# hchautran/SplatFormer

Measured on AMD Instinct MI355X. Metric: refined renders/sec (100k GS, 800x800) at 1/2/4/8 MI355X; PSNR vs ref, higher is better.
Workload: dtype fp32; 1 GPU; B: 100000 Gaussians SH1, full PTv3 (ptv3_base) + heads, 9 views 800x800, forward; parallelism=scene-dp1, attention=non-flash (K=128, ptv3_base.gin:27)

## Files before the change

### include/sfx.h

```cpp
#ifndef SFX_H_
#define SFX_H_

#include <stddef.h>
#include <stdint.h>

#ifdef __cplusplus
extern "C" {
#endif

#define SFX_OK 0
#define SFX_ERR_INVALID -1
#define SFX_ERR_HIP -2
#define SFX_ERR_WORKSPACE -3

int sfx_abi_version(void);
const char* sfx_last_error(void);

size_t sfx_scan_workspace_bytes(long long n);
long long sfx_lookback_timeouts(void* stream);
int sfx_lookback_release(void* stream);
int sfx_scan_i32(long long n, const int32_t* in, int32_t* out, int inclusive, void* ws, size_t ws_bytes,
                 int32_t* total, void* stream);
int sfx_scan_i64(long long n, const int64_t* in, int64_t* out, int inclusive, void* ws, size_t ws_bytes,
                 int64_t* total, void* stream);
// ... 58 lines not shown

int sfx_weight_split(int rows, int cols, const float* w, long long ld, float* w_split, float* w_inv, void* stream);

int sfx_amax_f32(int rows, int cols, const float* x, long long ld, unsigned long long* slot, unsigned tag,
                 void* stream);
int sfx_ln_amax_bound(int C, const float* gamma, const float* beta, unsigned long long* slot, unsigned tag,
                      void* stream);

int sfx_gemm_force_config(int cfg, int stream_k);

int sfx_gemm_force_epilogue(int cls);
int sfx_gemm_last_epilogue(void);

int sfx_set_precision(int mode);
int sfx_get_precision(void);

int sfx_linear_bwd_data(int M, int N, int K, const float* dY, long long ldy, const float* Wt, long long ldwt,
                        const float* rowscale, int dact, int dact_ncols, const float* dact_pre, long long ld_pre,
                        float* dX, long long lddx, int accumulate, const float* wt_split, const float* wt_inv,
                        void* stream);
int sfx_linear_wgrad(int M, int N, int K, const float* dY, long long ldy, const float* X, long long ldx, float* dW,
                     long long ldw, float* db, void* stream);
int sfx_linear_wgrad_rs(int M, int N, int K, const float* dY, long long ldy, const float* X, long long ldx,
                        const float* rowscale, float* scaled, float* dW, long long ldw, float* db, void* stream);
int sfx_subm_conv_wgrad(int n, int cin, int cout, const float* dy, long long ldy, const float* x, long long ldx,
                        const int* nbr, const int* pair_in, const int* pair_out, const int* pair_off_host, float* dw,
                        long long ldw, float* db, void* stream);
int sfx_profile_marker(int tag, void* stream);

int sfx_transpose(int rows, int cols, const float* src, long long lds, float* dst, long long ldd, void* stream);
int sfx_subm_conv_bwd_data(int n, int cin, int cout, const float* dy, long long ldy, const int* nbr,
                           const float* weight_t, const int* pair_in, const int* pair_out, const int* pair_off_host,
                           int* centre_ws, float* dx, long long lddx, const float* wt_split, const float* wt_inv,
                           void* stream);
int sfx_window_attention_bwd(int num_windows, int window, int heads, int head_dim, int channels, const float* qkv,
                             const int* order, const int* win, float scale, const float* attn_out, const float* dout,
                             float* dqkv, float* stats, void* stream);
int sfx_window_attention_varlen_bwd(int num_windows, int max_window, int heads, int head_dim, int channels,
                                    const float* qkv, const int* order, const int* win3, float scale,
                                    const float* dout, float* dqkv, float* stats, void* stream);
int sfx_layernorm_bwd(int M, int C, const float* X, long long ldx, const float* gamma, const float* dY,
                      long long ldgy, const float* dR, long long ldr, float eps, float* dX, long long lddx,
                      void* stream);
size_t sfx_layernorm_wgrad_workspace_bytes(int M, int C);
int sfx_layernorm_wgrad(int M, int C, const float* X, long long ldx, const float* dY, long long ldgy, float eps,
                        void* ws, size_t ws_bytes, float* dgamma, float* dbeta, int accumulate, void* stream);
int sfx_cpe_ln_bwd(int M, int C, const float* U, const float* X1, const float* gamma_cpe, const float* gamma1,
                   const float* dX2, const float* dH, float eps, float* dX1, float* dU, void* stream);
size_t sfx_colsum2_workspace_bytes(int M, int C);
int sfx_bn_stats(int M, int C, const float* X, long long ldx, void* ws, size_t ws_bytes, double* sums, void* stream);
int sfx_bn_finalize(int C, double count, const double* sums, const float* gamma, const float* beta, float eps,
                    float momentum, float* running_mean, float* running_var, float* mean_out, float* rstd_out,
                    float* scale_out, float* shift_out, void* stream);
int sfx_affine_act(int M, int C, const float* X, long long ldx, const float* scale, const float* shift, int act,
                   const float* R, long long ldr, const int* ridx, float* Y, long long ldy, void* stream);
int sfx_bn_act_bwd_reduce(int M, int C, const float* X, long long ldx, const float* mean, const float* rstd,
                          const float* gamma, const float* beta, int act, const float* dY, long long ldgy, void* ws,
                          size_t ws_bytes, double* sums, void* stream);
int sfx_bn_act_bwd_apply(int M, int C, const float* X, long long ldx, const float* mean, const float* rstd,
                         const float* gamma, const float* beta, int act, const float* dY, long long ldgy,
                         const double* sums, double count, float* dX, long long lddx, int accumulate, void* stream);
int sfx_segment_max_arg(int m, int C, const int* idx_ptr, const int* sorted_idx, const float* X, float* Y, int* arg,
                        void* stream);
int sfx_segment_max_bwd(int m, int C, const float* dY, const int* arg, float* dX, void* stream);
int sfx_segment_sum(int m, int C, const int* idx_ptr, const int* sorted_idx, const float* X, long long ldx, float* Y,
                    void* stream);
int sfx_act_bwd(int M, int N, const float* dY, long long ldgy, const float* pre, long long ldp, int act, int ncols,
                float* dX, long long lddx, void* stream);
int sfx_drop_mask(long long n, float keep, unsigned long long seed, float* out, void* stream);
int sfx_sumsq(long long n, const float* x, double* out, void* stream);
int sfx_clip_coef(const double* sumsq, float max_norm, float* coef, float* norm_out, void* stream);
int sfx_adam_step(long long n, float* param, const float* grad, float* exp_avg, float* exp_avg_sq,
                  const float* grad_scale, float lr, float beta1, float beta2, float eps, float weight_decay,
                  int step, void* stream);

int sfx_layernorm(int M, int C, const float* X, long long ldx, const float* gamma, const float* beta, float eps,
                  float* Y, long long ldy, void* stream);
int sfx_cpe_residual_ln(int M, int C, const float* T, const float* X, const float* gamma_cpe, const float* beta_cpe,
                        const float* gamma1, const float* beta1, float eps, float* X_out, float* H, void* stream);
int sfx_cpe_residual_ln_pairs(int M, int C, const float* T, long long ldt, const float* partials, const int* pair_pos,
                              long long num_pairs, const float* X, const float* gamma_cpe, const float* beta_cpe,
                              const float* gamma1, const float* beta1, float eps, float* X_out, float* H,
                              void* stream);
int sfx_cpe_residual_ln_cpairs(int M, int C, const float* T, long long ldt, const float* partials,
                               const int* pair_cpos, long long num_pairs, const float* X, const float* gamma_cpe,
                               const float* beta_cpe, const float* gamma1, const float* beta1, float eps, float* X_out,
                               float* H, void* stream);
int sfx_cpe_ln_qkv_pairs(int M, int C, const float* T, long long ldt, const float* partials, const int* pair_pos,
                         long long num_pairs, const float* X, const float* gamma_cpe, const float* beta_cpe,
                         const float* gamma1, const float* beta1, float eps, float* X_out, const float* w_split,
                         const float* w_inv, const float* bias, float* qkv, unsigned long long* amax_slot,
                         unsigned tag, void* stream);

int sfx_window_attention(int num_windows, int window, int heads, int head_dim, int channels, const float* qkv,
                         const int* order, const int* win, float scale, float* out,
                         const unsigned long long* qkv_amax, unsigned qkv_tag, void* stream);
int sfx_window_attention_varlen(int num_windows, int max_window, int heads, int head_dim, int channels,
                                const float* qkv, const int* order, const int* win3, float scale, float* out,
                                const unsigned long long* qkv_amax, unsigned qkv_tag, void* stream);
int sfx_window_attention_proj(int num_windows, int window, int heads, int head_dim, int channels, const float* qkv,
                              const int* order, const int* win, float scale, const unsigned long long* qkv_amax,
                              unsigned qkv_tag, const float* w_split, const float* w_inv, const float* bias,
                              const float* x1, long long ldx1, float* x2, long long ldx2, void* stream);

int sfx_serialize_keys(int n, const int* grid_coord, const int* batch, int depth, int num_orders, int t0, int t1,
                       int t2, int t3, int code_bits, int64_t* codes, uint64_t* keys, void* stream);
int sfx_serialize_permute(int n, int num_orders, const int* order, const int* inverse, const int64_t* codes,
                          const int* grid, const float* coord, int64_t* codes_p, int* order_p, int* inverse_p,
                          int* grid_p, float* coord_p, void* stream);
int sfx_serialize_finalize(int n, int num_orders, const int* sorted_pos, int* order, int* inverse, void* stream);

int sfx_pool_run_flags(int n, int num_orders, const int* order, const int64_t* codes, int shift, int* flags,
                       void* stream);
int sfx_pool_run_counts(int n, const int* order, const int64_t* codes, const int* shifts, int nshift, int* counts,
                        void* stream);
int sfx_pool_assign_runs(int n, int m, int row0, const int* order, const int* pos, const int* flags, int* cluster,
                         int* idx_ptr, int* head, int* sorted_idx, void* stream);
int sfx_pool_reorder(int n, int m, int num_orders, const int* order, const int* pos, const int* flags,
                     const int* cluster, int* new_order, int* new_inverse, void* stream);
int sfx_pool_gather(int m, int n, int num_orders, const int* head, const int64_t* codes, int pooling_depth,
                    const int* grid_coord, const int* batch, int code_bits, int64_t* new_codes, uint64_t* keys,
                    int* new_grid, int* new_batch, void* stream);
int sfx_segment_max_affine_act(int m, int C, const int* idx_ptr, const int* sorted_idx, const float* X,
                               const float* scale, const float* shift, int act, float* Y, void* stream);
int sfx_segment_mean(int m, int D, const int* idx_ptr, const int* sorted_idx, const float* X, float* Y,
                     void* stream);

int sfx_subm_table_log2(int n);
int sfx_subm_neighbors(int n, const int* grid_coord, const int* batch, int log2cap, unsigned long long* table_keys,
                       int* table_vals, int* nbr, unsigned* mask, unsigned long long* mask_keys, void* stream);
int sfx_subm_permute(int n, const int* perm, const int* nbr, const unsigned* mask, int* nbr_sorted,
                     unsigned* mask_sorted, void* stream);
size_t sfx_subm_pairs_workspace_bytes(int n);
int sfx_subm_pairs(int n, const int* nbr, void* ws, size_t ws_bytes, int* pair_in, int* pair_out, int* pair_off,
                   int with_centre, void* stream);
int sfx_subm_pair_pos(int n, long long num_pairs, const int* pair_out, const int* pair_off, int* pair_pos,
                      void* stream);
size_t sfx_subm_pair_lists_workspace_bytes(int n);
int sfx_subm_pair_lists(int n, const int* nbr, void* ws, size_t ws_bytes, int* pair_in, int* pair_out, int* pair_off,
                        int* pair_pos, int* pair_cpos, int with_centre, void* stream);
int sfx_subm_conv(int n, int cin, int cout, const float* x, long long ldx, const int* nbr, const float* weight,
                  const float* bias, const int* pair_in, const int* pair_out, const int* pair_off_host, float* out,
                  long long ldo, const unsigned long long* x_amax, unsigned x_tag,
                  const unsigned long long* w_amax, unsigned w_tag, const float* w_split, const float* w_inv,
                  void* stream);
int sfx_subm_conv_partials(int n, int cin, int cout, const float* x, long long ldx, const int* nbr,
                           const float* weight, const float* bias, const int* pair_in, const int* pair_out,
                           const int* pair_off_host, float* out, long long ldo, float* partials, long long ldp,
                           const float* w_split, const float* w_inv, void* stream);
int sfx_subm_conv_partials_pairs(int n, int cin, int cout, const float* x, long long ldx, const int* nbr,
                                 const float* weight, const float* bias, const int* pair_in, const int* pair_out,
                                 const int* pair_off_host, float* out, long long ldo, float* partials, long long ldp,
                                 const float* w_split, const float* w_inv, void* stream);

int sfx_gs_pack(int n, const float* means, long long ld_means, const float* scales, long long ld_scales,
                const float* opacities, long long ld_opacities, const float* quats, long long ld_quats,
                const float* features_dc, long long ld_dc, const float* features_rest, long long ld_rest,
                int rest_dim, float grid_resolution, float* feat, long long ld_feat, int* grid_coord, int* grid_max,
                void* stream);
int sfx_offsets_to_batch(int n, int B, const long long* offsets, int* batch, void* stream);
int sfx_move_rows(long long n, int words, const void* src, long long src_ld, const int* idx, void* dst,
                  long long dst_ld, int scatter, void* stream);

int sfx_render_prep_project_views(int n, int views, int num_bases, const float* means, long long ld_means,
                                  const float* log_scales, long long ld_scales, const float* quats_raw,
                                  long long ld_quats, const float* opac_logit, long long ld_opac,
                                  const float* features_dc, long long ld_dc, const float* features_rest,
                                  long long ld_rest, const float* camera_to_worlds, float fx, float fy, float cx,
                                  float cy, int img_h, int img_w, int block_width, float* rgbs, float* opacities,
                                  float* xys, float* depths, int* radii, float* conics, int* num_tiles_hit,
                                  float* records, void* stream);
int sfx_isect_emit_views(int n_total, int n_per_view, const float* xys, const float* depths, const int* radii,
                         const int* cum_tiles_hit, int tiles_x, int tiles_y, int block_width, int64_t* isect_ids,
                         int32_t* gaussian_ids, long long capacity, void* stream);
int sfx_rasterize_fwd_views(int views, int tiles_x, int tiles_y, int block_width, int img_h, int img_w,
                            const int32_t* gids_sorted, const int* tile_bins, const float* xys, const float* conics,
                            const float* colors, const float* opacity, const float* background, int clamp_max1,
                            float* final_Ts, int* final_idx, float* out_img, float* out_alpha, void* stream);
int sfx_isect_count_cull_views(int n_total, int n_per_view, const float* xys, const float* conics,
                               const float* opacities, const int* radii, int tiles_x, int tiles_y, int block_width,
                               int img_h, int img_w, int* num_tiles_kept, void* stream);
int sfx_isect_emit_cull_views(int n_total, int n_per_view, const float* xys, const float* conics,
                              const float* opacities, const float* depths, const int* radii, const int* cum_tiles_hit,
                              int tiles_x, int tiles_y, int block_width, int img_h, int img_w, int64_t* isect_ids,
                              int32_t* gaussian_ids, const int* rank, long long capacity, void* stream);
int sfx_depth_keys(long long n, const float* depths, uint64_t* keys, void* stream);
int sfx_invert_permutation(long long n, const int* perm, int* inv, void* stream);
int sfx_rasterize_fwd_views_quad(int views, int tiles_x, int tiles_y, int block_width, int img_h, int img_w,
                                 const int32_t* gids_sorted, const int* tile_bins, const float* records,
                                 const float* background, int clamp_max1, float* final_Ts, int* final_idx,
                                 float* out_img, float* out_alpha, void* stream);
int sfx_rasterize_bwd_quad(int tiles_x, int tiles_y, int block_width, int img_h, int img_w, const int32_t* gids_sorted,
                           const int* tile_bins, const float* xys, const float* conics, const float* colors,
                           const float* opacity, const float* background, const float* final_Ts, const int* final_idx,
                           const float* v_out, const float* v_out_alpha, float* v_xy, float* v_xy_abs, float* v_conic,
                           float* v_rgb, float* v_opacity, void* stream);
int sfx_rasterize_bwd_views_quad(int views, int tiles_x, int tiles_y, int block_width, int img_h, int img_w,
                                 const int32_t* gids_sorted, const int* tile_bins, const float* xys,
                                 const float* conics, const float* colors, const float* opacity,
                                 const float* background, const float* final_Ts, const int* final_idx,
                                 const float* v_out, const float* v_out_alpha, float* v_xy, float* v_xy_abs,
                                 float* v_conic, float* v_rgb, float* v_opacity, void* stream);
int sfx_render_prep_project_views_bwd(int n, int views, int num_bases, const float* means, long long ld_means,
                                      const float* log_scales, long long ld_scales, const float* quats_raw,
                                      long long ld_quats, const float* opac_logit, long long ld_opac,
                                      const float* features_dc, long long ld_dc, const float* features_rest,
                                      long long ld_rest, const float* camera_to_worlds, float fx, float fy,
                                      const int* radii, const float* conics, const float* v_xys,
                                      const float* v_conics, const float* v_rgbs, const float* v_opacities,
                                      float* v_means, long long ld_v_means, float* v_log_scales,
                                      long long ld_v_scales, float* v_quats_raw, long long ld_v_quats,
                                      float* v_opac_logit, long long ld_v_opac, float* v_features_dc,
                                      long long ld_v_dc, float* v_features_rest, long long ld_v_rest, void* stream);
int sfx_rasterize_fwd_nd(int tiles_x, int tiles_y, int block_width, int img_h, int img_w, int channels,
                         const int32_t* gids_sorted, const int* tile_bins, const float* xys, const float* conics,
                         const float* colors, const float* opacity, const float* background, float* final_Ts,
                         int* final_idx, float* out_img, float* out_alpha, void* stream);
int sfx_rasterize_bwd_nd(int tiles_x, int tiles_y, int block_width, int img_h, int img_w, int channels,
                         const int32_t* gids_sorted, const int* tile_bins, const float* xys, const float* conics,
                         const float* colors, const float* opacity, const float* background, const float* final_Ts,
                         const int* final_idx, const float* v_out, const float* v_out_alpha, float* v_xy,
                         float* v_xy_abs, float* v_conic, float* v_colors, float* v_opacity, void* stream);

int sfx_image_stats_u8(int num_images, long long elems_per_image, const float* pred, const float* gt,
                       int clamp_pred, unsigned long long* sums, int* maxes, void* stream);
size_t sfx_ssim_workspace_bytes(int num_images, int height, int width, int channels);
int sfx_ssim(int num_images, int height, int width, int channels, const float* img1, const float* img2,
             const float* window, int quantize_u8, float* out, void* ws, size_t ws_bytes, void* stream);
size_t sfx_image_loss_workspace_bytes(int num_images, int height, int width, int channels);
int sfx_image_loss(int num_images, int height, int width, int channels, const float* pred, const float* gt,
                   const float* window, float l1_weight, float ssim_weight, const float* view_scale, float* terms,
                   float* d_pred, void* ws, size_t ws_bytes, void* stream);

int sfx_voxel_keys(int n, const float* points, long long ld, float voxel_size, unsigned long long* keys,
                   void* stream);
int sfx_nn1(int n, int m, const float* queries, const float* refs, int* out, void* stream);
int sfx_fps(int n, int m, const float* xyz, int start, int* out, float* dist_ws, void* stream);

size_t sfx_mlp_stream_floats(int C);
size_t sfx_mlp_params_floats(int C);
int sfx_mlp_pack(int C, const float* w1, const float* b1, const float* w2, const float* b2, const float* gamma,
                 const float* beta, float* stream, float* params, int* workspace, void* stream_);
int sfx_block_mlp(int M, int C, const float* x, long long ldx, const float* stream, const float* params, float eps,
                  float* y, long long ldy, int* rowexp, void* stream_);
int sfx_block_mlp_last_plan(int* kind, int* split, int* main_wgs, int* tail_wgs, int* pts);
int sfx_block_mlp_train(int M, int C, const float* x, long long ldx, const float* stream, const float* params,
                        float eps, const float* rowscale, float* z, float* y, long long ldy, void* stream_);
int sfx_block_mlp_bwd(int M, int C, const float* dy, long long lddy, const float* stream, const float* params,
                      const float* rowscale, const float* z, float* dh2, long long lddh, void* stream_);

size_t sfx_subm_cpe_pack_bytes(int C);
int sfx_subm_cpe_pack(int C, const float* w, void* wpk, float* winv, float* ws, void* stream);
int sfx_subm_order_keys(int n, const int* nbr, uint64_t* keys, void* stream);
int sfx_subm_rowexp(int n, int C, const float* x, int* e, void* stream);
int sfx_subm_cpe_ln(int n, int C, const float* xc, const float* xres, const int* nbr, const int* perm,
                    const int* rowexp, const void* wpk, const float* winv, const float* bias, const float* gamma_cpe,
                    const float* beta_cpe, const float* gamma1, const float* beta1, float eps, float* x_out,
                    float* h_out, void* stream);

int sfx_point_embed(int n, int K, int N, const float* x, long long ldx, const float* w, const float* b,
                    const float* scale, const float* shift, float* y, long long ldy, void* stream);

size_t sfx_heads_stream_floats(int ng, int kin);
size_t sfx_heads_params_floats(int out_dim);
int sfx_heads_pack(int ng, int kin, int out_dim, const float* w1, int ld1, const float* b1, const float* wm,
                   const float* bm, const float* w4, const float* b4, float* stream, float* params, int* ws,
                   void* stream_);
int sfx_heads(int M, int ng, int kin, int out_dim, const float* x, long long ldx, int res_off, int n_tanh,
              const int* ocols, const float* stream, const float* params, float* y, void* stream_);

#ifdef __cplusplus
}
#endif

#endif
```

### splatformer_amd/csrc/gemm.hip

```cpp
#include <climits>
#include <cstdlib>
#include <cstring>
#include <type_traits>

#include "gemm_common.h"


namespace {

using namespace sfxg;

inline bool aligned16(const void* p) { return (reinterpret_cast<uintptr_t>(p) & 15) == 0; }

inline bool fits(long long rows, long long ld) { return rows * ld * 4 + 64 < (long long)OOB; }

struct TileCfg {
  int bm, bn, nw;
  float eff;
};
constexpr TileCfg kCfgs[] = {{128, 128, 4, 1.0f}, {128, 96, 4, 0.95f}, {128, 64, 4, 0.8f}, {64, 128, 4, 0.95f},
                             {64, 64, 4, 0.8f},   {256, 128, 8, 1.05f}, {128, 256, 8, 1.05f}};
constexpr int kNumCfgs = sizeof(kCfgs) / sizeof(kCfgs[0]);

thread_local int g_prec = 0;
// ... 461 lines not shown
      const int row = 4 * c4 + j;
#pragma unroll
      for (int q = 0; q < NQ; ++q)
        *reinterpret_cast<uint4*>(img + (op * 3 + q) * WG2_PLANE + chunk_off(row, mg)) =
            make_uint4(t0[q].x, t0[q].y, t1[q].x, t1[q].y);
    }
    __syncthreads();
    if (m0 + BK < m_end) {
      load(m0 + BK);
      load_idx(m0 + 2 * BK);
    }
#pragma unroll
    for (int s = 0; s < 2; ++s) {
      bf16x8 af[2][3], bf[2][3];
#pragma unroll
      for (int i = 0; i < 2; ++i)
#pragma unroll
        for (int q = 0; q < NQ; ++q) {
          af[i][q] = __builtin_bit_cast(bf16x8, *reinterpret_cast<const uint4*>(
                                                    img + q * WG2_PLANE + chunk_off(wn * 64 + i * 32 + l32, 2 * s + h)));
          bf[i][q] = __builtin_bit_cast(bf16x8, *reinterpret_cast<const uint4*>(
                                                    img + (3 + q) * WG2_PLANE + chunk_off(wk * 64 + i * 32 + l32, 2 * s + h)));
        }
      constexpr int QA[6] = {2, 1, 0, 1, 0, 0}, QB[6] = {0, 1, 2, 0, 1, 0};
#pragma unroll
      for (int i = 0; i < 2; ++i)
#pragma unroll
        for (int j = 0; j < 2; ++j)
#pragma unroll
          for (int p = NQ == 3 ? 0 : 3; p < 6; ++p)
            acc[i][j] = __builtin_amdgcn_mfma_f32_32x32x16_bf16(af[i][QA[p]], bf[j][QB[p]], acc[i][j], 0, 0, 0);
    }
  }
  if (do_db) {
#pragma unroll
    for (int j = 0; j < 4; ++j)
      if (col + j < N) atomicAdd(&db[col + j], dbs[j]);
  }
  const __amdgpu_buffer_rsrc_t rW = rsrc(dW);
  const unsigned ldw32 = (unsigned)ldw;
#pragma unroll
  for (int i = 0; i < 2; ++i)
#pragma unroll
    for (int j = 0; j < 2; ++j) {
      const int k = k0 + wk * 64 + j * 32 + l32;
#pragma unroll
      for (int r = 0; r < 16; ++r) {
        const int n = n0 + wn * 64 + i * 32 + (r & 3) + 8 * (r >> 2) + 4 * h;
        __builtin_amdgcn_raw_ptr_buffer_atomic_fadd_f32(
            acc[i][j][r], rW, (n < N && k < K) ? ((unsigned)n * ldw32 + (unsigned)k) * 4u : OOB, 0, 0);
      }
    }
}

template <int NQ, int SRC>
__global__ void __launch_bounds__(256, 2) wgrad2_kernel(int M, int N, int K, const float* __restrict__ dY,
                                                        long long ldy, const float* __restrict__ X, long long ldx,
                                                        float* __restrict__ dW, long long ldw, int chunk,
                                                        float* __restrict__ db) {
  __shared__ __attribute__((aligned(16))) char img[2 * 3 * WG2_PLANE];
  const int tiles_k = (K + WG2_T - 1) / WG2_T;
  const int n0 = (blockIdx.x / tiles_k) * WG2_T, k0 = (blockIdx.x % tiles_k) * WG2_T;
  const int m_begin = blockIdx.y * chunk;
  const int m_end = min(M, m_begin + chunk);
  wgrad2_body<NQ, SRC>(img, m_begin, m_end, N, K, n0, k0, dY, ldy, X, ldx, dW, ldw, db, nullptr, nullptr, 0, 0);
}

struct SubmWgradPlan {
  int pair_off[28];
  int item_off[28];
  int chunk;
};

template <int NQ>
__global__ void __launch_bounds__(256, 2) subm_wgrad_kernel(int n, int cin, int cout, const float* __restrict__ dY,
                                                            long long ldy, const float* __restrict__ X, long long ldx,
                                                            const int* __restrict__ nbr,
                                                            const int* __restrict__ pair_in,
                                                            const int* __restrict__ pair_out, SubmWgradPlan plan,
                                                            float* __restrict__ dW, long long ldw,
                                                            float* __restrict__ db) {
  __shared__ __attribute__((aligned(16))) char img[2 * 3 * WG2_PLANE];
  const int tiles_k = (cin + WG2_T - 1) / WG2_T;
  const int n0 = (blockIdx.x / tiles_k) * WG2_T, k0 = (blockIdx.x % tiles_k) * WG2_T;
  const int item = blockIdx.y;
  int k = 0;
  while (k < 26 && item >= plan.item_off[k + 1]) ++k;
  const bool centre = k == 13;
  const int base = centre ? 0 : plan.pair_off[k];
  const int count = centre ? n : plan.pair_off[k + 1] - base;
  const int m_begin = base + (item - plan.item_off[k]) * plan.chunk;
  const int m_end = min(base + count, m_begin + plan.chunk);
  wgrad2_body<NQ, WG2_PAIRS>(img, m_begin, m_end, cout, cin, n0, k0, dY, ldy, X, ldx, dW + (long long)k * cin, ldw,
                             centre ? db : nullptr, centre ? nullptr : pair_out, centre ? nbr : pair_in,
                             centre ? 27 : 1, centre ? 13 : 0);
}

__global__ void __launch_bounds__(256) rowscale_rows_kernel(int M, int n4, const float* __restrict__ dY, long long ldy,
                                                            const float* __restrict__ rowscale,
                                                            float* __restrict__ out) {
  const long long i = (long long)blockIdx.x * 256 + threadIdx.x;
  if (i >= (long long)M * n4) return;
  const int m = (int)(i / n4), c = (int)(i % n4) * 4;
  const float s = rowscale[m];
  const float4 v = *reinterpret_cast<const float4*>(dY + (long long)m * ldy + c);
  *reinterpret_cast<float4*>(out + i * 4) = make_float4(v.x * s, v.y * s, v.z * s, v.w * s);
}

__global__ void __launch_bounds__(256) transpose_kernel(int rows, int cols, const float* __restrict__ src,
                                                        long long lds, float* __restrict__ dst, long long ldd) {
  __shared__ float t[32][33];
  const int r0 = blockIdx.y * 32, c0 = blockIdx.x * 32;
  const int tx = threadIdx.x & 31, ty = threadIdx.x >> 5;
  for (int i = ty; i < 32; i += 8) {
    const int r = r0 + i, c = c0 + tx;
    t[i][tx] = (r < rows && c < cols) ? src[(long long)r * lds + c] : 0.f;
  }
  __syncthreads();
  for (int i = ty; i < 32; i += 8) {
    const int c = c0 + i, r = r0 + tx;
    if (c < cols && r < rows) dst[(long long)c * ldd + r] = t[tx][i];
  }
}


__global__ void centre_pairs_kernel(int n, const int* __restrict__ nbr, int* __restrict__ gather,
                                    int* __restrict__ scatter) {
  const int i = blockIdx.x * 256 + threadIdx.x;
  if (i >= n) return;
  gather[i] = i;
  scatter[i] = nbr[(long long)i * 27 + 13];
}

}

extern "C" {

int sfx_gemm_force_config(int cfg, int stream_k) {
  SFX_REQUIRE(cfg >= -1 && cfg < kNumCfgs && stream_k >= -1 && stream_k <= 1, "sfx_gemm_force_config: bad values");
  read_force_env();
  forced = cfg;
  forced_sk = stream_k;
  return SFX_OK;
}

int sfx_gemm_force_epilogue(int cls) {
  SFX_REQUIRE(cls == -1 || cls == 0, "sfx_gemm_force_epilogue: class %d (-1 automatic, 0 general)", cls);
  forced_epi = cls;
  return SFX_OK;
}

int sfx_gemm_last_epilogue(void) { return last_epi; }

int sfx_weight_split(int rows, int cols, const float* w, long long ld, float* w_split, float* w_inv, void* stream) {
  SFX_REQUIRE(rows >= 0 && cols > 0 && cols % 4 == 0 && ld >= cols && ld % 4 == 0,
              "sfx_weight_split: bad sizes (cols and ld must be multiples of 4)");
  if (rows == 0) return SFX_OK;
  SFX_REQUIRE(w && w_split && w_inv, "sfx_weight_split: null buffer");
  SFX_REQUIRE((reinterpret_cast<uintptr_t>(w) & 15) == 0 && (reinterpret_cast<uintptr_t>(w_split) & 15) == 0,
              "sfx_weight_split: buffers must be 16-byte aligned");
  weight_split_kernel<<<sfx::ceil_div(rows, 4), 256, 0, sfx::as_stream(stream)>>>(rows, cols, w, ld, w_split, w_inv);
  return sfx::check_launch("sfx_weight_split");
}

int sfx_amax_f32(int rows, int cols, const float* x, long long ld, unsigned long long* slot, unsigned tag,
                 void* stream) {
  SFX_REQUIRE(rows >= 0 && cols >= 0 && ld >= cols, "sfx_amax_f32: bad sizes");
  SFX_REQUIRE(slot && tag != 0, "sfx_amax_f32: null slot or tag 0");
  SFX_REQUIRE(rows == 0 || cols == 0 || x, "sfx_amax_f32: null buffer");
  const AmaxJob j{x, ld, 0, rows, cols, 1, nullptr, 0, 1};
  amax_kernel<<<dim3(amax_blocks(j), 1), 256, 0, sfx::as_stream(stream)>>>(j, j, slot, slot, tag, tag);
  return sfx::check_launch("sfx_amax_f32");
}

int sfx_linear(int M, int N, int K, const float* A, long long lda, const int* gather_idx, int num_segments,
               const float* W, long long ldw, const float* bias, const float* scale, const float* shift, int act,
               int act_ncols, const float* R, long long ldr, const int* residual_idx, float* Y, long long ldy,
               float* Ypre, long long ldypre, int groups, long long group_stride_A, long long group_stride_W,
               long long group_stride_bias, long long group_stride_Y, const int* out_row_idx, const float* rowscale,
               int pre_before_act, const unsigned long long* a_amax, unsigned a_tag,
               const unsigned long long* w_amax, unsigned w_tag, unsigned long long* y_amax, unsigned y_tag,
               const float* w_split, const float* w_inv, void* stream) {
  SFX_REQUIRE(M >= 0 && N > 0 && K > 0, "sfx_linear: bad sizes M=%d N=%d K=%d", M, N, K);
  SFX_REQUIRE(act >= 0 && act <= 3, "sfx_linear: bad activation %d", act);
  SFX_REQUIRE(groups >= 1, "sfx_linear: groups < 1");
  if (M == 0) return SFX_OK;
  SFX_REQUIRE(A && W && Y, "sfx_linear: null buffer");
  const int S = gather_idx ? num_segments : 1;
  SFX_REQUIRE(!gather_idx || (S >= 1 && K % S == 0), "sfx_linear: K must be a multiple of num_segments");
  const int Kseg = K / S;
  SFX_REQUIRE(!gather_idx || Kseg % 4 == 0, "sfx_linear: gathered segment width must be a multiple of 4");
  SFX_REQUIRE(ldw >= K && (gather_idx || lda >= K) && ldy >= N, "sfx_linear: leading dimension too small");
  SFX_REQUIRE(!(scale == nullptr) == !(shift == nullptr), "sfx_linear: scale and shift go together");
  SFX_REQUIRE((gather_idx || fits(M, lda)) && fits(M, ldy) && fits(N, ldw) && (!R || residual_idx || fits(M, ldr)) &&
                  (!Ypre || fits(M, ldypre)),
              "sfx_linear: operand exceeds the 2 GiB buffer-descriptor range");
  GemmArgs a{};
  a.M = M; a.N = N; a.K = K; a.A = A; a.lda = lda; a.gidx = gather_idx; a.S = S; a.Kseg = Kseg; a.gstride = S;
  a.W = W; a.ldw = ldw; a.bias = bias; a.scale = scale; a.shift = shift; a.act = act;
  a.act_ncols = act_ncols < 0 ? N : act_ncols; a.R = R; a.ldr = ldr; a.ridx = residual_idx; a.Y = Y; a.ldy = ldy;
  a.Ypre = Ypre; a.ldypre = ldypre; a.gA = group_stride_A; a.gW = group_stride_W; a.gB = group_stride_bias;
  a.gY = group_stride_Y; a.out_rows = out_row_idx; a.rowscale = rowscale; a.pre_before_act = pre_before_act;
  a.a_amax = a_amax; a.a_tag = a_tag; a.w_amax = w_amax; a.w_tag = w_tag; a.y_amax = y_amax; a.y_tag = y_tag;
  const bool vec = (K % 4 == 0) && (lda % 4 == 0) && (ldw % 4 == 0) && aligned16(A) && aligned16(W) &&
                   (group_stride_A % 4 == 0) && (group_stride_W % 4 == 0);
  SFX_REQUIRE(!w_split == !w_inv, "sfx_linear: w_split and w_inv go together");
  if (w_split && vec && aligned16(w_split)) {
    SFX_REQUIRE(groups == 1 || group_stride_W == (long long)N * K, "sfx_linear: w_split needs contiguous groups");
    a.Wsp = w_split; a.ldws = K; a.winv = w_inv; a.gWinv = N;
  }
  dispatch(a, groups, vec, sfx::as_stream(stream));
  return sfx::check_launch("sfx_linear");
}

static int subm_conv_impl(int n, int cin, int cout, const float* x, long long ldx, const int* nbr,
                          const float* weight, const float* bias, const int* pair_in, const int* pair_out,
                          const int* pair_off_host, float* out, long long ldo, const unsigned long long* x_amax,
                          unsigned x_tag, const unsigned long long* w_amax, unsigned w_tag, const float* w_split,
                          const float* w_inv, float* partials, long long ldp, void* stream,
                          bool skip_centre = false) {
  SFX_REQUIRE(n >= 0 && cin > 0 && cout > 0, "sfx_subm_conv: bad sizes");
  if (n == 0) return SFX_OK;
  SFX_REQUIRE(x && nbr && weight && out && pair_off_host, "sfx_subm_conv: null buffer");
  SFX_REQUIRE(ldx >= cin && ldo >= cout, "sfx_subm_conv: leading dimension too small");
  SFX_REQUIRE(fits(n, ldx) && fits(n, ldo) && fits(cout, 27ll * cin),
              "sfx_subm_conv: operand exceeds the 2 GiB buffer-descriptor range");
  SFX_REQUIRE(!partials || (ldp >= cout && fits(pair_off_host[27], ldp)),
              "sfx_subm_conv_partials: partials leading dimension too small or too large");
  hipStream_t st = sfx::as_stream(stream);
  const bool vec = (cin % 4 == 0) && (ldx % 4 == 0) && aligned16(x) && aligned16(weight);
  GemmArgs a{};
  a.M = n; a.N = cout; a.K = cin; a.A = x; a.lda = ldx; a.gidx = nbr + 13; a.S = 1; a.Kseg = cin; a.gstride = 27;
  for (const TunedLaunch& t : kTunedConv)
    if (t.N == cout && t.K == cin && 5ll * n >= 4ll * t.M && 4ll * n <= 5ll * t.M) {
      a.tuned = t.cfg + 1;
      a.tuned_sk = t.sk;
      break;
    }
  a.W = weight + 13ll * cin; a.ldw = 27ll * cin; a.bias = bias; a.act = 0; a.act_ncols = cout; a.Y = out; a.ldy = ldo;
  a.a_amax = x_amax; a.a_tag = x_tag; a.w_amax = w_amax; a.w_tag = w_tag;
  SFX_REQUIRE(!w_split == !w_inv, "sfx_subm_conv: w_split and w_inv go together");
  if (w_split && vec && aligned16(w_split)) {
    a.Wsp = w_split + 13ll * cin; a.ldws = 27ll * cin; a.winv = w_inv;
  }
  if (!a.Wsp && vec && split_mode(cin) == 2 &&
      !prepare_amax(a, AmaxJob{x, ldx, 0, n, cin, 1, nullptr, 0, 1},
                    AmaxJob{weight, 27ll * cin, 0, cout, 27 * cin, 1, nullptr, 0, 1}, st)) {
    a.a_amax = a.w_amax = nullptr;
  }
  if (!skip_centre) {
    dispatch(a, 1, vec, st);
    int rc = sfx::check_launch("sfx_subm_conv(centre)");
    if (rc) return rc;
  }
  if (!pair_in || pair_off_host[27] == 0) return SFX_OK;
  GemmArgs b = a;
  b.gidx = nullptr; b.bias = nullptr; b.gstride = 1; b.pair_mode = 1; b.pair_in = pair_in; b.pair_out = pair_out;
  b.W = weight; b.slice_w_stride = cin; b.num_slices = 27;
  if (a.Wsp) b.Wsp = w_split;
  for (int k = 0; k <= 27; ++k) b.slice_pair_off[k] = pair_off_host[k];
  b.M = pair_off_host[27];
  if (partials) {
    b.pair_store = 1;
    b.Y = partials;
    b.ldy = ldp;
  }
  dispatch(b, 1, vec, st);
  return sfx::check_launch("sfx_subm_conv(pairs)");
}

int sfx_subm_conv(int n, int cin, int cout, const float* x, long long ldx, const int* nbr, const float* weight,
                  const float* bias, const int* pair_in, const int* pair_out, const int* pair_off_host, float* out,
                  long long ldo, const unsigned long long* x_amax, unsigned x_tag,
                  const unsigned long long* w_amax, unsigned w_tag, const float* w_split, const float* w_inv,
                  void* stream) {
  return subm_conv_impl(n, cin, cout, x, ldx, nbr, weight, bias, pair_in, pair_out, pair_off_host, out, ldo, x_amax,
                        x_tag, w_amax, w_tag, w_split, w_inv, nullptr, 0, stream);
}

int sfx_subm_conv_partials(int n, int cin, int cout, const float* x, long long ldx, const int* nbr,
                           const float* weight, const float* bias, const int* pair_in, const int* pair_out,
                           const int* pair_off_host, float* out, long long ldo, float* partials, long long ldp,
                           const float* w_split, const float* w_inv, void* stream) {
  SFX_REQUIRE(n == 0 || pair_off_host[27] == 0 || (partials && pair_in && pair_out),
              "sfx_subm_conv_partials: null partials / pair lists");
  return subm_conv_impl(n, cin, cout, x, ldx, nbr, weight, bias, pair_in, pair_out, pair_off_host, out, ldo, nullptr,
                        0, nullptr, 0, w_split, w_inv, partials, ldp, stream);
}

int sfx_subm_conv_partials_pairs(int n, int cin, int cout, const float* x, long long ldx, const int* nbr,
                                 const float* weight, const float* bias, const int* pair_in, const int* pair_out,
                                 const int* pair_off_host, float* out, long long ldo, float* partials, long long ldp,
                                 const float* w_split, const float* w_inv, void* stream) {
  SFX_REQUIRE(n == 0 || pair_off_host[27] == 0 || (partials && pair_in && pair_out),
              "sfx_subm_conv_partials_pairs: null partials / pair lists");
  return subm_conv_impl(n, cin, cout, x, ldx, nbr, weight, bias, pair_in, pair_out, pair_off_host, out, ldo, nullptr,
                        0, nullptr, 0, w_split, w_inv, partials, ldp, stream, true);
}

int sfx_subm_conv_bwd_data(int n, int cin, int cout, const float* dy, long long ldy, const int* nbr,
                           const float* weight_t, const int* pair_in, const int* pair_out, const int* pair_off_host,
                           int* centre_ws, float* dx, long long lddx, const float* wt_split, const float* wt_inv,
                           void* stream) {
  SFX_REQUIRE(n >= 0 && cin > 0 && cout > 0, "sfx_subm_conv_bwd_data: bad sizes");
  if (n == 0) return SFX_OK;
  SFX_REQUIRE(dy && nbr && weight_t && dx && pair_off_host && centre_ws, "sfx_subm_conv_bwd_data: null buffer");
  SFX_REQUIRE(ldy >= cout && lddx >= cin, "sfx_subm_conv_bwd_data: leading dimension too small");
  SFX_REQUIRE(fits(n, ldy) && fits(n, lddx) && fits(27ll * cin, cout),
              "sfx_subm_conv_bwd_data: operand exceeds the 2 GiB buffer-descriptor range");
  hipStream_t st = sfx::as_stream(stream);
  const bool vec = (cout % 4 == 0) && (ldy % 4 == 0) && aligned16(dy) && aligned16(weight_t);
  SFX_REQUIRE(!wt_split == !wt_inv, "sfx_subm_conv_bwd_data: wt_split and wt_inv go together");
  const bool presplit = wt_split && vec && aligned16(wt_split);
  GemmArgs am{};
  if (!presplit && vec && split_mode(cout) == 2)
    (void)prepare_amax(am, AmaxJob{dy, ldy, 0, n, cout, 1, nullptr, 0, 1},
                       AmaxJob{weight_t, (long long)cout, 0, 27 * cin, cout, 1, nullptr, 0, 1}, st);
  int* cg = centre_ws;
  int* cs = centre_ws + n;
  centre_pairs_kernel<<<sfx::ceil_div(n, 256), 256, 0, st>>>(n, nbr, cg, cs);
  GemmArgs a{};
  a.N = cin; a.K = cout; a.A = dy; a.lda = ldy; a.S = 1; a.Kseg = cout; a.gstride = 1;
  a.ldw = cout; a.act = 0; a.act_ncols = cin; a.Y = dx; a.ldy = lddx;
  a.pair_mode = 1; a.slice_w_stride = (long long)cin * cout;
  a.a_amax = am.a_amax; a.a_tag = am.a_tag; a.w_amax = am.w_amax; a.w_tag = am.w_tag;
  if (presplit) { a.ldws = cout; a.winv = wt_inv; a.slice_winv_stride = cin; }
  GemmArgs c = a;
  c.pair_in = cg; c.pair_out = cs; c.W = weight_t + 13ll * cin * cout; c.num_slices = 1;
  if (presplit) { c.Wsp = wt_split + 13ll * cin * cout; c.winv = wt_inv + 13ll * cin; }
  c.slice_pair_off[0] = 0; c.slice_pair_off[1] = n; c.M = n;
  dispatch(c, 1, vec, st);
  int rc = sfx::check_launch("sfx_subm_conv_bwd_data(centre)");
  if (rc || !pair_in || pair_off_host[27] == 0) return rc;
  GemmArgs b = a;
  b.pair_in = pair_out; b.pair_out = pair_in; b.W = weight_t; b.num_slices = 27;
  if (presplit) b.Wsp = wt_split;
  for (int k = 0; k <= 27; ++k) b.slice_pair_off[k] = pair_off_host[k];
  b.M = pair_off_host[27];
  dispatch(b, 1, vec, st);
  return sfx::check_launch("sfx_subm_conv_bwd_data(pairs)");
}

int sfx_linear_bwd_data(int M, int N, int K, const float* dY, long long ldy, const float* Wt, long long ldwt,
                        const float* rowscale, int dact, int dact_ncols, const float* dact_pre, long long ld_pre,
                        float* dX, long long lddx, int accumulate, const float* wt_split, const float* wt_inv,
                        void* stream) {
  SFX_REQUIRE(M >= 0 && N > 0 && K > 0, "sfx_linear_bwd_data: bad sizes M=%d N=%d K=%d", M, N, K);
  SFX_REQUIRE(dact >= 0 && dact <= 3, "sfx_linear_bwd_data: bad dact %d", dact);
  if (M == 0) return SFX_OK;
  SFX_REQUIRE(dY && Wt && dX && (!dact || dact_pre), "sfx_linear_bwd_data: null buffer");
  SFX_REQUIRE(ldy >= N && ldwt >= N && lddx >= K && (!dact || ld_pre >= K), "sfx_linear_bwd_data: leading dim");
  SFX_REQUIRE(fits(M, ldy) && fits(K, ldwt) && fits(M, lddx) && (!dact || fits(M, ld_pre)),
              "sfx_linear_bwd_data: operand exceeds the 2 GiB buffer-descriptor range");
  GemmArgs a{};
  a.M = M; a.N = K; a.K = N; a.A = dY; a.lda = ldy; a.S = 1; a.Kseg = N; a.gstride = 1;
  a.W = Wt; a.ldw = ldwt; a.act = 0; a.act_ncols = dact_ncols < 0 ? K : dact_ncols;
  a.Y = dX; a.ldy = lddx;
  if (accumulate) { a.R = dX; a.ldr = lddx; }
  a.rowscale = rowscale; a.dact = dact; a.dact_pre = dact_pre; a.ld_dact = ld_pre;
  const bool vec = (N % 4 == 0) && (ldy % 4 == 0) && (ldwt % 4 == 0) && aligned16(dY) && aligned16(Wt);
  SFX_REQUIRE(!wt_split == !wt_inv, "sfx_linear_bwd_data: wt_split and wt_inv go together");
  if (wt_split && vec && aligned16(wt_split)) {
    a.Wsp = wt_split; a.ldws = N; a.winv = wt_inv;
  }
  dispatch(a, 1, vec, sfx::as_stream(stream));
  return sfx::check_launch("sfx_linear_bwd_data");
}

int sfx_set_precision(int mode) {
  SFX_REQUIRE(mode == 0 || mode == 1, "sfx_set_precision: mode %d (0 fp32-accurate, 1 reference precision)", mode);
  g_prec = mode;
  return SFX_OK;
}

int sfx_get_precision(void) { return g_prec; }

static int linear_wgrad(const char* what, int M, int N, int K, const float* dY, long long ldy, const float* X,
                        long long ldx, float* dW, long long ldw, float* db, void* stream) {
  SFX_REQUIRE(M >= 0 && N > 0 && K > 0, "%s: bad sizes M=%d N=%d K=%d", what, M, N, K);
  if (M == 0) return SFX_OK;
  SFX_REQUIRE(dY && X && dW, "%s: null buffer", what);
  SFX_REQUIRE(N % 4 == 0 && K % 4 == 0 && ldy % 4 == 0 && ldx % 4 == 0 && aligned16(dY) && aligned16(X),
              "%s: N, K, leading dims must be multiples of 4 and operands 16-byte aligned", what);
  SFX_REQUIRE(ldy >= N && ldx >= K && ldw >= K, "%s: leading dim", what);
  SFX_REQUIRE(fits(M, ldy) && fits(M, ldx) && fits(N, ldw), "%s: operand exceeds 2 GiB range", what);
  hipStream_t st = sfx::as_stream(stream);
  const int slabs = (int)sfx::ceil_div(M, BK);
  if (split_mode(M) != 0) {
    const int tiles2 = (int)(sfx::ceil_div(N, WG2_T) * sfx::ceil_div(K, WG2_T));
    int splits2 = (int)sfx::ceil_div(2 * num_cus(), tiles2);
    if (splits2 > slabs) splits2 = slabs;
    if (splits2 < 1) splits2 = 1;
    const int chunk2 = (int)sfx::ceil_div(slabs, splits2) * BK;
    splits2 = (int)sfx::ceil_div(M, chunk2);
    if (g_prec == 1)
      wgrad2_kernel<2, WG2_DENSE><<<dim3(tiles2, splits2), 256, 0, st>>>(M, N, K, dY, ldy, X, ldx, dW, ldw, chunk2, db);
    else
      wgrad2_kernel<3, WG2_DENSE><<<dim3(tiles2, splits2), 256, 0, st>>>(M, N, K, dY, ldy, X, ldx, dW, ldw, chunk2, db);
    return sfx::check_launch(what);
  }
  const int tiles = (int)(sfx::ceil_div(N, WG_TILE) * sfx::ceil_div(K, WG_TILE));
  int splits = (int)sfx::ceil_div(4 * num_cus(), tiles);
  if (splits > slabs) splits = slabs;
  if (splits < 1) splits = 1;
  const int chunk = (int)sfx::ceil_div(slabs, splits) * BK;
  splits = (int)sfx::ceil_div(M, chunk);
  wgrad_kernel<<<dim3(tiles, splits), THREADS, 0, st>>>(M, N, K, dY, ldy, X, ldx, dW, ldw, chunk, db);
  return sfx::check_launch(what);
}

int sfx_linear_wgrad(int M, int N, int K, const float* dY, long long ldy, const float* X, long long ldx, float* dW,
                     long long ldw, float* db, void* stream) {
  return linear_wgrad("sfx_linear_wgrad", M, N, K, dY, ldy, X, ldx, dW, ldw, db, stream);
}

int sfx_linear_wgrad_rs(int M, int N, int K, const float* dY, long long ldy, const float* X, long long ldx,
                        const float* rowscale, float* scaled, float* dW, long long ldw, float* db, void* stream) {
  if (!rowscale || M <= 0) return linear_wgrad("sfx_linear_wgrad_rs", M, N, K, dY, ldy, X, ldx, dW, ldw, db, stream);
  SFX_REQUIRE(N > 0 && N % 4 == 0 && dY && ldy >= N && ldy % 4 == 0 && aligned16(dY) && fits(M, ldy),
              "sfx_linear_wgrad_rs: bad dY");
  SFX_REQUIRE(scaled && aligned16(scaled) && fits(M, N), "sfx_linear_wgrad_rs: scaled must be M*N floats, 16-byte aligned");
  rowscale_rows_kernel<<<sfx::ceil_div((long long)M * (N / 4), 256), 256, 0, sfx::as_stream(stream)>>>(
      M, N / 4, dY, ldy, rowscale, scaled);
  int rc = sfx::check_launch("sfx_linear_wgrad_rs(scale)");
  if (rc) return rc;
  return linear_wgrad("sfx_linear_wgrad_rs", M, N, K, scaled, N, X, ldx, dW, ldw, db, stream);
}

int sfx_subm_conv_wgrad(int n, int cin, int cout, const float* dy, long long ldy, const float* x, long long ldx,
                        const int* nbr, const int* pair_in, const int* pair_out, const int* pair_off_host, float* dw,
                        long long ldw, float* db, void* stream) {
  SFX_REQUIRE(n >= 0 && cin > 0 && cout > 0, "sfx_subm_conv_wgrad: bad sizes");
  if (n == 0) return SFX_OK;
  SFX_REQUIRE(dy && x && nbr && dw && pair_off_host, "sfx_subm_conv_wgrad: null buffer");
  SFX_REQUIRE(cin % 4 == 0 && cout % 4 == 0 && ldy % 4 == 0 && ldx % 4 == 0 && aligned16(dy) && aligned16(x),
              "sfx_subm_conv_wgrad: channels and leading dims must be multiples of 4 and operands 16-byte aligned");
  SFX_REQUIRE(ldy >= cout && ldx >= cin && ldw >= 27ll * cin, "sfx_subm_conv_wgrad: leading dimension too small");
  SFX_REQUIRE(fits(n, ldy) && fits(n, ldx) && fits(cout, ldw) && fits(n, 27),
              "sfx_subm_conv_wgrad: operand exceeds the 2 GiB buffer-descriptor range");
  const int pairs = pair_off_host[27];
  SFX_REQUIRE(pair_off_host[0] == 0 && pairs >= 0 && pairs <= 26ll * n && pair_off_host[14] == pair_off_host[13],
              "sfx_subm_conv_wgrad: pair offsets are not those of lists without the centre offset");
  for (int k = 0; k < 27; ++k)
    SFX_REQUIRE(pair_off_host[k + 1] >= pair_off_host[k], "sfx_subm_conv_wgrad: pair offsets decrease");
  SFX_REQUIRE(pairs == 0 || (pair_in && pair_out && fits(pairs, 1)), "sfx_subm_conv_wgrad: null pair lists");
  const int tiles = (int)(sfx::ceil_div(cout, WG2_T) * sfx::ceil_div(cin, WG2_T));
  const long long total = (long long)n + pairs;
  const long long want = sfx::ceil_div(2 * num_cus(), tiles);
  SubmWgradPlan plan;
  plan.chunk = (int)sfx::ceil_div(sfx::ceil_div(total, want), BK) * BK;
// ... 27 lines not shown
```

### splatformer_amd/csrc/gemm_common.h

```cpp
#pragma once

#include <type_traits>

#include "common.h"

namespace sfxg {

typedef float floatx16 __attribute__((ext_vector_type(16)));
typedef float floatx4 __attribute__((ext_vector_type(4)));
typedef __bf16 bf16x8 __attribute__((ext_vector_type(8)));

constexpr int BK = 32;
#ifndef SFX_PERCU4
#define SFX_PERCU4 2
#endif
#ifndef SFX_PERCU8
#define SFX_PERCU8 1
#endif
#ifndef SFX_NBUF8
#define SFX_NBUF8 2
#endif
constexpr int kPerCu4 = SFX_PERCU4, kPerCu8 = SFX_PERCU8;
constexpr int LDS_STRIDE = BK + 4;
constexpr int THREADS = 256;
constexpr unsigned OOB = 0x7ffffff0u;
constexpr int RSRC_FLAGS = 0x00020000;

enum Act { ACT_NONE = 0, ACT_GELU = 1, ACT_RELU = 2, ACT_TANH = 3 };
enum Epi { EPI_GENERAL = 0, EPI_LIN = 1, EPI_LIN_GELU = 2, EPI_PAIR_STORE = 3 };

struct GemmArgs {
  int M, N, K;
  const float* A;
  long long lda;
  const int* gidx;
  int S, Kseg, gstride;
  const float* W;
  long long ldw;
  const float* bias;
  const float* scale;
  const float* shift;
  int act, act_ncols;
  const float* R;
  long long ldr;
  const int* ridx;
  float* Y;
  long long ldy;
  float* Ypre;
  long long ldypre;
  long long gA, gW, gB, gY;
  const int* out_rows;
  int pair_mode;
  const int* pair_in;
  const int* pair_out;
  int slice_tile_off[28];
  int slice_pair_off[28];
  int num_slices;
  long long slice_w_stride;
  const float* rowscale;
  int pre_before_act;
  const float* dact_pre;
  long long ld_dact;
  int dact;
  int sk;
  int split;
  const unsigned long long* a_amax;
  const unsigned long long* w_amax;
  unsigned a_tag, w_tag;
  unsigned long long* y_amax;
  unsigned y_tag;
  const float* Wsp;
  long long ldws;
  const float* winv;
  long long gWinv;
  long long slice_winv_stride;
  int tuned, tuned_sk;
  int pair_store;
  int epi;
  int dbg;
};

__device__ __forceinline__ int row_exp(float m) {
  int e = __builtin_amdgcn_frexp_expf(m);
  e = 13 - e;
  return e > 126 ? 126 : (e < -126 ? -126 : e);
}

__device__ __forceinline__ float gelu_erf(float x) {
  const float t = fminf(fabsf(x), 5.65f);
  float q = 2.79405867e-06f;
  q = __builtin_fmaf(q, t, -3.89084234e-05f);
  q = __builtin_fmaf(q, t, 0.000184072458f);
  q = __builtin_fmaf(q, t, 0.000141672252f);
  q = __builtin_fmaf(q, t, -0.00706906663f);
  q = __builtin_fmaf(q, t, 0.0524996631f);
  q = __builtin_fmaf(q, t, 0.459207207f);
  q = __builtin_fmaf(q, t, 1.15110528f);
  const float half_tail = 0.5f * __builtin_amdgcn_exp2f(-(t * q));
  return x >= 0.f ? x * (1.f - half_tail) : (x < -5.65f ? 0.f : x * half_tail);
}
__device__ __forceinline__ float gelu_erf_grad(float x) {
  const float cdf = 0.5f * (1.f + erff(x * 0.70710678118654752f));
  const float pdf = 0.39894228040143268f * expf(-0.5f * x * x);
  return cdf + x * pdf;
}
enum DAct { DACT_NONE = 0, DACT_GELU = 1, DACT_RELU = 2, DACT_TANH_OUT = 3 };
__device__ __forceinline__ float dact_grad(int dact, float pre) {
  if (dact == DACT_GELU) return gelu_erf_grad(pre);
  if (dact == DACT_RELU) return pre > 0.f ? 1.f : 0.f;
  return 1.f - pre * pre;
}

__device__ __forceinline__ __amdgpu_buffer_rsrc_t rsrc(const void* p) {
  const unsigned long long a = reinterpret_cast<unsigned long long>(p);
  const unsigned lo = __builtin_amdgcn_readfirstlane((unsigned)a);
  const unsigned hi = __builtin_amdgcn_readfirstlane((unsigned)(a >> 32));
  void* u = reinterpret_cast<void*>(((unsigned long long)hi << 32) | lo);
  return __builtin_amdgcn_make_buffer_rsrc(u, (short)0, (int)OOB, RSRC_FLAGS);
}

__device__ __forceinline__ __amdgpu_buffer_rsrc_t rsrc_ext(const void* p, unsigned bytes) {
  const unsigned long long a = reinterpret_cast<unsigned long long>(p);
  const unsigned lo = __builtin_amdgcn_readfirstlane((unsigned)a);
  const unsigned hi = __builtin_amdgcn_readfirstlane((unsigned)(a >> 32));
  void* u = reinterpret_cast<void*>(((unsigned long long)hi << 32) | lo);
  return __builtin_amdgcn_make_buffer_rsrc(u, (short)0, (int)__builtin_amdgcn_readfirstlane(bytes), RSRC_FLAGS);
}

__device__ __forceinline__ float4 bload4(__amdgpu_buffer_rsrc_t r, unsigned off) {
  const floatx4 v = __builtin_bit_cast(floatx4, __builtin_amdgcn_raw_buffer_load_b128(r, off, 0, 0));
  return make_float4(v.x, v.y, v.z, v.w);
}
__device__ __forceinline__ float bload1(__amdgpu_buffer_rsrc_t r, unsigned off) {
  return __builtin_bit_cast(float, __builtin_amdgcn_raw_buffer_load_b32(r, off, 0, 0));
}
__device__ __forceinline__ int bload1i(__amdgpu_buffer_rsrc_t r, unsigned off) {
  return (int)__builtin_amdgcn_raw_buffer_load_b32(r, off, 0, 0);
}
__device__ __forceinline__ void bstore1(__amdgpu_buffer_rsrc_t r, unsigned off, float v) {
  __builtin_amdgcn_raw_buffer_store_b32(__builtin_bit_cast(unsigned, v), r, off, 0, 0);
}

using sfx::split3;
using sfx::split2h;

enum Mode { MODE_DENSE = 0, MODE_GATHER1 = 1, MODE_GATHERS = 2, MODE_PAIR = 3 };

inline int num_cus() {
  static int cus = 0;
  if (!cus) {
    int dev = 0;
    (void)hipGetDevice(&dev);
    if (hipDeviceGetAttribute(&cus, hipDeviceAttributeMultiprocessorCount, dev) != hipSuccess || cus <= 0) cus = 256;
  }
  return cus;
}

inline int tiles_m_of(GemmArgs& a, int BM) {
  if (!a.pair_mode) return (int)sfx::ceil_div(a.M, BM);
  int t = 0;
  for (int k = 0; k < a.num_slices; ++k) {
    a.slice_tile_off[k] = t;
    t += (a.slice_pair_off[k + 1] - a.slice_pair_off[k] + BM - 1) / BM;
  }
  a.slice_tile_off[a.num_slices] = t;
  return t;
}

void launch_m0_w4(int cfg, const GemmArgs& a, int groups, bool vec, hipStream_t st);
void launch_m0_w8(int cfg, const GemmArgs& a, int groups, bool vec, hipStream_t st);
void launch_m1_w4(int cfg, const GemmArgs& a, int groups, bool vec, hipStream_t st);
void launch_m1_w8(int cfg, const GemmArgs& a, int groups, bool vec, hipStream_t st);
void launch_m2_w4(int cfg, const GemmArgs& a, int groups, bool vec, hipStream_t st);
void launch_m3_w4(int cfg, const GemmArgs& a, int groups, bool vec, hipStream_t st);
void launch_m3_w8(int cfg, const GemmArgs& a, int groups, bool vec, hipStream_t st);

}
```

### splatformer_amd/csrc/gemm_kernel.h

```cpp
#pragma once
#include <climits>
#include <cstdlib>
#include <cstring>
#include <type_traits>

#include "gemm_common.h"


namespace {

using namespace sfxg;



template <int BM, int BN, int WGM, int NW, bool VEC, int MODE, int SPL, int EPI = EPI_GENERAL>
__global__ void __launch_bounds__(NW * 64, NW == 4 ? 2 : 1) gemm_kernel(GemmArgs p, int tiles_n, int total_tiles) {
  constexpr bool SPLIT = SPL != 0;
  static_assert(EPI == EPI_GENERAL || (SPL == 2 && VEC), "specialised epilogues: fp16x2 operands only");
  static_assert((EPI != EPI_LIN && EPI != EPI_LIN_GELU) || MODE == MODE_DENSE, "EPI_LIN*: dense rows");
  static_assert(EPI != EPI_PAIR_STORE || MODE == MODE_PAIR, "EPI_PAIR_STORE: pair mode");
  constexpr bool F16 = SPL == 2 || SPL == 1;
  constexpr int NTERM = SPL == 1 ? 1 : (F16 ? 2 : 3);
  static_assert(SPL == 0 || SPL == 1 || SPL == 2 || SPL == 3, "operand precision");
  constexpr int NT = NW * 64;
  constexpr int WGN = NW / WGM;
  constexpr int WM = BM / WGM, WN = BN / WGN;
  constexpr int MB = WM / 32, NB = WN / 32;
  constexpr int RPP = NT / 8;
  static_assert(WM % 32 == 0 && WN % 32 == 0 && (BM * BK / 4) % NT == 0 && (BN * BK / 4) % NT == 0,
                "tile shape must split into 32x32 MFMA blocks and whole staging passes");
  static_assert(SPLIT || NW == 4, "fp32 tiles run 4 waves");
  constexpr int A_ITERS = BM * BK / 4 / NT;
  constexpr int W_ITERS = BN * BK / 4 / NT;
  constexpr int NBUF = SPLIT ? (NW == 8 ? SFX_NBUF8 : 1) : 2;
  constexpr int AUX_FLOATS = F16 ? NBUF * BM + 2 * BM + 4 : 0;
  constexpr int A_FLOATS = (SPLIT ? NBUF * NTERM * BM * BK / 2 : 2 * BM * LDS_STRIDE) + AUX_FLOATS;
  constexpr int W_FLOATS = SPLIT ? NBUF * NTERM * BN * BK / 2 : 2 * BN * LDS_STRIDE;
  __shared__ __attribute__((aligned(16))) float sAraw[A_FLOATS];
  __shared__ __attribute__((aligned(16))) float sWraw[W_FLOATS];
  float (*sA)[BM * LDS_STRIDE] = reinterpret_cast<float (*)[BM * LDS_STRIDE]>(sAraw);
  float (*sW)[BN * LDS_STRIDE] = reinterpret_cast<float (*)[BN * LDS_STRIDE]>(sWraw);
  char* sAs = reinterpret_cast<char*>(sAraw);
  char* sWs = reinterpret_cast<char*>(sWraw);
  auto swz = [](int r, int c4) -> int { return r * 64 + ((((c4 >> 1) ^ (r >> 2)) & 3) << 4) + ((c4 & 1) << 3); };
  float* s_fac = sAraw + (A_FLOATS - AUX_FLOATS);
  float* s_inv = s_fac + NBUF * BM;
  int* s_flag = reinterpret_cast<int*>(s_inv + 2 * BM);

  const int g = blockIdx.z;
  const float* A = p.A + g * p.gA;
  const float* bias = p.bias ? p.bias + g * p.gB : nullptr;
  float* Y = p.Y + g * p.gY;
  const __amdgpu_buffer_rsrc_t rA = rsrc(A);
  const __amdgpu_buffer_rsrc_t rY = rsrc(Y);
  const __amdgpu_buffer_rsrc_t rR = rsrc(p.R ? p.R : Y);
  const __amdgpu_buffer_rsrc_t rP = rsrc(p.Ypre ? p.Ypre : Y);

  const int tid = threadIdx.x, lane = tid & 63, wid = tid >> 6;
  const int wm = wid / WGN, wn = wid % WGN;
  const int h = lane >> 5, l32 = lane & 31;
  const int K = p.K;
  const int nk = (K + BK - 1) / BK;
  if constexpr (F16) {
    if (tid < NBUF) s_flag[tid] = 0;
  }
  const unsigned lda32 = (unsigned)p.lda, ldw32 = (unsigned)p.ldw, ldy32 = (unsigned)p.ldy, ldws32 = (unsigned)p.ldws;
  const unsigned ldr32 = (unsigned)p.ldr, ldp32 = (unsigned)p.ldypre;
  const int lrow = tid >> 3, lcol = (tid & 7) * 4;

  struct Tile {
    int m0, n0, M;
    const int* gidx;
    int gstride;
    const int* out_rows;
    const float* W;
    const float* winv;
  };
  auto tile_info = [&](int t) -> Tile {
    Tile ti;
    const int tm = t / tiles_n, tn = t - tm * tiles_n;
    ti.n0 = tn * BN;
    ti.m0 = tm * BM;
    ti.M = p.M;
    ti.gidx = MODE == MODE_DENSE ? nullptr : p.gidx;
    ti.gstride = p.gstride;
    ti.out_rows = p.out_rows;
    ti.W = (F16 ? p.Wsp : p.W) + g * p.gW;
    ti.winv = p.winv ? p.winv + g * p.gWinv : nullptr;
    if constexpr (MODE == MODE_PAIR) {
      int sl = 0;
      for (int q = 1; q < p.num_slices; ++q)
        if (p.slice_tile_off[q] <= tm) sl = q;
      const int base = p.slice_pair_off[sl];
      ti.M = p.slice_pair_off[sl + 1] - base;
      ti.m0 = (tm - p.slice_tile_off[sl]) * BM;
      ti.gidx = p.pair_in + base;
      ti.gstride = 1;
      ti.out_rows = p.pair_out + base;
      ti.W = (F16 ? p.Wsp : p.W) + sl * p.slice_w_stride;
      if (p.winv) ti.winv = p.winv + sl * p.slice_winv_stride;
    }
    return ti;
  };

  int grow[A_ITERS];
  auto load_rows = [&](const Tile& ti, int kt, int (&rows)[A_ITERS]) {
    if constexpr (MODE != MODE_DENSE) {
      const __amdgpu_buffer_rsrc_t rG = rsrc(ti.gidx);
      const int seg = MODE == MODE_GATHERS ? (kt * BK + lcol) / p.Kseg : 0;
#pragma unroll
      for (int i = 0; i < A_ITERS; ++i) {
        const int m = ti.m0 + lrow + RPP * i;
        rows[i] = bload1i(rG, (m < ti.M && seg < p.S) ? ((unsigned)m * (unsigned)ti.gstride + (unsigned)seg) * 4u
                                                      : OOB);
      }
    }
  };

  float4 ra[A_ITERS], rw[W_ITERS];
  auto load_tiles = [&](const Tile& ti, int kt, bool first) {
    const __amdgpu_buffer_rsrc_t rW = rsrc(ti.W);
    const int k = kt * BK + lcol;
    const bool kin = k < K && !(p.dbg & 2);
    int seg = 0, kk = k;
    if constexpr (MODE == MODE_GATHERS) {
      seg = k / p.Kseg;
      kk = k - seg * p.Kseg;
    }
#pragma unroll
    for (int i = 0; i < A_ITERS; ++i) {
      const int m = ti.m0 + lrow + RPP * i;
      const bool mok = m < ti.M;
      unsigned off;
      if constexpr (MODE != MODE_DENSE) {
        const int r = grow[i];
        off = (mok && r >= 0 && kin && seg < p.S) ? ((unsigned)r * lda32 + (unsigned)kk) * 4u : OOB;
      } else {
        off = (mok && kin) ? ((unsigned)m * lda32 + (unsigned)kk) * 4u : OOB;
      }
      if (VEC) {
        ra[i] = bload4(rA, off);
      } else {
        float4 v;
        v.x = bload1(rA, (k + 0 < K) ? off : OOB);
        v.y = bload1(rA, (k + 1 < K) ? off + 4 : OOB);
        v.z = bload1(rA, (k + 2 < K) ? off + 8 : OOB);
        v.w = bload1(rA, (k + 3 < K) ? off + 12 : OOB);
        ra[i] = v;
      }
    }
#pragma unroll
    for (int i = 0; i < W_ITERS; ++i) {
      const int n = ti.n0 + lrow + RPP * i;
      const unsigned off = (n < p.N && kin) ? ((unsigned)n * (F16 ? ldws32 : ldw32) + (unsigned)k) * 4u : OOB;
      if (VEC) {
        rw[i] = bload4(rW, off);
      } else {
        float4 v;
        v.x = bload1(rW, (k + 0 < K) ? off : OOB);
        v.y = bload1(rW, (k + 1 < K) ? off + 4 : OOB);
        v.z = bload1(rW, (k + 2 < K) ? off + 8 : OOB);
        v.w = bload1(rW, (k + 3 < K) ? off + 12 : OOB);
        rw[i] = v;
      }
    }
  };
  int erow[A_ITERS];
  float srow[A_ITERS], thr[A_ITERS];
#pragma unroll
  for (int i = 0; i < A_ITERS; ++i) { erow[i] = INT_MIN; srow[i] = 1.f; thr[i] = 0.f; }
  int sq = 0, cq = 0;
  int sp = 0;
  auto store_tiles = [&](int buf, bool first, int par) {
    if (p.dbg & 8) return;
    if constexpr (SPLIT) {
      const int b = NBUF == 2 ? buf : 0;
      if constexpr (F16) {
        ++sq;
        float m[A_ITERS];
        bool over = false;
#pragma unroll
        for (int i = 0; i < A_ITERS; ++i) {
          m[i] = fmaxf(fmaxf(fabsf(ra[i].x), fabsf(ra[i].y)), fmaxf(fabsf(ra[i].z), fabsf(ra[i].w)));
          over |= m[i] > thr[i];
        }
        bool dec = false;
        if (first || __builtin_amdgcn_ballot_w64(over) != 0) {
#pragma unroll
          for (int i = 0; i < A_ITERS; ++i) {
            float mr = m[i];
            mr = fmaxf(mr, __int_as_float(__builtin_amdgcn_mov_dpp(__float_as_int(mr), 0xB1, 0xF, 0xF, false)));
            mr = fmaxf(mr, __int_as_float(__builtin_amdgcn_mov_dpp(__float_as_int(mr), 0x4E, 0xF, 0xF, false)));
            mr = fmaxf(mr, __int_as_float(__builtin_amdgcn_mov_dpp(__float_as_int(mr), 0x141, 0xF, 0xF, false)));
            int e = first ? INT_MIN : erow[i];
            float fac = 1.f;
            bool chg = first;
            if (mr > 0.f && mr <= 3.4028235e38f) {
              int e2 = 13 - __builtin_amdgcn_frexp_expf(mr);
              e2 = e2 > 126 ? 126 : (e2 < -126 ? -126 : e2);
              if (e == INT_MIN) {
                e = e2;
                chg = true;
              } else if (mr * srow[i] > 65504.f) {
                fac = ldexpf(1.f, e2 - e);
                e = e2;
                chg = true;
                dec = true;
              }
            }
            erow[i] = e;
            const bool set = e != INT_MIN;
            srow[i] = set ? ldexpf(1.f, e) : 1.f;
            thr[i] = set ? ldexpf(65504.f, -e) : 0.f;
            if ((tid & 7) == 0) {
              s_fac[b * BM + lrow + RPP * i] = fac;
              if (chg) s_inv[par * BM + lrow + RPP * i] = set ? ldexpf(1.f, -e) : 1.f;
            }
          }
        } else if ((tid & 7) == 0) {
#pragma unroll
          for (int i = 0; i < A_ITERS; ++i) s_fac[b * BM + lrow + RPP * i] = 1.f;
        }
        if (__builtin_amdgcn_ballot_w64(dec) != 0 && lane == 0) s_flag[b] = sq;
#pragma unroll
        for (int i = 0; i < A_ITERS; ++i) {
          uint2 t[2];
          split2h(ra[i], srow[i], t);
          const int o = swz(lrow + RPP * i, lcol >> 2);
          *reinterpret_cast<uint2*>(sAs + ((b * NTERM + 0) * BM) * 64 + o) = t[0];
          if constexpr (NTERM == 2) *reinterpret_cast<uint2*>(sAs + ((b * NTERM + 1) * BM) * 64 + o) = t[1];
        }
#pragma unroll
        for (int i = 0; i < W_ITERS; ++i) {
          const uint4 w = __builtin_bit_cast(uint4, rw[i]);
          const int o = swz(lrow + RPP * i, lcol >> 2);
          *reinterpret_cast<uint2*>(sWs + ((b * NTERM + 0) * BN) * 64 + o) = make_uint2(w.x, w.y);
          if constexpr (NTERM == 2) *reinterpret_cast<uint2*>(sWs + ((b * NTERM + 1) * BN) * 64 + o) = make_uint2(w.z, w.w);
        }
        return;
      } else {
#pragma unroll
      for (int i = 0; i < A_ITERS; ++i) {
        uint2 t[NTERM];
        split3(ra[i], t);
        const int o = swz(lrow + RPP * i, lcol >> 2);
#pragma unroll
        for (int q = 0; q < NTERM; ++q) *reinterpret_cast<uint2*>(sAs + ((b * NTERM + q) * BM) * 64 + o) = t[q];
      }
#pragma unroll
      for (int i = 0; i < W_ITERS; ++i) {
        uint2 t[NTERM];
        split3(rw[i], t);
        const int o = swz(lrow + RPP * i, lcol >> 2);
#pragma unroll
        for (int q = 0; q < NTERM; ++q) *reinterpret_cast<uint2*>(sWs + ((b * NTERM + q) * BN) * 64 + o) = t[q];
      }
      return;
      }
    }
#pragma unroll
    for (int i = 0; i < A_ITERS; ++i)
      *reinterpret_cast<float4*>(&sA[buf][(lrow + RPP * i) * LDS_STRIDE + lcol]) = ra[i];
#pragma unroll
    for (int i = 0; i < W_ITERS; ++i)
      *reinterpret_cast<float4*>(&sW[buf][(lrow + RPP * i) * LDS_STRIDE + lcol]) = rw[i];
  };

  floatx16 acc[MB][NB];
  auto zero_acc = [&]() {
#pragma unroll
    for (int a = 0; a < MB; ++a)
#pragma unroll
      for (int b = 0; b < NB; ++b)
#pragma unroll
        for (int r = 0; r < 16; ++r) acc[a][b][r] = 0.f;
  };

  float ebias[NB], escale[NB], eshift[NB], ewinv[NB];
  int mrow[MB][16];
  float ymax = 0.f;
  auto load_mrow = [&](const Tile& ti, __amdgpu_buffer_rsrc_t rO) {
#pragma unroll
    for (int a = 0; a < MB; ++a)
#pragma unroll
      for (int r = 0; r < 16; ++r) {
        const int mt = ti.m0 + wm * WM + a * 32 + (r & 3) + 8 * (r >> 2) + 4 * h;
        mrow[a][r] = bload1i(rO, mt < ti.M ? (unsigned)mt * 4u : OOB);
// ... 307 lines not shown
        }
        if (p.Ypre && !p.pre_before_act) {
#pragma unroll
          for (int r = 0; r < 16; ++r) {
            const int m = mrow[a][r];
            bstore1(rP, (nok && m >= 0) ? ((unsigned)m * ldp32 + (unsigned)n) * 4u : OOB, v[r]);
          }
        }
        if (p.R && owner0) {
          float rv[16];
          const __amdgpu_buffer_rsrc_t rI = rsrc(p.ridx ? (const void*)p.ridx : (const void*)p.W);
          int rr[16];
#pragma unroll
          for (int r = 0; r < 16; ++r) {
            const int m = mrow[a][r];
            const int ri = bload1i(rI, (p.ridx && m >= 0) ? (unsigned)m * 4u : OOB);
            rr[r] = p.ridx ? ri : m;
          }
#pragma unroll
          for (int r = 0; r < 16; ++r) {
            const int m = mrow[a][r];
            rv[r] = bload1(rR, (nok && m >= 0) ? ((unsigned)rr[r] * ldr32 + (unsigned)n) * 4u : OOB);
          }
#pragma unroll
          for (int r = 0; r < 16; ++r) v[r] += rv[r];
        }
        if (p.y_amax) {
#pragma unroll
          for (int r = 0; r < 16; ++r) ymax = fmaxf(ymax, mrow[a][r] >= 0 ? fabsf(v[r]) : 0.f);
        }
        if (partial) {
#pragma unroll
          for (int r = 0; r < 16; ++r) {
            const int m = mrow[a][r];
            __builtin_amdgcn_raw_ptr_buffer_atomic_fadd_f32(
                v[r], rY, (nok && m >= 0) ? ((unsigned)m * ldy32 + (unsigned)n) * 4u : OOB, 0, 0);
          }
        } else {
#pragma unroll
          for (int r = 0; r < 16; ++r) {
            const int m = mrow[a][r];
            bstore1(rY, (nok && m >= 0) ? ((unsigned)m * ldy32 + (unsigned)n) * 4u : OOB, v[r]);
          }
        }
      }
    }
  };

  auto compute_split = [&](int buf, int s0, int s1) {
    const int bb = NBUF == 2 ? buf : 0;
    typedef __attribute__((ext_vector_type(8))) _Float16 f16x8;
    typedef typename std::conditional<F16, f16x8, bf16x8>::type frag_t;
#pragma unroll
    for (int s = s0; s < s1; ++s) {
      frag_t af[MB][NTERM], wf[NB][NTERM];
#pragma unroll
      for (int q = 0; q < NTERM; ++q) {
#pragma unroll
        for (int a = 0; a < MB; ++a) {
          const int r = wm * WM + a * 32 + l32;
          af[a][q] = __builtin_bit_cast(
              frag_t, *reinterpret_cast<const uint4*>(sAs + ((bb * NTERM + q) * BM) * 64 + swz(r, 4 * s + 2 * h)));
        }
#pragma unroll
        for (int b = 0; b < NB; ++b) {
          const int r = wn * WN + b * 32 + l32;
          wf[b][q] = __builtin_bit_cast(
              frag_t, *reinterpret_cast<const uint4*>(sWs + ((bb * NTERM + q) * BN) * 64 + swz(r, 4 * s + 2 * h)));
        }
      }
      if constexpr (F16) {
        constexpr int QA[3] = {1, 0, 0}, QW[3] = {0, 1, 0};
#pragma unroll
        for (int j = SPL == 1 ? 2 : 0; j < 3; ++j)
#pragma unroll
          for (int a = 0; a < MB; ++a)
#pragma unroll
            for (int b = 0; b < NB; ++b)
              acc[a][b] = __builtin_amdgcn_mfma_f32_32x32x16_f16(af[a][QA[j]], wf[b][QW[j]], acc[a][b], 0, 0, 0);
      } else {
        constexpr int QA[6] = {2, 1, 0, 1, 0, 0}, QW[6] = {0, 1, 2, 0, 1, 0};
#pragma unroll
        for (int j = 0; j < 6; ++j)
#pragma unroll
          for (int a = 0; a < MB; ++a)
#pragma unroll
            for (int b = 0; b < NB; ++b)
              acc[a][b] = __builtin_amdgcn_mfma_f32_32x32x16_bf16(af[a][QA[j]], wf[b][QW[j]], acc[a][b], 0, 0, 0);
      }
    }
  };
  auto compute = [&](int buf) {
    if (p.dbg & 1) return;
    if constexpr (F16) {
      ++cq;
      const int b = NBUF == 2 ? buf : 0;
      if (__builtin_amdgcn_readfirstlane(s_flag[b]) == cq) {
#pragma unroll
        for (int a = 0; a < MB; ++a)
#pragma unroll
          for (int gq = 0; gq < 4; ++gq) {
            const float4 f = *reinterpret_cast<const float4*>(s_fac + b * BM + wm * WM + a * 32 + 8 * gq + 4 * h);
#pragma unroll
            for (int bb = 0; bb < NB; ++bb) {
              acc[a][bb][4 * gq + 0] *= f.x;
              acc[a][bb][4 * gq + 1] *= f.y;
              acc[a][bb][4 * gq + 2] *= f.z;
              acc[a][bb][4 * gq + 3] *= f.w;
            }
          }
      }
    }
    if constexpr (SPLIT) {
      compute_split(buf, 0, BK / 16);
      return;
    }
    const float* a_lds = &sA[buf][(wm * WM + l32) * LDS_STRIDE + h * 16];
    const float* w_lds = &sW[buf][(wn * WN + l32) * LDS_STRIDE + h * 16];
#pragma unroll
    for (int c = 0; c < 4; ++c) {
      float4 af[MB], wf[NB];
#pragma unroll
      for (int a = 0; a < MB; ++a) af[a] = *reinterpret_cast<const float4*>(a_lds + a * 32 * LDS_STRIDE + 4 * c);
#pragma unroll
      for (int b = 0; b < NB; ++b) wf[b] = *reinterpret_cast<const float4*>(w_lds + b * 32 * LDS_STRIDE + 4 * c);
#pragma unroll
      for (int a = 0; a < MB; ++a)
#pragma unroll
        for (int b = 0; b < NB; ++b) {
          acc[a][b] = __builtin_amdgcn_mfma_f32_32x32x2f32(af[a].x, wf[b].x, acc[a][b], 0, 0, 0);
          acc[a][b] = __builtin_amdgcn_mfma_f32_32x32x2f32(af[a].y, wf[b].y, acc[a][b], 0, 0, 0);
          acc[a][b] = __builtin_amdgcn_mfma_f32_32x32x2f32(af[a].z, wf[b].z, acc[a][b], 0, 0, 0);
          acc[a][b] = __builtin_amdgcn_mfma_f32_32x32x2f32(af[a].w, wf[b].w, acc[a][b], 0, 0, 0);
        }
    }
  };

  const int nwg = (int)gridDim.x;
  const int lid = (nwg % 8 == 0) ? (int)(blockIdx.x % 8) * (nwg / 8) + (int)(blockIdx.x / 8) : (int)blockIdx.x;
  int t, kb = 0, ke = nk;
  long long it_end = 0;
  if (p.sk) {
    const long long total_it = (long long)total_tiles * nk;
    const long long it0 = total_it * lid / nwg;
    it_end = total_it * (lid + 1) / nwg;
    if (it0 >= it_end) return;
    t = (int)(it0 / nk);
    kb = (int)(it0 - (long long)t * nk);
    ke = (int)min((long long)nk, kb + (it_end - it0));
  } else {
    t = lid;
    if (t >= total_tiles) return;
  }
  constexpr bool per_tile_rows = MODE == MODE_GATHER1 || MODE == MODE_PAIR;
  Tile ti = tile_info(t);
  load_rows(ti, kb, grow);
  load_tiles(ti, kb, true);
  store_tiles(0, true, sp);
  __syncthreads();
  int buf = 0;
  while (true) {
    int nt, nke = nk;
    bool has_next;
    if (p.sk) {
      nt = t + 1;
      has_next = (long long)nt * nk < it_end;
      if (has_next) nke = (int)min((long long)nk, it_end - (long long)nt * nk);
    } else {
      nt = t + nwg;
      has_next = nt < total_tiles;
    }
    const Tile tn = has_next ? tile_info(nt) : ti;
    int grow_next[A_ITERS];
    if constexpr (per_tile_rows) load_rows(tn, 0, grow_next);
    zero_acc();
    for (int kt = kb; kt + 1 < ke; ++kt) {
      if constexpr (MODE == MODE_GATHERS) load_rows(ti, kt + 1, grow);
      load_tiles(ti, kt + 1, false);
      __builtin_amdgcn_sched_barrier(0);
      compute(buf);
      __builtin_amdgcn_sched_barrier(0);
      if constexpr (NBUF == 1) __syncthreads();
      store_tiles(buf ^ 1, false, sp);
      __syncthreads();
      if constexpr (NBUF == 2) buf ^= 1;
    }
    pre_epilogue(ti);
    if (has_next) {
      if constexpr (per_tile_rows) {
#pragma unroll
        for (int i = 0; i < A_ITERS; ++i) grow[i] = grow_next[i];
      } else {
        load_rows(tn, 0, grow);
      }
      load_tiles(tn, 0, true);
    }
    __builtin_amdgcn_sched_barrier(0);
    compute(buf);
    __builtin_amdgcn_sched_barrier(0);
    epilogue(ti, kb != 0 || ke != nk, kb == 0);
    if (!has_next) break;
    if constexpr (NBUF == 1) __syncthreads();
    __builtin_amdgcn_sched_barrier(0);
    store_tiles(buf ^ 1, true, sp ^ 1);
    __syncthreads();
    if constexpr (NBUF == 2) buf ^= 1;
    sp ^= 1;
    t = nt;
    ti = tn;
    kb = 0;
    ke = nke;
  }
  if (p.y_amax) {
    __shared__ float ywaves[NW];
    sfx::publish_amax(ymax, p.y_amax, p.y_tag, ywaves);
  }
}
template <int BM, int BN, int WGM, int NW, int MODE>
void launch_f16x2(const GemmArgs& a, dim3 grid, int tiles_n, int total, hipStream_t st) {
  constexpr int T = NW * 64;
  if constexpr (MODE == MODE_DENSE) {
    if (a.epi == EPI_LIN) {
      gemm_kernel<BM, BN, WGM, NW, true, MODE, 2, EPI_LIN><<<grid, T, 0, st>>>(a, tiles_n, total);
      return;
    }
    if (a.epi == EPI_LIN_GELU) {
      gemm_kernel<BM, BN, WGM, NW, true, MODE, 2, EPI_LIN_GELU><<<grid, T, 0, st>>>(a, tiles_n, total);
      return;
    }
  }
  if constexpr (MODE == MODE_PAIR) {
    if (a.epi == EPI_PAIR_STORE) {
      gemm_kernel<BM, BN, WGM, NW, true, MODE, 2, EPI_PAIR_STORE><<<grid, T, 0, st>>>(a, tiles_n, total);
      return;
    }
  }
  gemm_kernel<BM, BN, WGM, NW, true, MODE, 2><<<grid, T, 0, st>>>(a, tiles_n, total);
}

template <int BM, int BN, int WGM, int NW, int MODE>
void launch(GemmArgs a, int groups, bool vec, hipStream_t st) {
  const bool split = a.split != 0;
  const int tiles_m = tiles_m_of(a, BM);
  const int tiles_n = (int)sfx::ceil_div(a.N, BN);
  const int total = tiles_m * tiles_n;
  const int per_cu = NW == 4 ? kPerCu4 : kPerCu8;
  const int slots = per_cu * num_cus() / groups > 0 ? per_cu * num_cus() / groups : 1;
  int grid_x;
  if (a.sk) {
    const long long iters = (long long)total * sfx::ceil_div(a.K, BK);
    grid_x = (int)(iters < slots ? iters : slots);
    if (grid_x >= 8) grid_x = grid_x / 8 * 8;
    if (grid_x < 1) grid_x = 1;
    if (!a.pair_mode)
      (void)hipMemset2DAsync(a.Y, (size_t)a.ldy * 4, 0, (size_t)a.N * 4, (size_t)a.M, st);
  } else {
    const int per = (total + slots - 1) / slots;
    grid_x = total > 0 ? (total + per - 1) / per : 1;
    if (grid_x >= 8) grid_x = (grid_x + 7) / 8 * 8;
  }
  dim3 grid(grid_x, 1, groups);
  if constexpr (NW == 8) {
    if (a.split == 2)
      launch_f16x2<BM, BN, WGM, 8, MODE>(a, grid, tiles_n, total, st);
    else if (a.split == 1)
      gemm_kernel<BM, BN, WGM, 8, true, MODE, 1><<<grid, 512, 0, st>>>(a, tiles_n, total);
    else
      gemm_kernel<BM, BN, WGM, 8, true, MODE, 3><<<grid, 512, 0, st>>>(a, tiles_n, total);
  } else {
    if (vec && a.split == 2)
      launch_f16x2<BM, BN, WGM, 4, MODE>(a, grid, tiles_n, total, st);
    else if (vec && a.split == 1)
      gemm_kernel<BM, BN, WGM, 4, true, MODE, 1><<<grid, 256, 0, st>>>(a, tiles_n, total);
    else if (vec && split)
      gemm_kernel<BM, BN, WGM, 4, true, MODE, 3><<<grid, 256, 0, st>>>(a, tiles_n, total);
    else if (vec)
      gemm_kernel<BM, BN, WGM, 4, true, MODE, 0><<<grid, 256, 0, st>>>(a, tiles_n, total);
    else
      gemm_kernel<BM, BN, WGM, 4, false, MODE, 0><<<grid, 256, 0, st>>>(a, tiles_n, total);
  }
}

}
```

### splatformer_amd/csrc/subm.hip

```cpp
#include "common.h"

#include <climits>

namespace {

constexpr unsigned long long EMPTY = ~0ull;

__device__ __forceinline__ unsigned long long pack(int b, int x, int y, int z) {
  return ((unsigned long long)(unsigned)b << 48) | ((unsigned long long)(unsigned)(x + 1) << 32) |
         ((unsigned long long)(unsigned)(y + 1) << 16) | (unsigned long long)(unsigned)(z + 1);
}

__device__ __forceinline__ unsigned slot_of(unsigned long long key, int log2cap) {
  return (unsigned)((key * 0x9E3779B97F4A7C15ull) >> (64 - log2cap));
}

__global__ void subm_init_kernel(long long cap, int n, unsigned long long* __restrict__ keys, int* __restrict__ vals,
                                 unsigned* __restrict__ mask, unsigned long long* __restrict__ mask_keys) {
  const long long t = (long long)blockIdx.x * blockDim.x + threadIdx.x;
  if (t < cap) {
    keys[t] = EMPTY;
    vals[t] = 0x7f7f7f7f;
  }
  if (t < n) {
    if (mask) mask[t] = 0u;
    if (mask_keys) mask_keys[t] = 0ull;
  }
}

__global__ void subm_insert_kernel(int n, const int* __restrict__ grid, const int* __restrict__ batch,
                                   unsigned long long* __restrict__ keys, int* __restrict__ vals, int log2cap) {
  const int i = blockIdx.x * blockDim.x + threadIdx.x;
  if (i >= n) return;
  const unsigned long long key = pack(batch ? batch[i] : 0, grid[3 * i], grid[3 * i + 1], grid[3 * i + 2]);
  const unsigned mask = (1u << log2cap) - 1u;
  unsigned s = slot_of(key, log2cap);
  while (true) {
    const unsigned long long prev = atomicCAS(&keys[s], EMPTY, key);
    if (prev == EMPTY || prev == key) {
      atomicMin(&vals[s], i);
      return;
    }
    s = (s + 1) & mask;
  }
}

__global__ void subm_query_kernel(int n, const int* __restrict__ grid, const int* __restrict__ batch,
                                  const unsigned long long* __restrict__ keys, const int* __restrict__ vals,
                                  int log2cap, int* __restrict__ nbr, unsigned* __restrict__ mask_out,
                                  unsigned long long* __restrict__ mask_keys) {
  const long long q = (long long)blockIdx.x * blockDim.x + threadIdx.x;
  if (q >= 27ll * n) return;
  const int i = (int)(q / 27), k = (int)(q - 27ll * i);
  const int x = grid[3 * i] + k / 9 - 1, y = grid[3 * i + 1] + (k / 3) % 3 - 1, z = grid[3 * i + 2] + k % 3 - 1;
  const unsigned cmask = (1u << log2cap) - 1u;
  int out = -1;
  if (x >= 0 && y >= 0 && z >= 0) {
    const unsigned long long key = pack(batch ? batch[i] : 0, x, y, z);
    unsigned s = slot_of(key, log2cap);
    while (true) {
      const unsigned long long kk = keys[s];
      if (kk == key) {
        out = vals[s];
        break;
      }
      if (kk == EMPTY) break;
      s = (s + 1) & cmask;
    }
  }
  nbr[q] = out;
  if (out >= 0) {
    if (mask_out) atomicOr(&mask_out[i], 1u << k);
    if (mask_keys) atomicOr(&mask_keys[i], 1ull << k);
  }
}

__global__ void subm_permute_kernel(int n, const int* __restrict__ perm, const int* __restrict__ nbr,
                                    const unsigned* __restrict__ mask, int* __restrict__ nbr_sorted,
                                    unsigned* __restrict__ mask_sorted) {
  const long long t = (long long)blockIdx.x * blockDim.x + threadIdx.x;
  if (t >= 27ll * n) return;
  const int p = (int)(t / 27), k = (int)(t - 27ll * p);
  const int src = perm[p];
  nbr_sorted[t] = nbr[27ll * src + k];
  if (k == 0) mask_sorted[p] = mask[src];
}

__global__ void subm_pair_flags_kernel(int n, const int* __restrict__ nbr, int* __restrict__ flags, int with_centre) {
  const long long t = (long long)blockIdx.x * blockDim.x + threadIdx.x;
  if (t >= 27ll * n) return;
  const int k = (int)(t / n), i = (int)(t - (long long)k * n);
  flags[t] = ((k != 13 || with_centre) && nbr[27ll * i + k] >= 0) ? 1 : 0;
}

__global__ void subm_pair_fill_kernel(int n, const int* __restrict__ nbr, const int* __restrict__ flags,
                                      const int* __restrict__ pos, int* __restrict__ pair_in,
                                      int* __restrict__ pair_out, int* __restrict__ pair_off) {
  const long long t = (long long)blockIdx.x * blockDim.x + threadIdx.x;
  if (t >= 27ll * n) return;
  const int k = (int)(t / n), i = (int)(t - (long long)k * n);
  if (i == 0) pair_off[k] = pos[t];
  if (flags[t]) {
    const int p = pos[t];
    pair_out[p] = i;
    pair_in[p] = nbr[27ll * i + k];
  }
}

__global__ void subm_pair_pos_kernel(long long num_pairs, const int* __restrict__ pair_out,
                                     const int* __restrict__ pair_off, int* __restrict__ pair_pos) {
  const long long p = (long long)blockIdx.x * blockDim.x + threadIdx.x;
  if (p >= num_pairs) return;
  int k = 0;
#pragma unroll 1
  for (int q = 1; q < 27; ++q)
    if (pair_off[q] <= p) k = q;
  pair_pos[27ll * pair_out[p] + k] = (int)p;
}

__device__ __forceinline__ bool pair_flag(const int* row, int k, bool in, int with_centre) {
  return in && (k != 13 || with_centre) && row[k] >= 0;
}
__global__ void __launch_bounds__(256) subm_pair_count_kernel(int n, const int* __restrict__ nbr,
                                                              int* __restrict__ counts, int nb, int with_centre) {
  __shared__ int wc[27][4];
  const int i = blockIdx.x * 256 + threadIdx.x, lane = threadIdx.x & 63, wid = threadIdx.x >> 6;
  const bool in = i < n;
  const int* row = nbr + 27ll * (in ? i : 0);
#pragma unroll
  for (int k = 0; k < 27; ++k) {
    const unsigned long long bal = __ballot(pair_flag(row, k, in, with_centre));
    if (lane == 0) wc[k][wid] = __popcll(bal);
  }
  __syncthreads();
  if (threadIdx.x < 27) {
    const int k = threadIdx.x;
    counts[(long long)k * nb + blockIdx.x] = wc[k][0] + wc[k][1] + wc[k][2] + wc[k][3];
  }
}
__global__ void __launch_bounds__(256) subm_pair_write_kernel(int n, const int* __restrict__ nbr,
                                                              const int* __restrict__ first, int nb, int with_centre,
                                                              int* __restrict__ pair_in, int* __restrict__ pair_out,
                                                              int* __restrict__ pair_off, int* __restrict__ pair_pos,
                                                              int* __restrict__ pair_cpos) {
  __shared__ int wc[27][4];
  const int i = blockIdx.x * 256 + threadIdx.x, lane = threadIdx.x & 63, wid = threadIdx.x >> 6;
  const bool in = i < n;
  const int* row = nbr + 27ll * (in ? i : 0);
  unsigned long long bal[27];
#pragma unroll
  for (int k = 0; k < 27; ++k) {
    bal[k] = __ballot(pair_flag(row, k, in, with_centre));
    if (lane == 0) wc[k][wid] = __popcll(bal[k]);
  }
  __syncthreads();
  if (blockIdx.x == 0 && threadIdx.x < 27) pair_off[threadIdx.x] = first[(long long)threadIdx.x * nb];
  int pk[27], rank[27], cnt = 0;
#pragma unroll
  for (int k = 0; k < 27; ++k) {
    int base = first[(long long)k * nb + blockIdx.x];
    for (int w = 0; w < wid; ++w) base += wc[k][w];
    const unsigned lrank = __builtin_amdgcn_mbcnt_hi((unsigned)(bal[k] >> 32),
                                                     __builtin_amdgcn_mbcnt_lo((unsigned)bal[k], 0u));
    const bool fl = (bal[k] >> lane) & 1ull;
    const int p = base + (int)lrank;
    if (fl) {
      pair_out[p] = i;
      pair_in[p] = row[k];
    }
    if (pair_pos && in) pair_pos[27ll * i + k] = fl ? p : -1;
    pk[k] = fl ? p : -1;
    rank[k] = cnt;
    cnt += fl ? 1 : 0;
  }
  if (pair_cpos && in) {
    int c[32];
#pragma unroll
    for (int q = 0; q < 31; ++q) c[q] = -1;
#pragma unroll
    for (int k = 0; k < 27; ++k)
#pragma unroll
      for (int q = 0; q <= k; ++q) c[q] = (pk[k] >= 0 && rank[k] == q) ? pk[k] : c[q];
    c[31] = cnt;
    int4* dst = reinterpret_cast<int4*>(pair_cpos + 32ll * i);
#pragma unroll
    for (int q = 0; q < 8; ++q) dst[q] = make_int4(c[4 * q], c[4 * q + 1], c[4 * q + 2], c[4 * q + 3]);
  }
}
}

extern "C" {

int sfx_subm_table_log2(int n) {
  int l = 4;
  while ((1ll << l) < 2ll * (n > 0 ? n : 1)) ++l;
  return l;
}

int sfx_subm_neighbors(int n, const int* grid_coord, const int* batch, int log2cap, unsigned long long* table_keys,
                       int* table_vals, int* nbr, unsigned* mask, unsigned long long* mask_keys, void* stream) {
  SFX_REQUIRE(n >= 0, "sfx_subm_neighbors: n < 0");
  SFX_REQUIRE(log2cap >= 4 && log2cap <= 31 && (1ll << log2cap) >= 2ll * n, "sfx_subm_neighbors: table too small");
  if (n == 0) return SFX_OK;
  SFX_REQUIRE(grid_coord && table_keys && table_vals && nbr, "sfx_subm_neighbors: null buffer");
  hipStream_t st = sfx::as_stream(stream);
  const size_t cap = (size_t)1 << log2cap;
  subm_init_kernel<<<sfx::ceil_div((long long)cap, 256), 256, 0, st>>>((long long)cap, n, table_keys, table_vals, mask,
                                                                       mask_keys);
  subm_insert_kernel<<<sfx::ceil_div(n, 256), 256, 0, st>>>(n, grid_coord, batch, table_keys, table_vals, log2cap);
  subm_query_kernel<<<sfx::ceil_div(27ll * n, 256), 256, 0, st>>>(n, grid_coord, batch, table_keys, table_vals,
                                                                  log2cap, nbr, mask, mask_keys);
  return sfx::check_launch("sfx_subm_neighbors");
}

size_t sfx_subm_pairs_workspace_bytes(int n) {
  const long long e = 27ll * (n > 0 ? n : 1);
  return (size_t)(2 * e * sizeof(int) + 256) + sfx_scan_workspace_bytes(e);
}

int sfx_subm_pairs(int n, const int* nbr, void* ws, size_t ws_bytes, int* pair_in, int* pair_out, int* pair_off,
                   int with_centre, void* stream) {
  SFX_REQUIRE(n >= 0, "sfx_subm_pairs: n < 0");
  SFX_REQUIRE(ws_bytes >= sfx_subm_pairs_workspace_bytes(n), "sfx_subm_pairs: workspace too small");
  SFX_REQUIRE(pair_off, "sfx_subm_pairs: null pair_off");
  hipStream_t st = sfx::as_stream(stream);
  if (n == 0) {
    hipMemsetAsync(pair_off, 0, 28 * sizeof(int), st);
    return sfx::check_launch("sfx_subm_pairs");
  }
  SFX_REQUIRE(nbr && ws && pair_in && pair_out, "sfx_subm_pairs: null buffer");
  const long long e = 27ll * n;
  int* flags = reinterpret_cast<int*>(ws);
  int* pos = flags + e;
  char* scan_ws = reinterpret_cast<char*>(pos + e);
  scan_ws += (256 - (reinterpret_cast<uintptr_t>(scan_ws) & 255)) & 255;
  subm_pair_flags_kernel<<<sfx::ceil_div(e, 256), 256, 0, st>>>(n, nbr, flags, with_centre);
  int rc = sfx_scan_i32(e, flags, pos, 0, scan_ws, sfx_scan_workspace_bytes(e), pair_off + 27, stream);
  if (rc) return rc;
  subm_pair_fill_kernel<<<sfx::ceil_div(e, 256), 256, 0, st>>>(n, nbr, flags, pos, pair_in, pair_out, pair_off);
  return sfx::check_launch("sfx_subm_pairs");
}

size_t sfx_subm_pair_lists_workspace_bytes(int n) {
  const long long e = 27ll * sfx::ceil_div(n > 0 ? n : 1, 256);
  return (size_t)(2 * e * sizeof(int) + 256) + sfx_scan_workspace_bytes(e);
}
int sfx_subm_pair_lists(int n, const int* nbr, void* ws, size_t ws_bytes, int* pair_in, int* pair_out, int* pair_off,
                        int* pair_pos, int* pair_cpos, int with_centre, void* stream) {
  SFX_REQUIRE(n >= 0, "sfx_subm_pair_lists: n < 0");
  SFX_REQUIRE(ws_bytes >= sfx_subm_pair_lists_workspace_bytes(n), "sfx_subm_pair_lists: workspace too small");
  SFX_REQUIRE(pair_off, "sfx_subm_pair_lists: null pair_off");
  hipStream_t st = sfx::as_stream(stream);
  if (n == 0) {
    hipMemsetAsync(pair_off, 0, 28 * sizeof(int), st);
    return sfx::check_launch("sfx_subm_pair_lists");
  }
  SFX_REQUIRE(nbr && ws && pair_in && pair_out, "sfx_subm_pair_lists: null buffer");
  const int nb = (int)sfx::ceil_div(n, 256);
  const long long e = 27ll * nb;
  int* counts = reinterpret_cast<int*>(ws);
  int* first = counts + e;
  char* scan_ws = reinterpret_cast<char*>(first + e);
  scan_ws += (256 - (reinterpret_cast<uintptr_t>(scan_ws) & 255)) & 255;
  subm_pair_count_kernel<<<nb, 256, 0, st>>>(n, nbr, counts, nb, with_centre);
  const int rc = sfx_scan_i32(e, counts, first, 0, scan_ws, sfx_scan_workspace_bytes(e), pair_off + 27, stream);
  if (rc) return rc;
  subm_pair_write_kernel<<<nb, 256, 0, st>>>(n, nbr, first, nb, with_centre, pair_in, pair_out, pair_off, pair_pos,
                                             pair_cpos);
  return sfx::check_launch("sfx_subm_pair_lists");
}
int sfx_subm_pair_pos(int n, long long num_pairs, const int* pair_out, const int* pair_off, int* pair_pos,
                      void* stream) {
  SFX_REQUIRE(n >= 0 && num_pairs >= 0 && num_pairs <= 26ll * n, "sfx_subm_pair_pos: bad sizes");
  if (n == 0) return SFX_OK;
  SFX_REQUIRE(pair_pos && (num_pairs == 0 || (pair_out && pair_off)), "sfx_subm_pair_pos: null buffer");
  hipStream_t st = sfx::as_stream(stream);
  hipMemsetAsync(pair_pos, 0xff, 27ll * n * sizeof(int), st);
  if (num_pairs > 0)
    subm_pair_pos_kernel<<<sfx::ceil_div(num_pairs, 256), 256, 0, st>>>(num_pairs, pair_out, pair_off, pair_pos);
  return sfx::check_launch("sfx_subm_pair_pos");
}

int sfx_subm_permute(int n, const int* perm, const int* nbr, const unsigned* mask, int* nbr_sorted,
                     unsigned* mask_sorted, void* stream) {
  SFX_REQUIRE(n >= 0, "sfx_subm_permute: n < 0");
  if (n == 0) return SFX_OK;
  SFX_REQUIRE(perm && nbr && mask && nbr_sorted && mask_sorted, "sfx_subm_permute: null buffer");
  subm_permute_kernel<<<sfx::ceil_div(27ll * n, 256), 256, 0, sfx::as_stream(stream)>>>(n, perm, nbr, mask,
                                                                                        nbr_sorted, mask_sorted);
  return sfx::check_launch("sfx_subm_permute");
}

}
```

### splatformer_amd/ptv3.py

```python
from __future__ import annotations

import math
import os
from typing import Dict, List, Optional, Sequence

import torch
import torch.nn as nn
from torch import Tensor

from . import _lib
from . import ptv3_ops as ops

ORDERS = ("z", "z-trans", "hilbert", "hilbert-trans")
POOL_COUNTS_UPFRONT = os.environ.get("SFX_POOL_COUNTS_UPFRONT", "1") != "0"


NBR_EARLY = os.environ.get("SFX_NBR_EARLY", "1") != "0"

class Point(dict):

    def __getattr__(self, k):
        try:
            return self[k]
        except KeyError as e:
            raise AttributeError(k) from e

    def __setattr__(self, k, v):
        self[k] = v


class SubMConv3d(nn.Module):

    def __init__(self, in_channels, out_channels, kernel_size=3, bias=True, indice_key=None):
        super().__init__()
        assert kernel_size == 3
        self.in_channels, self.out_channels, self.indice_key = in_channels, out_channels, indice_key
        self.weight = nn.Parameter(torch.empty(out_channels, 3, 3, 3, in_channels))
        self.bias = nn.Parameter(torch.empty(out_channels)) if bias else None
        fan_in = in_channels * 27
        bound = 1.0 / math.sqrt(fan_in)
        nn.init.uniform_(self.weight, -math.sqrt(3.0) * bound, math.sqrt(3.0) * bound)
        if self.bias is not None:
            nn.init.uniform_(self.bias, -bound, bound)


class PointSequential(nn.Sequential):
    pass


class MLP(nn.Module):
    def __init__(self, in_channels, hidden_channels, out_channels):
        super().__init__()
        self.fc1 = nn.Linear(in_channels, hidden_channels)
        self.act = nn.GELU()
        self.fc2 = nn.Linear(hidden_channels, out_channels)
        self.drop = nn.Dropout(0.0)


class SerializedAttention(nn.Module):
    def __init__(self, channels, num_heads, patch_size, order_index=0, enable_flash=False):
        super().__init__()
        assert channels % num_heads == 0
        self.channels, self.num_heads = channels, num_heads
        self.enable_flash = enable_flash
        self.scale = (channels // num_heads) ** -0.5
        self.order_index = order_index
        self.patch_size_max = patch_size
        self.qkv = nn.Linear(channels, channels * 3, bias=True)
        self.proj = nn.Linear(channels, channels)
        self.attn_drop = nn.Dropout(0.0)
        self.proj_drop = nn.Dropout(0.0)
        self.softmax = nn.Softmax(dim=-1)


class Block(nn.Module):
    def __init__(self, channels, num_heads, patch_size=128, mlp_ratio=4.0, order_index=0, cpe_indice_key=None,
                 enable_flash=False):
        super().__init__()
        self.channels = channels
        self.pre_norm = True
        self.cpe = PointSequential(SubMConv3d(channels, channels, 3, True, cpe_indice_key),
                                   nn.Linear(channels, channels), nn.LayerNorm(channels))
        self.norm1 = PointSequential(nn.LayerNorm(channels))
        self.attn = SerializedAttention(channels, num_heads, patch_size, order_index, enable_flash)
        self.norm2 = PointSequential(nn.LayerNorm(channels))
        self.mlp = PointSequential(MLP(channels, int(channels * mlp_ratio), channels))
        self.drop_path = PointSequential(nn.Identity())
        self.drop_prob = 0.0

    def cpe_fused(self):
        conv, lin = self.cpe[0], self.cpe[1]
        ts = (conv.weight, conv.bias, lin.weight, lin.bias)
        key = tuple((t.data_ptr(), t._version) for t in ts)
        cache = self.__dict__.get("_sfx_cpe")
        if cache is not None and cache[0] == key:
            return cache[1], cache[2]
        from .train_ops import transpose
        with torch.no_grad():
            C = self.channels
            wc = conv.weight.detach().reshape(C, -1)
            wf = ops.linear(lin.weight.detach(), transpose(wc))
            bf = ops.linear(conv.bias.detach()[None].contiguous(), lin.weight.detach(), lin.bias.detach())[0]
        self.__dict__["_sfx_cpe"] = (key, wf.contiguous(), bf.contiguous())
        return wf, bf

    def cpe_packed(self):
        wf, bf = self.cpe_fused()
        key = self.__dict__["_sfx_cpe"][0]
        cache = self.__dict__.get("_sfx_cpe_pk")
        if cache is None or cache[0] != key:
            with torch.no_grad():
                wpk, winv = ops.subm_cpe_pack(wf)
            cache = (key, wpk, winv)
            self.__dict__["_sfx_cpe_pk"] = cache
        return cache[1], cache[2], bf

    def run(self, point: Point, conv_in: Optional[Tensor] = None, out: Optional[Tensor] = None) -> Point:
        x = point.feat
        C = self.channels
        ln_c = self.cpe[2]
        ln1 = self.norm1[0]
        xc = x if conv_in is None else conv_in
        fused = ops.subm_fused_ok(C, x.shape[0])
        if fused:
            wpk, winv, bf = self.cpe_packed()
            re = point.get("feat_rowexp")
            x1, h = ops.subm_cpe_ln(xc, x, point.nbr, wpk, winv, bf, ln_c.weight, ln_c.bias, ln1.weight, ln1.bias,
                                    ln1.eps, rowexp=re[1] if re is not None and re[0] is xc else None)
        else:
            wf, bf = self.cpe_fused()
            t = ops.subm_conv(xc, point.nbr, wf, bf, partials=ops.subm_partials_ok(xc, point.nbr, C))
            if ops.cpe_ln_qkv_ok(t, C, self.attn.qkv.weight):
                x1, qkv, q_amax = ops.cpe_ln_qkv(t, x, ln_c.weight, ln_c.bias, ln1.weight, ln1.bias, ln1.eps,
                                                 self.attn.qkv)
                h = None
            else:
                x1, h = ops.cpe_residual_ln(t, x, ln_c.weight, ln_c.bias, ln1.weight, ln1.bias, ln1.eps)
        oi = point.order_type[self.attn.order_index]
        if h is not None:
            qkv, q_amax = ops.linear(h, self.attn.qkv.weight, self.attn.qkv.bias, y_amax=True)
        if self.attn.enable_flash:
            K, win3, nw = point_windows_flash(point, self.attn.patch_size_max)
            a = ops.window_attention_varlen(qkv, point.order_phys[oi], win3, nw, K, self.attn.num_heads, C,
                                            qkv_amax=q_amax)
        else:
            K, win, nw = point_windows(point, self.attn.patch_size_max)
            if ops.window_attention_proj_ok(C, self.attn.num_heads):
                x2 = ops.window_attention_proj(qkv, point.order_phys[oi], win, nw, K, self.attn.num_heads, C,
                                               self.attn.proj, x1, q_amax)
                return self._mlp_tail(point, x2, out, rowexp=fused)
            a = ops.window_attention(qkv, point.order_phys[oi], win, nw, K, self.attn.num_heads, C, qkv_amax=q_amax)
        x2 = ops.linear(a, self.attn.proj.weight, self.attn.proj.bias, residual=x1)
        return self._mlp_tail(point, x2, out, rowexp=fused)

    def _mlp_tail(self, point: Point, x2: Tensor, out: Optional[Tensor], rowexp: bool = False) -> Point:
        ln2 = self.norm2[0]
        mlp = self.mlp[0]
        point.pop("feat_rowexp", None)
        if ops.block_mlp_ok(x2, self.channels):
            e = torch.empty(x2.shape[0], device=x2.device, dtype=torch.int32) if rowexp else None
            point.feat = ops.block_mlp(x2, ln2, mlp.fc1, mlp.fc2, out=out, rowexp=e)
            if e is not None:
                point.feat_rowexp = (point.feat, e)
            return point
        h2 = ops.layernorm(x2, ln2.weight, ln2.bias, ln2.eps)
        m = ops.linear(h2, mlp.fc1.weight, mlp.fc1.bias, act=ops.ACT_GELU)
        point.feat = ops.linear(m, mlp.fc2.weight, mlp.fc2.bias, residual=x2, out=out)
        return point


def bn_affine(bn: nn.BatchNorm1d):
    ts = (bn.weight, bn.bias, bn.running_mean, bn.running_var)
    key = tuple((t.data_ptr(), t._version) for t in ts) + (bn.eps,)
    cache = getattr(bn, "_sfx_affine", None)
    if cache is not None and cache[0] == key:
        return cache[1]
    with torch.no_grad():
        scale = bn.weight / torch.sqrt(bn.running_var + bn.eps)
        shift = bn.bias - bn.running_mean * scale
    val = (scale.detach().contiguous(), shift.detach().contiguous())
    object.__setattr__(bn, "_sfx_affine", (key, val))
    return val


class SerializedPooling(nn.Module):
    def __init__(self, in_channels, out_channels, stride=2, norm_layer=None, act_layer=None):
        super().__init__()
        assert stride == 2 ** (math.ceil(stride) - 1).bit_length()
        self.stride = stride
        self.proj = nn.Linear(in_channels, out_channels)
        self.norm = PointSequential(norm_layer(out_channels))
        self.act = PointSequential(act_layer())

    def pooling_depth(self, depth: int) -> int:
        pd = (math.ceil(self.stride) - 1).bit_length()
        return 0 if pd > depth else pd

    def _pd(self, point: Point) -> int:
        return self.pooling_depth(point.serialized_depth)

    def geometry_begin(self, point: Point):
        return ops.pool_geometry_begin(point.codes_phys, point.order_phys, self._pd(point))

    def geometry_end(self, point: Point, perm: Sequence[int], state, m: Optional[int] = None,
                     deferred: Optional[list] = None, pairs: bool = True, centre: bool = False):
        pd = self._pd(point)
        depth = point.serialized_depth - pd
        code_bits = point.code_bits - 3 * pd
        sidx, cluster, idx_ptr, m, codes, order, inverse, grid, batch = ops.pool_geometry_end(
            state, point.codes_phys, point.order_phys, point.order_type[0], pd, point.grid_coord, point.get("batch"),
            point.code_bits, m=m, deferred=deferred)
        coord = ops.segment_mean(point.coord, idx_ptr, sidx, m)
        new = Point(coord=coord, grid_coord=grid, codes_phys=codes, order_phys=order,
                    inverse_phys=inverse, order_type=[point.order_type[p] for p in perm],
                    serialized_depth=depth, code_bits=code_bits, pooling_inverse=cluster, pooling_parent=point)
        if batch is not None:
            new.batch = batch
            new.offset = torch.cumsum(torch.bincount(batch.long().cpu(), minlength=len(point.offset)), 0).tolist()
        else:
            new.offset = [m]
        new.nbr = ops.subm_neighbors(grid, new.get("batch"), with_pairs=pairs, centre=centre)
        return new, sidx, idx_ptr, m

    def geometry(self, point: Point, perm: Sequence[int]):
        return self.geometry_end(point, perm, self.geometry_begin(point))

    def run(self, point: Point, perm: Sequence[int], m: Optional[int] = None, deferred: Optional[list] = None,
            pairs: bool = True, centre: bool = False) -> Point:
        st = self.geometry_begin(point)
        pf = ops.linear(point.feat, self.proj.weight, self.proj.bias)
        new, sidx, idx_ptr, m = self.geometry_end(point, perm, st, m, deferred, pairs=pairs, centre=centre)
        sc, sh = bn_affine(self.norm[0])
        new.feat = ops.segment_max_affine_act(pf, idx_ptr, sidx, m, sc, sh, ops.ACT_GELU)
        return new


class SerializedUnpooling(nn.Module):
    def __init__(self, in_channels, skip_channels, out_channels, norm_layer=None, act_layer=None):
        super().__init__()
        self.proj = PointSequential(nn.Linear(in_channels, out_channels), norm_layer(out_channels), act_layer())
        self.proj_skip = PointSequential(nn.Linear(skip_channels, out_channels), norm_layer(out_channels),
                                         act_layer())

    def run(self, point: Point) -> Point:
        parent = point.pop("pooling_parent")
        inverse = point.pop("pooling_inverse")
        sc, sh = bn_affine(self.proj[1])
        coarse = ops.linear(point.feat, self.proj[0].weight, self.proj[0].bias, scale=sc, shift=sh, act=ops.ACT_GELU)
        sc2, sh2 = bn_affine(self.proj_skip[1])
        skip = torch.empty(parent.feat.shape[0], coarse.shape[1], device=coarse.device)
        parent.feat = ops.linear(
            parent.feat, self.proj_skip[0].weight, self.proj_skip[0].bias, scale=sc2, shift=sh2, act=ops.ACT_GELU,
            residual=coarse, residual_idx=inverse, pre_out=skip)
        parent.stale_conv_feat = skip
        return parent


def point_windows(point: Point, patch_size_max: int):
    counts = [b - a for a, b in zip([0] + list(point.offset[:-1]), point.offset)]
    K = min(min(counts), patch_size_max)
    key = ("win", K)
    if key not in point:
        t = torch.from_numpy(ops.window_table_np(point.offset, K)).pin_memory()
        point[key] = (t.to(point.feat.device, non_blocking=True), t.shape[0])
    win, nw = point[key]
    return K, win, nw


def point_windows_flash(point: Point, patch_size_max: int):
    K = patch_size_max
    key = ("winv", K)
    if key not in point:
        t = torch.from_numpy(ops.window_table_varlen_np(point.offset, K)).pin_memory()
        point[key] = (t.to(point.feat.device, non_blocking=True), t.shape[0])
    win3, nw = point[key]
    return K, win3, nw


class _Container(nn.Module):
    def add(self, module, name):
        self.add_module(name, module)


class PointTransformerV3(nn.Module):
    def __init__(self, in_channels=6, order=ORDERS, stride=(2, 2, 2, 2), enc_depths=(2, 2, 2, 6, 2),
                 enc_channels=(32, 64, 128, 256, 512), enc_num_head=(2, 4, 8, 16, 32),
                 enc_patch_size=(48, 48, 48, 48, 48), dec_depths=(2, 2, 2, 2), dec_channels=(64, 64, 128, 256),
                 dec_num_head=(4, 4, 8, 16), dec_patch_size=(48, 48, 48, 48), mlp_ratio=4, turn_off_bn=False,
                 shuffle_orders=True, embedding_type="MLP", drop_path=0.3, enable_flash=False):
        super().__init__()
        if turn_off_bn:
            raise NotImplementedError("turn_off_bn=True is not on the SplatFormer path (ptv3_base.gin:30)")
        if embedding_type != "MLP":
            raise NotImplementedError("only embedding_type='MLP' (ptv3_base.gin:32) is on the path")
        self.num_stages = len(enc_depths)
        self.order = [order] if isinstance(order, str) else list(order)
        self.shuffle_orders = shuffle_orders
        self.enc_channels, self.dec_channels = list(enc_channels), list(dec_channels)
        assert self.num_stages == len(stride) + 1 == len(enc_channels) == len(enc_num_head)
        bn_layer = lambda c: nn.BatchNorm1d(c, eps=1e-3, momentum=0.01)
        self.embedding = PointSequential(nn.Linear(in_channels, enc_channels[0]), bn_layer(enc_channels[0]),
                                         nn.GELU())
        self.enc = _Container()
        for s in range(self.num_stages):
            enc = _Container()
            if s > 0:
                enc.add(SerializedPooling(enc_channels[s - 1], enc_channels[s], stride[s - 1], bn_layer, nn.GELU),
                        "down")
            for i in range(enc_depths[s]):
                enc.add(Block(enc_channels[s], enc_num_head[s], enc_patch_size[s], mlp_ratio, i % len(self.order),
                              f"stage{s}", enable_flash), f"block{i}")
            self.enc.add(enc, f"enc{s}")
        enc_dp = torch.linspace(0, drop_path, sum(enc_depths)).tolist()
        for s in range(self.num_stages):
            stage = getattr(self.enc, f"enc{s}")
            for i in range(enc_depths[s]):
                getattr(stage, f"block{i}").drop_prob = enc_dp[sum(enc_depths[:s]) + i]
        self.dec = _Container()
        dch = list(dec_channels) + [enc_channels[-1]]
        for s in reversed(range(self.num_stages - 1)):
            dec = _Container()
            dec.add(SerializedUnpooling(dch[s + 1], enc_channels[s], dch[s], bn_layer, nn.GELU), "up")
            for i in range(dec_depths[s]):
                dec.add(Block(dch[s], dec_num_head[s], dec_patch_size[s], mlp_ratio, i % len(self.order),
                              f"stage{s}", enable_flash), f"block{i}")
            self.dec.add(dec, f"dec{s}")
        dec_dp = torch.linspace(0, drop_path, sum(dec_depths)).tolist()
        for s in range(self.num_stages - 1):
            sl = dec_dp[sum(dec_depths[:s]):sum(dec_depths[:s + 1])][::-1]
            stage = getattr(self.dec, f"dec{s}")
            for i in range(dec_depths[s]):
                getattr(stage, f"block{i}").drop_prob = sl[i]
        self.last_perms: List[List[int]] = []

    def _draw_perm(self, perms_override, k):
        if perms_override is not None:
            p = list(perms_override[k])
        elif self.shuffle_orders:
            p = torch.randperm(len(self.order)).tolist()
        else:
            p = list(range(len(self.order)))
        self.last_perms.append(p)
        return p

    def stage_needs_pairs(self, s: int, n: Optional[int] = None) -> bool:
        chans = [self.enc_channels[s]] + ([self.dec_channels[s]] if s < len(self.dec_channels) else [])
        return not all(ops.subm_fused_ok(c, n) for c in chans)

    def prepare(self, data_dict, perms: Optional[List[Sequence[int]]] = None, pairs: bool = True,
                reorder: bool = False, centre_pairs: bool = False) -> Point:
        feat = data_dict["feat"]
        _lib.require_gpu(feat)
        dev = feat.device
        offset = data_dict["offset"]
        offset = offset.tolist() if isinstance(offset, Tensor) else list(offset)
        grid = data_dict["grid_coord"]
        grid = grid if grid.dtype == torch.int32 else grid.int()
        grid = grid.contiguous()
        n = feat.shape[0]
        B = len(offset)
        batch = None
        if B > 1:
            batch = torch.empty(n, device=dev, dtype=torch.int32)
            offs = torch.tensor(offset, dtype=torch.int64, device=dev)
            _lib.call("sfx_offsets_to_batch", n, B, offs.data_ptr(), batch.data_ptr(), _lib.stream())
        nbr = None if (reorder or not NBR_EARLY) else ops.subm_neighbors(grid, batch, with_pairs=pairs,
                                                                          centre=centre_pairs)
        d = data_dict.get("serialized_depth")
        if isinstance(d, _lib.HostRead):
            depth = int(d.get()[0]).bit_length()
        else:
            depth = int(d) if d is not None else int(grid.max().item()).bit_length()
        assert depth * 3 + len(offset).bit_length() <= 63 and depth <= 16
        code_bits = 3 * depth + max(0, (B - 1).bit_length())
        self.last_perms = []
        codes, order, inverse = ops.serialize(grid, batch, depth, code_bits, self.order)
        p0 = self._draw_perm(perms, 0)
        coord = data_dict["coord"].float().contiguous()
        perm = None
        if reorder and batch is None:
            perm = order[0]
            codes, order, inverse, grid, coord = ops.serialize_permute(codes, order, inverse, grid, coord)
        point = Point(coord=coord, grid_coord=grid, offset=offset, codes_phys=codes,
                      order_phys=order, inverse_phys=inverse, order_type=p0, serialized_depth=depth,
                      code_bits=code_bits)
        if perm is not None:
            point.perm = perm
        if batch is not None:
            point.batch = batch
        point.nbr = nbr if nbr is not None else ops.subm_neighbors(grid, batch, with_pairs=pairs, centre=centre_pairs)
        return point

    @torch.no_grad()
    def forward(self, data_dict, perms: Optional[List[Sequence[int]]] = None, out: Optional[Tensor] = None,
                reorder: bool = False) -> Point:
        feat = data_dict["feat"]
        _lib.require_gpu(feat)
        emb, bnm = self.embedding[0], self.embedding[1]
        sc, sh = bn_affine(bnm)
        if ops.point_embed_ok(feat, emb.weight):
            emb_feat = ops.point_embed(feat, emb.weight, emb.bias, sc, sh)
        else:
            emb_feat = ops.linear(feat, emb.weight, emb.bias, scale=sc, shift=sh, act=ops.ACT_GELU)
        cp = ops.SUBM_CENTRE_PAIRS
        point = self.prepare(data_dict, perms, pairs=self.stage_needs_pairs(0, feat.shape[0]), reorder=reorder,
                             centre_pairs=cp)
        perm = point.get("perm")
        point.feat = emb_feat if perm is None else ops.move_rows(emb_feat, perm)
        final_out = out
        if perm is not None:
            out = None
        pools = [getattr(self.enc, f"enc{s}").down for s in range(1, self.num_stages)]
        shifts, depth, cum = [], point.serialized_depth, 0
        for mod in pools:
            pd = mod.pooling_depth(depth)
            depth, cum = depth - pd, cum + pd
            shifts.append(3 * cum)
        counts_rd = ops.pool_counts_begin(point.codes_phys, point.order_phys, shifts) if POOL_COUNTS_UPFRONT else None
        self.check_deferred(wait=True)
        self._forward_id = self.__dict__.get("_forward_id", 0) + 1
        deferred: list = []
        k = 1
        for s in range(self.num_stages):
            stage = getattr(self.enc, f"enc{s}")
            for name, mod in stage.named_children():
                if name == "down":
                    m = counts_rd.get()[k - 1] if counts_rd is not None else None
                    point = mod.run(point, self._draw_perm(perms, k), m=m, deferred=deferred,
                                    pairs=self.stage_needs_pairs(s, m), centre=cp)
                    k += 1
                else:
                    point = mod.run(point)
        dec_names = [f"dec{s}" for s in reversed(range(self.num_stages - 1))]
        for di, dn in enumerate(dec_names):
            stage = getattr(self.dec, dn)
            children = list(stage.named_children())
            for ci, (name, mod) in enumerate(children):
                if name == "up":
                    point = mod.run(point)
                else:
                    conv_in = point.pop("stale_conv_feat", None)
                    last = di == len(dec_names) - 1 and ci == len(children) - 1
                    point = mod.run(point, conv_in=conv_in, out=out if last else None)
        fid = self._forward_id
        self._deferred = self.__dict__.get("_deferred", []) + [(rd, m, fid, i + 1) for i, (rd, m) in
                                                                enumerate(deferred)]
        self.check_deferred(wait=False)
        if perm is not None and final_out is not None:
            ops.move_rows(point.feat, perm, dst=final_out, scatter=True)
        return point

    def check_deferred(self, wait: bool = True) -> None:
        pending, errors = [], []
        for rd, m, fid, k in self.__dict__.get("_deferred", []):
            if not (wait or rd.ready()):
                pending.append((rd, m, fid, k))
                continue
            try:
                ops.check_pool_runs(rd.get(), m)
            except RuntimeError as e:
                errors.append(f"forward {fid}, pooling {k}: {e}")
        self._deferred = pending
        if errors:
            raise RuntimeError("; ".join(errors))


class PointTransformerV3Model(nn.Module):

    def __init__(self, in_channels, enable_flash=False, enc_dim=64, output_dim=96, turn_off_bn=False,
                 stride=(1, 2, 2, 2), embedding_type="MLP", enc_depths=(2, 2, 2, 6, 2), enc_num_head=(2, 4, 8, 16, 32),
                 dec_depths=(2, 2, 2, 2), dec_num_head=(4, 4, 8, 16), dec_channels=None, enc_channels=None,
                 pdnorm_bn=False, pdnorm_ln=False, pretrained_ckpt=None, additional_info=None):
        super().__init__()
        if pdnorm_bn or pdnorm_ln:
            raise NotImplementedError("PDNorm is not on the SplatFormer path")
        if additional_info and additional_info.get("tome") not in (None, "base") or \
                (additional_info and float(additional_info.get("r", 0.0)) != 0.0):
            raise NotImplementedError("token merging variants are out of scope (SURVEY.md §2); base r=0 only")
        if dec_channels is None:
            dec_channels = {64: (64, 64, 128, 256), 128: (128, 128, 256, 256), 96: (96, 96, 128, 256)}.get(output_dim)
            if dec_channels is None:
                raise ValueError("Unsupported output_dim")
        if enc_channels is None:
            enc_channels = {32: (32, 64, 128, 256, 512), 64: (64, 96, 128, 256, 512)}.get(enc_dim)
            if enc_channels is None:
                raise ValueError("Unsupported enc_dim")
        self.dec_channels = tuple(dec_channels)
        patch = 1024 if enable_flash else 128
        self.backbone = PointTransformerV3(
            in_channels=in_channels, order=ORDERS, stride=stride, enc_depths=enc_depths, enc_channels=enc_channels,
            enc_num_head=enc_num_head, enc_patch_size=(patch,) * len(enc_channels), dec_depths=dec_depths,
            dec_channels=dec_channels, dec_num_head=dec_num_head, dec_patch_size=(patch,) * len(dec_channels),
            mlp_ratio=4, turn_off_bn=turn_off_bn, shuffle_orders=True, embedding_type=embedding_type,
            enable_flash=enable_flash)
        self.enable_flash = enable_flash
        self.output_dim = self.dec_channels[0]
        if pretrained_ckpt is not None:
            sd = torch.load(pretrained_ckpt, map_location="cpu", weights_only=True)["state_dict"]
            sd = {k.replace("module.backbone.", ""): v for k, v in sd.items() if "backbone." in k}
            own = self.backbone.state_dict()
            load = {k: v for k, v in sd.items() if k in own and own[k].shape == v.shape}
            self.backbone.load_state_dict(load, strict=False)

    def forward(self, x, perms=None, out=None, reorder=False):
        return self.backbone(x, perms=perms, out=out, reorder=reorder)
```

### splatformer_amd/ptv3_ops.py

```python
from __future__ import annotations

import contextlib
import ctypes
import os
from typing import List, Optional, Sequence, Tuple

import numpy as np
import torch
from torch import Tensor

from . import _lib
from ._lib import call, ptr, stream

ACT_NONE, ACT_GELU, ACT_RELU, ACT_TANH = 0, 1, 2, 3
GEMM_NUM_CONFIGS = 7


def gemm_force_config(cfg: int = -1, stream_k: int = -1) -> None:
    call("sfx_gemm_force_config", cfg, stream_k)


def gemm_force_epilogue(cls: int = -1) -> None:
    call("sfx_gemm_force_epilogue", cls)

# ... 185 lines not shown
    px, ldx = _rows(x)
    y = torch.empty(M, out_dim, device=x.device, dtype=torch.float32)
    oc = (ctypes.c_int * len(ocols))(*ocols)
    call("sfx_heads", M, len(ocols) - 1, kin, out_dim, px, ldx, res_off, n_tanh, oc, ptr(st), ptr(pr), ptr(y),
         stream())
    return y


def grouped_linear(x: Tensor, weight: Tensor, bias: Tensor, groups: int, *, act: int = ACT_NONE,
                   out: Optional[Tensor] = None, a_amax: Optional[Tuple[int, int]] = None,
                   w_amax: Optional[Tuple[int, int]] = None, y_amax: bool = False):
    G, N, K = weight.shape
    M = x.shape[0]
    if out is None:
        out = torch.empty(M, G * N, device=x.device, dtype=torch.float32)
    pa, lda = _rows(x)
    py, ldy = _rows(out)
    ys = new_amax(out.device) if y_amax else None
    call("sfx_linear", M, N, K, pa, lda, None, 1, ptr(weight), K, ptr(bias), None, None, act, -1, None, 0, None, py,
         ldy, None, 0, G, K, N * K, N, N, None, None, 0, *_slot_args(a_amax), *_slot_args(w_amax),
         *_slot_args(ys), *weight_split(weight, G * N), stream())
    return (out, ys) if y_amax else out


MLP_FUSED = os.environ.get("SFX_MLP_FUSED", "1") != "0"
MLP_CHANNELS = (64, 96, 128, 256)
MLP_FUSED_CHANNELS = tuple(int(c) for c in os.environ.get("SFX_MLP_CHANNELS", "64,96,128,256").split(",") if c)


def mlp_pack(ln2, fc1, fc2) -> Tuple[Tensor, Tensor]:
    ts = (ln2.weight, ln2.bias, fc1.weight, fc1.bias, fc2.weight, fc2.bias)
    key = tuple((t.data_ptr(), t._version) for t in ts)
    c = fc1.__dict__.get("_sfx_mlp")
    if c is not None and c[0] == key:
        return c[1], c[2]
    C = fc1.weight.shape[1]
    dev = fc1.weight.device
    st = torch.empty(int(_lib.fn("sfx_mlp_stream_floats")(C)), device=dev, dtype=torch.float32)
    pr = torch.empty(int(_lib.fn("sfx_mlp_params_floats")(C)), device=dev, dtype=torch.float32)
    ws = torch.empty(9 * C, device=dev, dtype=torch.int32)
    w = [t.detach().contiguous() for t in ts]
    call("sfx_mlp_pack", C, ptr(w[2]), ptr(w[3]), ptr(w[4]), ptr(w[5]), ptr(w[0]), ptr(w[1]), ptr(st), ptr(pr),
         ptr(ws), stream())
    fc1.__dict__["_sfx_mlp"] = (key, st, pr, w)
    return st, pr


def block_mlp_ok(x: Tensor, C: int) -> bool:
    return MLP_FUSED and C in MLP_FUSED_CHANNELS and C in MLP_CHANNELS and x.dim() == 2 and x.stride(1) == 1 and x.data_ptr() % 16 == 0 \
        and x.stride(0) % 4 == 0


def block_mlp(x2: Tensor, ln2, fc1, fc2, out: Optional[Tensor] = None, rowexp: Optional[Tensor] = None) -> Tensor:
    M, C = x2.shape
    st, pr = mlp_pack(ln2, fc1, fc2)
    if out is None:
        out = torch.empty(M, C, device=x2.device, dtype=torch.float32)
    px, ldx = _rows(x2)
    py, ldy = _rows(out)
    call("sfx_block_mlp", M, C, px, ldx, ptr(st), ptr(pr), float(ln2.eps), py, ldy, ptr(rowexp, torch.int32), stream())
    return out


def block_mlp_last_plan() -> dict:
    import ctypes
    v = [ctypes.c_int(0) for _ in range(5)]
    call("sfx_block_mlp_last_plan", *[ctypes.addressof(c) for c in v])
    return dict(zip(("kind", "split", "main_wgs", "tail_wgs", "pts"), (c.value for c in v)))


def block_mlp_train(x2: Tensor, ln2, fc1, fc2, z: Tensor, rowscale: Optional[Tensor] = None,
                    out: Optional[Tensor] = None) -> Tensor:
    M, C = x2.shape
    if z.shape != (M, 4 * C) or not z.is_contiguous():
        raise ValueError("block_mlp_train: z must be a contiguous [M, 4C] tensor")
    st, pr = mlp_pack(ln2, fc1, fc2)
    if out is None:
        out = torch.empty(M, C, device=x2.device, dtype=torch.float32)
    px, ldx = _rows(x2)
    py, ldy = _rows(out)
    call("sfx_block_mlp_train", M, C, px, ldx, ptr(st), ptr(pr), float(ln2.eps), ptr(rowscale), ptr(z), py, ldy,
         stream())
    return out


def mlp_bwd_pack(ln2, fc1, fc2) -> Tuple[Tensor, Tensor]:
    ts = (fc1.weight, fc2.weight)
    key = tuple((t.data_ptr(), t._version) for t in ts)
    c = fc2.__dict__.get("_sfx_mlp_bwd")
    if c is not None and c[0] == key:
        return c[1], c[2]
    C = fc1.weight.shape[1]
    dev = fc1.weight.device
    st = torch.empty(int(_lib.fn("sfx_mlp_stream_floats")(C)), device=dev, dtype=torch.float32)
    pr = torch.empty(int(_lib.fn("sfx_mlp_params_floats")(C)), device=dev, dtype=torch.float32)
    ws = torch.empty(9 * C, device=dev, dtype=torch.int32)
    w1t = fc2.weight.detach().t().contiguous()
    w2t = fc1.weight.detach().t().contiguous()
    z4, z1 = torch.zeros(4 * C, device=dev), torch.zeros(C, device=dev)
    one = torch.ones(C, device=dev)
    call("sfx_mlp_pack", C, ptr(w1t), ptr(z4), ptr(w2t), ptr(z1), ptr(one), ptr(z1), ptr(st), ptr(pr), ptr(ws),
         stream())
    fc2.__dict__["_sfx_mlp_bwd"] = (key, st, pr, (w1t, w2t, z4, z1, one))
    return st, pr


def block_mlp_bwd(dy: Tensor, ln2, fc1, fc2, z: Tensor, rowscale: Optional[Tensor] = None,
                  out: Optional[Tensor] = None) -> Tensor:
    M, C = dy.shape
    if z.shape != (M, 4 * C) or not z.is_contiguous():
        raise ValueError("block_mlp_bwd: z must be a contiguous [M, 4C] tensor")
    st, pr = mlp_bwd_pack(ln2, fc1, fc2)
    if out is None:
        out = torch.empty(M, C, device=dy.device, dtype=torch.float32)
    pd, ldd = _rows(dy)
    po, ldo = _rows(out)
    call("sfx_block_mlp_bwd", M, C, pd, ldd, ptr(st), ptr(pr), ptr(rowscale), ptr(z), po, ldo, stream())
    return out


def layernorm(x: Tensor, gamma: Tensor, beta: Tensor, eps: float, out: Optional[Tensor] = None) -> Tensor:
    M, C = x.shape
    if out is None:
        out = torch.empty(M, C, device=x.device, dtype=torch.float32)
    px, ldx = _rows(x)
    py, ldy = _rows(out)
    call("sfx_layernorm", M, C, px, ldx, ptr(gamma), ptr(beta), float(eps), py, ldy, stream())
    return out


def cpe_residual_ln(t, x: Tensor, g_cpe: Tensor, b_cpe: Tensor, g1: Tensor, b1: Tensor, eps: float,
                    x_out: Optional[Tensor] = None) -> Tuple[Tensor, Tensor]:
    M, C = x.shape
    x_out = torch.empty_like(x) if x_out is None else x_out
    h = torch.empty_like(x)
    if isinstance(t, SubmPartials):
        if t.cpos is not None:
            call("sfx_cpe_residual_ln_cpairs", M, C, ptr(t.centre), t.ldt, ptr(t.partials), ptr(t.cpos), t.num_pairs,
                 ptr(x), ptr(g_cpe), ptr(b_cpe), ptr(g1), ptr(b1), float(eps), ptr(x_out), ptr(h), stream())
        else:
            call("sfx_cpe_residual_ln_pairs", M, C, ptr(t.centre), t.ldt, ptr(t.partials), ptr(t.pair_pos),
                 t.num_pairs, ptr(x), ptr(g_cpe), ptr(b_cpe), ptr(g1), ptr(b1), float(eps), ptr(x_out), ptr(h), stream())
    else:
        call("sfx_cpe_residual_ln", M, C, ptr(t), ptr(x), ptr(g_cpe), ptr(b_cpe), ptr(g1), ptr(b1), float(eps),
             ptr(x_out), ptr(h), stream())
    return x_out, h


LN_QKV = os.environ.get("SFX_LN_QKV", "0") == "1"
LN_QKV_CHANNELS = (64, 96, 128)


def cpe_ln_qkv_ok(t, C: int, qkv_weight: Tensor) -> bool:
    return (LN_QKV and isinstance(t, SubmPartials) and C in LN_QKV_CHANNELS and get_precision() == "fp32"
            and weight_split(qkv_weight)[0] is not None)


def cpe_ln_qkv(t: "SubmPartials", x: Tensor, g_cpe: Tensor, b_cpe: Tensor, g1: Tensor, b1: Tensor, eps: float,
               qkv: "torch.nn.Linear") -> Tuple[Tensor, Tensor, Tuple[int, int]]:
    M, C = x.shape
    x_out = torch.empty_like(x)
    out = torch.empty(M, 3 * C, device=x.device, dtype=torch.float32)
    wsp, winv = weight_split(qkv.weight)
    ys = new_amax(x.device)
    call("sfx_cpe_ln_qkv_pairs", M, C, ptr(t.centre), t.ldt, ptr(t.partials), ptr(t.pair_pos), t.num_pairs, ptr(x),
         ptr(g_cpe), ptr(b_cpe), ptr(g1), ptr(b1), float(eps), ptr(x_out), wsp, winv, ptr(qkv.bias), ptr(out),
         ys[0], ys[1], stream())
    return x_out, out, ys


def window_table(offsets: Sequence[int], K: int) -> List[Tuple[int, int]]:
    tab = []
    start = 0
    for end in offsets:
        n = end - start
        nw = (n + K - 1) // K
        for w in range(nw):
            ks = start + w * K
            qs = ks
            if ks + K > end:
                ks = end - K
            tab.append((ks, qs))
        start = end
    return tab


def window_table_np(offsets: Sequence[int], K: int) -> np.ndarray:
    parts = []
    start = 0
    for end in offsets:
        n = end - start
        nw = (n + K - 1) // K
        qs = start + K * np.arange(nw, dtype=np.int64)
        ks = np.minimum(qs, end - K)
        parts.append(np.stack([ks, qs], 1))
        start = end
    tab = np.concatenate(parts) if parts else np.zeros((0, 2), np.int64)
    return np.ascontiguousarray(tab, dtype=np.int32)


def window_table_varlen_np(offsets: Sequence[int], K: int) -> np.ndarray:
    parts = []
    start = 0
    for end in offsets:
        n = end - start
        if 0 < n <= K:
            parts.append(np.array([[start, start, n]], np.int64))
        elif n > K:
            qs = start + K * np.arange((n + K - 1) // K, dtype=np.int64)
            ks = np.minimum(qs, end - K)
            parts.append(np.stack([ks, qs, np.full_like(qs, K)], 1))
        start = end
    tab = np.concatenate(parts) if parts else np.zeros((0, 3), np.int64)
    return np.ascontiguousarray(tab, dtype=np.int32)


def window_attention_varlen(qkv: Tensor, order: Tensor, win3: Tensor, num_windows: int, K: int, heads: int,
                            channels: int, out: Optional[Tensor] = None,
                            qkv_amax: Optional[Tuple[int, int]] = None) -> Tensor:
    n = qkv.shape[0]
    d = channels // heads
    if qkv.shape != (n, 3 * channels) or order.shape[0] != n or tuple(win3.shape) != (num_windows, 3):
        raise ValueError(f"window_attention_varlen: shapes qkv {tuple(qkv.shape)} order {tuple(order.shape)} "
                         f"win3 {tuple(win3.shape)} for C={channels}, {num_windows} windows")
    if out is None:
        out = torch.empty(n, channels, device=qkv.device, dtype=torch.float32)
    call("sfx_window_attention_varlen", num_windows, K, heads, d, channels, ptr(qkv), ptr(order, torch.int32),
         ptr(win3, torch.int32), float(d ** -0.5), ptr(out), *_slot_args(qkv_amax), stream())
    return out


def window_attention(qkv: Tensor, order: Tensor, win: Tensor, num_windows: int, K: int, heads: int, channels: int,
                     out: Optional[Tensor] = None, qkv_amax: Optional[Tuple[int, int]] = None) -> Tensor:
    n = qkv.shape[0]
    d = channels // heads
    if out is None:
        out = torch.empty(n, channels, device=qkv.device, dtype=torch.float32)
    call("sfx_window_attention", num_windows, K, heads, d, channels, ptr(qkv), ptr(order, torch.int32),
         ptr(win, torch.int32), float(d ** -0.5), ptr(out), *_slot_args(qkv_amax), stream())
    return out


_ATTN_PROJ_MODE = os.environ.get("SFX_ATTN_PROJ", "1")
_ATTN_PROJ_SHAPES = {(64, 32), (96, 24), (128, 16), (256, 16)}
_ATTN_PROJ_DEFAULT = {(64, 32), (96, 24)}


def window_attention_proj_ok(channels: int, heads: int) -> bool:
    if _ATTN_PROJ_MODE == "0":
        return False
    shapes = _ATTN_PROJ_SHAPES if _ATTN_PROJ_MODE == "all" else _ATTN_PROJ_DEFAULT
    return (channels, channels // heads) in shapes and get_precision() == "fp32"


def window_attention_proj(qkv: Tensor, order: Tensor, win: Tensor, num_windows: int, K: int, heads: int,
                          channels: int, proj: "torch.nn.Linear", x1: Tensor, qkv_amax: Tuple[int, int],
                          out: Optional[Tensor] = None) -> Tensor:
    n = qkv.shape[0]
    d = channels // heads
    if qkv.shape != (n, 3 * channels) or order.shape[0] != n or x1.shape != (n, channels):
        raise ValueError(f"window_attention_proj: shapes qkv {tuple(qkv.shape)} order {tuple(order.shape)} "
                         f"x1 {tuple(x1.shape)} for C={channels}")
    wsp, winv = weight_split(proj.weight)
    if wsp is None:
        raise RuntimeError("window_attention_proj: the projection weight has no fp16x2 pre-split")
    if out is None:
        out = torch.empty(n, channels, device=qkv.device, dtype=torch.float32)
    px, ldx = _rows(x1)
    po, ldo = _rows(out)
    call("sfx_window_attention_proj", num_windows, K, heads, d, channels, ptr(qkv), ptr(order, torch.int32),
         ptr(win, torch.int32), float(d ** -0.5), *qkv_amax, wsp, winv, ptr(proj.bias), px, ldx, po, ldo, stream())
    return out


def _sort(keys: Tensor, vals: Optional[Tensor], begin: int, end: int) -> Tuple[Tensor, Tensor]:
    n = keys.shape[0]
    ko = torch.empty_like(keys)
    vo = torch.empty(n, device=keys.device, dtype=torch.int32)
    ws = _lib.workspace(_lib.fn("sfx_sort_workspace_bytes")(n), keys.device)
    call("sfx_sort_pairs_u64", n, ptr(keys), ptr(vals), ptr(ko), ptr(vo), begin, end, ptr(ws), ws.numel(), stream())
    return ko, vo


def _finalize(keys: Tensor, n: int, R: int, code_bits: int) -> Tuple[Tensor, Tensor]:
    _, pos = _sort(keys, None, 0, code_bits + 2)
    order = torch.empty(R, n, device=keys.device, dtype=torch.int32)
    inverse = torch.empty(R, n, device=keys.device, dtype=torch.int32)
    call("sfx_serialize_finalize", n, R, ptr(pos), ptr(order), ptr(inverse), stream())
    return order, inverse


def serialize(grid_coord: Tensor, batch: Optional[Tensor], depth: int, code_bits: int,
              orders: Sequence[str]) -> Tuple[Tensor, Tensor, Tensor]:
    n = grid_coord.shape[0]
    R = len(orders)
    t = [ORDER_TYPES[o] for o in orders] + [0] * (4 - R)
    codes = torch.empty(R, n, device=grid_coord.device, dtype=torch.int64)
    keys = torch.empty(R * n, device=grid_coord.device, dtype=torch.int64)
    call("sfx_serialize_keys", n, ptr(grid_coord, torch.int32), ptr(batch), depth, R, t[0], t[1], t[2], t[3],
         code_bits, ptr(codes), ptr(keys), stream())
    order, inverse = _finalize(keys, n, R, code_bits)
    return codes, order, inverse


def serialize_permute(codes: Tensor, order: Tensor, inverse: Tensor, grid: Tensor, coord: Tensor):
    R, n = codes.shape
    cp, op, ip = torch.empty_like(codes), torch.empty_like(order), torch.empty_like(inverse)
# ... 3 lines not shown
         ptr(grid, torch.int32), ptr(coord, torch.float32), ptr(cp), ptr(op), ptr(ip), ptr(gp), ptr(xp), stream())
    return cp, op, ip, gp, xp


def scan_i32(x: Tensor, inclusive: bool = True, total: Optional[Tensor] = None) -> Tuple[Tensor, Tensor]:
    n = x.shape[0]
    out = torch.empty_like(x)
    if total is None:
        total = torch.empty(1, device=x.device, dtype=torch.int32)
    ws = _lib.workspace(_lib.fn("sfx_scan_workspace_bytes")(n), x.device)
    call("sfx_scan_i32", n, ptr(x), ptr(out), 1 if inclusive else 0, ptr(ws), ws.numel(), ptr(total), stream())
    return out, total


def pool_geometry_begin(codes: Tensor, order: Tensor, pooling_depth: int):
    R, n = codes.shape
    flags = torch.empty(R * n, device=codes.device, dtype=torch.int32)
    call("sfx_pool_run_flags", n, R, ptr(order, torch.int32), ptr(codes, torch.int64), 3 * pooling_depth,
         ptr(flags), stream())
    pos, _ = scan_i32(flags)
    return flags, pos, _lib.HostRead(pos.view(R, n)[:, -1])


def pool_counts_begin(codes: Tensor, order: Tensor, shifts: Sequence[int]) -> "_lib.HostRead":
    n = codes.shape[1]
    counts = torch.empty(max(len(shifts), 1), device=codes.device, dtype=torch.int32)
    for k in range(0, len(shifts), 8):
        sh = list(shifts[k:k + 8])
        call("sfx_pool_run_counts", n, ptr(order[0], torch.int32), ptr(codes[0], torch.int64),
             ctypes.cast((ctypes.c_int * len(sh))(*sh), ctypes.c_void_p), len(sh), counts[k:].data_ptr(), stream())
    return _lib.HostRead(counts)


def check_pool_runs(ends: Sequence[int], m: int) -> None:
    runs = [ends[0]] + [ends[r] - ends[r - 1] for r in range(1, len(ends))]
    if any(c != m for c in runs):
        raise RuntimeError(f"sfx pooling: order rows count cluster runs {runs}, expected {m}; the serialization codes "
                           "are not hierarchical (code >> 3 must be the parent cell's code)")


def pool_geometry_end(state, codes: Tensor, order: Tensor, row0: int, pooling_depth: int, grid_coord: Tensor,
                      batch: Optional[Tensor], code_bits: int, m: Optional[int] = None,
                      deferred: Optional[list] = None):
    flags, pos, ends_rd = state
    R, n = codes.shape
    dev = codes.device
    shift = 3 * pooling_depth
    if m is None:
        ends = ends_rd.get()
        m = ends[0]
        check_pool_runs(ends, m)
    else:
        deferred.append((ends_rd, m))
    cluster = torch.empty(n, device=dev, dtype=torch.int32)
    sidx = torch.empty(n, device=dev, dtype=torch.int32)
    idx_ptr = torch.empty(m + 1, device=dev, dtype=torch.int32)
    head = torch.empty(m, device=dev, dtype=torch.int32)
    call("sfx_pool_assign_runs", n, m, row0, ptr(order), ptr(pos), ptr(flags), ptr(cluster), ptr(idx_ptr),
         ptr(head), ptr(sidx), stream())
    new_order = torch.empty(R, m, device=dev, dtype=torch.int32)
    new_inverse = torch.empty(R, m, device=dev, dtype=torch.int32)
    call("sfx_pool_reorder", n, m, R, ptr(order), ptr(pos), ptr(flags), ptr(cluster), ptr(new_order),
         ptr(new_inverse), stream())
    new_codes = torch.empty(R, m, device=dev, dtype=torch.int64)
    new_grid = torch.empty(m, 3, device=dev, dtype=torch.int32)
    new_batch = torch.empty(m, device=dev, dtype=torch.int32) if batch is not None else None
    call("sfx_pool_gather", m, n, R, ptr(head), ptr(codes), pooling_depth, ptr(grid_coord), ptr(batch),
         code_bits - shift, ptr(new_codes), None, ptr(new_grid), ptr(new_batch), stream())
    return sidx, cluster, idx_ptr, m, new_codes, new_order, new_inverse, new_grid, new_batch


def pool_geometry(codes: Tensor, order: Tensor, row0: int, pooling_depth: int, grid_coord: Tensor,
                  batch: Optional[Tensor], code_bits: int):
    st = pool_geometry_begin(codes, order, pooling_depth)
    return pool_geometry_end(st, codes, order, row0, pooling_depth, grid_coord, batch, code_bits)


def segment_max_affine_act(x: Tensor, idx_ptr: Tensor, sorted_idx: Tensor, m: int, scale: Optional[Tensor],
                           shift: Optional[Tensor], act: int) -> Tensor:
    C = x.shape[1]
    out = torch.empty(m, C, device=x.device, dtype=torch.float32)
    call("sfx_segment_max_affine_act", m, C, ptr(idx_ptr), ptr(sorted_idx), ptr(x), ptr(scale), ptr(shift), act,
         ptr(out), stream())
    return out


def segment_mean(x: Tensor, idx_ptr: Tensor, sorted_idx: Tensor, m: int) -> Tensor:
    D = x.shape[1]
    out = torch.empty(m, D, device=x.device, dtype=torch.float32)
    call("sfx_segment_mean", m, D, ptr(idx_ptr), ptr(sorted_idx), ptr(x.contiguous()), ptr(out), stream())
    return out


PAIR_LISTS = os.environ.get("SFX_PAIR_LISTS", "1") != "0"
LN_COMPACT = os.environ.get("SFX_LN_COMPACT", "1") != "0"


class PairLists:

    def __init__(self, nbr: Tensor, centre: bool):
        n = nbr.shape[0]
        dev = nbr.device
        cap = max(1, (27 if centre else 26) * n)
        self.centre = centre
        self.pair_in = torch.empty(cap, device=dev, dtype=torch.int32)
        self.pair_out = torch.empty(cap, device=dev, dtype=torch.int32)
        self.off_dev = torch.empty(28, device=dev, dtype=torch.int32)
        if PAIR_LISTS:
            self.cpos = torch.empty(max(1, n), 32, device=dev, dtype=torch.int32) if LN_COMPACT else None
            self._pos = None if LN_COMPACT else torch.empty(max(1, n), 27, device=dev, dtype=torch.int32)
            ws = _lib.workspace(_lib.fn("sfx_subm_pair_lists_workspace_bytes")(n), dev)
            call("sfx_subm_pair_lists", n, ptr(nbr), ptr(ws), ws.numel(), ptr(self.pair_in), ptr(self.pair_out),
                 ptr(self.off_dev), ptr(self._pos), ptr(self.cpos), 1 if centre else 0, stream())
        else:
            self._pos = None
            self.cpos = None
            ws = _lib.workspace(_lib.fn("sfx_subm_pairs_workspace_bytes")(n), dev)
            call("sfx_subm_pairs", n, ptr(nbr), ptr(ws), ws.numel(), ptr(self.pair_in), ptr(self.pair_out),
                 ptr(self.off_dev), 1 if centre else 0, stream())
        self._rd = _lib.HostRead(self.off_dev)
        self._n = n
        self._off = None
        self._off_c = None

    def off_ready(self) -> bool:
        return self._off is not None

    @property
    def pair_off(self) -> List[int]:
        if self._off is None:
            self._off = self._rd.get()
        return self._off

    @property
    def off_host(self):
        if self._off_c is None:
            self._off_c = (ctypes.c_int * 28)(*self.pair_off)
        return self._off_c

    @property
    def num_pairs(self) -> int:
        return self.pair_off[27]

    @property
    def pair_pos(self) -> Tensor:
        if self._pos is None:
            pos = torch.empty(self._n, 27, device=self.pair_in.device, dtype=torch.int32)
            call("sfx_subm_pair_pos", self._n, self.num_pairs, ptr(self.pair_out), ptr(self.off_dev), ptr(pos),
                 stream())
            self._pos = pos
        return self._pos


class SubmMap:

    def __init__(self, nbr: Tensor, mask: Optional[Tensor], centre_pref: bool = False):
        self.nbr, self.mask = nbr, mask
        self.centre_pref = centre_pref
        self._lists = {}
        self._order = None

    def lists(self, centre: bool = False) -> PairLists:
        pl = self._lists.get(centre)
        if pl is None:
            pl = self._lists[centre] = PairLists(self.nbr, centre)
        return pl

    def ensure_pairs(self) -> "SubmMap":
        self.lists(False)
        return self

    @property
    def pair_in(self) -> Tensor:
        return self.lists(False).pair_in

    @property
    def pair_out(self) -> Tensor:
        return self.lists(False).pair_out

    @property
    def pair_pos(self) -> Tensor:
        return self.lists(False).pair_pos

    @property
    def order(self) -> Tensor:
        if self._order is None:
            n = self.nbr.shape[0]
            keys = torch.empty(n, device=self.nbr.device, dtype=torch.int64)
            call("sfx_subm_order_keys", n, ptr(self.nbr), ptr(keys), stream())
            _, self._order = _sort(keys, None, 0, 16)
        return self._order

    def pair_off_ready(self) -> bool:
        return self.lists(False).off_ready()

    @property
    def pair_off(self) -> List[int]:
        return self.lists(False).pair_off

    @property
    def _off_host(self):
        return self.lists(False).off_host

    @property
    def shape(self):
        return self.nbr.shape

    @property
    def num_pairs(self) -> int:
        return self.lists(False).num_pairs


SUBM_MASK = os.environ.get("SFX_SUBM_MASK", "0") == "1"


def subm_neighbors(grid_coord: Tensor, batch: Optional[Tensor], with_pairs: bool = True, centre: bool = False):
    n = grid_coord.shape[0]
    dev = grid_coord.device
    l2 = _lib.fn("sfx_subm_table_log2")(n)
    tk = torch.empty(1 << l2, device=dev, dtype=torch.int64)
    tv = torch.empty(1 << l2, device=dev, dtype=torch.int32)
    nbr = torch.empty(n, 27, device=dev, dtype=torch.int32)
    mask = torch.empty(n, device=dev, dtype=torch.int32) if SUBM_MASK else None
    call("sfx_subm_neighbors", n, ptr(grid_coord, torch.int32), ptr(batch), l2, ptr(tk), ptr(tv), ptr(nbr), ptr(mask),
         None, stream())
    smap = SubmMap(nbr, mask, centre_pref=centre)
    if with_pairs:
        smap.lists(centre)
    return smap


SUBM_PARTIALS = os.environ.get("SFX_SUBM_ATOMIC", "0") != "1"
SUBM_CENTRE_PAIRS = os.environ.get("SFX_SUBM_CENTRE_PAIRS", "1") != "0"
SUBM_CENTRE_FIRST = os.environ.get("SFX_SUBM_CENTRE_FIRST", "1") != "0"
PAIRS_LN_CHANNELS = (64, 96, 128, 256, 512)


def subm_partials_ok(x: Tensor, smap: "SubmMap", cout: int) -> bool:
    return (SUBM_PARTIALS and cout in PAIRS_LN_CHANNELS and x.shape[1] == cout and x.is_contiguous()
            and x.data_ptr() % 16 == 0 and (27 * smap.nbr.shape[0] * cout * 4 + 64 < 0x7ffffff0
                                            or smap.lists(smap.centre_pref).num_pairs * cout * 4 + 64 < 0x7ffffff0))


SUBM_FUSED_MODE = os.environ.get("SFX_SUBM_FUSED", "auto")
SUBM_FUSED_MIN_ROWS = int(os.environ.get("SFX_SUBM_FUSED_MIN_ROWS", "120000"))
SUBM_FUSED_AUTO_MAX_C = 128
SUBM_FUSED_KERNELS = (64, 96, 128, 256)
SUBM_FUSED_CHANNELS = tuple(int(c) for c in os.environ.get("SFX_SUBM_FUSED_CHANNELS", "64,96,128,256").split(",")
                            if c and int(c) in SUBM_FUSED_KERNELS)


def subm_fused_ok(C: int, n: Optional[int] = None) -> bool:
    if SUBM_FUSED_MODE == "0" or C not in SUBM_FUSED_CHANNELS:
        return False
    if SUBM_FUSED_MODE == "1":
        return True
    return n is not None and n >= SUBM_FUSED_MIN_ROWS and C <= SUBM_FUSED_AUTO_MAX_C


def subm_cpe_pack(wf: Tensor) -> Tuple[Tensor, Tensor]:
    C = wf.shape[0]
    nb = int(_lib.fn("sfx_subm_cpe_pack_bytes")(C))
    if nb == 0 or wf.shape[1] != 27 * C:
        raise RuntimeError(f"subm_cpe_pack: no fused conv for C={C}")
    wpk = torch.empty(nb // 4, device=wf.device, dtype=torch.float32)
    winv = torch.empty(C, device=wf.device, dtype=torch.float32)
    ws = torch.empty(C, device=wf.device, dtype=torch.float32)
    call("sfx_subm_cpe_pack", C, ptr(wf.contiguous()), ptr(wpk), ptr(winv), ptr(ws), stream())
    return wpk, winv


def subm_rowexp(x: Tensor) -> Tensor:
    n, C = x.shape
    e = torch.empty(n, device=x.device, dtype=torch.int32)
    call("sfx_subm_rowexp", n, C, ptr(x), ptr(e), stream())
    return e


def subm_cpe_ln(xc: Tensor, x: Tensor, smap: "SubmMap", wpk: Tensor, winv: Tensor, bias: Tensor, g_cpe: Tensor,
                b_cpe: Tensor, g1: Tensor, b1: Tensor, eps: float,
                rowexp: Optional[Tensor] = None) -> Tuple[Tensor, Tensor]:
    n, C = x.shape
    if xc.shape != x.shape or not (xc.is_contiguous() and x.is_contiguous()):
        raise RuntimeError("subm_cpe_ln: contiguous [n, C] inputs expected")
    x1 = torch.empty_like(x)
    h = torch.empty_like(x)
    call("sfx_subm_cpe_ln", n, C, ptr(xc), ptr(x), ptr(smap.nbr), ptr(smap.order),
         ptr(subm_rowexp(xc) if rowexp is None else rowexp), ptr(wpk),
         ptr(winv), ptr(bias), ptr(g_cpe), ptr(b_cpe), ptr(g1), ptr(b1), float(eps), ptr(x1), ptr(h), stream())
    return x1, h


_ZERO_OFFS = (ctypes.c_int * 28)()


class SubmPartials:

    def __init__(self, centre: Tensor, partials: Tensor, pair_pos, num_pairs: int, ldt: Optional[int] = None,
                 cpos: Optional[Tensor] = None):
        self.centre, self.partials, self._pair_pos, self.num_pairs = centre, partials, pair_pos, num_pairs
        self.ldt = centre.shape[-1] if ldt is None else ldt
        self.cpos = cpos

    @property
    def pair_pos(self) -> Tensor:
        return self._pair_pos.pair_pos if isinstance(self._pair_pos, PairLists) else self._pair_pos

    def total(self) -> Tensor:
        n = self.pair_pos.shape[0]
        out = self.centre.expand(n, -1).clone() if self.ldt == 0 else self.centre.clone()
        pos = self.pair_pos.long()
        for k in range(27):
            sel = pos[:, k] >= 0
            if bool(sel.any()):
                out[sel] += self.partials[pos[sel, k]]
        return out


def subm_conv(x: Tensor, smap: "SubmMap", weight: Tensor, bias: Optional[Tensor],
              out: Optional[Tensor] = None, x_amax: Optional[Tuple[int, int]] = None,
              w_amax: Optional[Tuple[int, int]] = None, partials: bool = False):
    n, cin = x.shape
    cout = weight.shape[0]
    if out is None:
        out = torch.empty(n, cout, device=x.device, dtype=torch.float32)
    px, ldx = _rows(x)
    po, ldo = _rows(out)
    if partials:
        wsp = weight_split(weight)
        if smap.centre_pref and SUBM_CENTRE_PAIRS:
            pl = smap.lists(True)
            npairs = pl.num_pairs
            part = torch.empty(max(1, npairs), cout, device=x.device, dtype=torch.float32)
            call("sfx_subm_conv_partials_pairs", n, cin, cout, px, ldx, ptr(smap.nbr), ptr(weight), ptr(bias),
                 ptr(pl.pair_in), ptr(pl.pair_out), pl.off_host, po, ldo, ptr(part), cout, *wsp, stream())
            b = bias if bias is not None else torch.zeros(cout, device=x.device, dtype=torch.float32)
            return SubmPartials(b.contiguous(), part, pl, npairs, ldt=0, cpos=pl.cpos)
        if SUBM_CENTRE_FIRST and not smap.pair_off_ready():
            call("sfx_subm_conv_partials", n, cin, cout, px, ldx, ptr(smap.nbr), ptr(weight), ptr(bias), None, None,
                 _ZERO_OFFS, po, ldo, None, cout, *wsp, stream())
            npairs = smap.num_pairs
            part = torch.empty(max(1, npairs), cout, device=x.device, dtype=torch.float32)
            call("sfx_subm_conv_partials_pairs", n, cin, cout, px, ldx, ptr(smap.nbr), ptr(weight), ptr(bias),
                 ptr(smap.pair_in), ptr(smap.pair_out), smap._off_host, po, ldo, ptr(part), cout, *wsp, stream())
            return SubmPartials(out, part, smap.lists(False), npairs, cpos=smap.lists(False).cpos)
        npairs = smap.num_pairs
        part = torch.empty(max(1, npairs), cout, device=x.device, dtype=torch.float32)
        call("sfx_subm_conv_partials", n, cin, cout, px, ldx, ptr(smap.nbr), ptr(weight), ptr(bias),
             ptr(smap.pair_in), ptr(smap.pair_out), smap._off_host, po, ldo, ptr(part), cout, *wsp, stream())
        return SubmPartials(out, part, smap.lists(False), npairs, cpos=smap.lists(False).cpos)
    call("sfx_subm_conv", n, cin, cout, px, ldx, ptr(smap.nbr), ptr(weight), ptr(bias), ptr(smap.pair_in),
         ptr(smap.pair_out), smap._off_host, po, ldo, *_slot_args(x_amax), *_slot_args(w_amax),
         *weight_split(weight), stream())
    return out


def move_rows(src: Tensor, idx: Tensor, dst: Optional[Tensor] = None, scatter: bool = False) -> Tensor:
    s2 = src if src.dim() == 2 else src.reshape(src.shape[0], -1)
    esz = s2.element_size()
    if esz not in (4, 8) or s2.stride(1) != 1:
        raise RuntimeError("move_rows: rows of 4- or 8-byte elements, unit column stride")
    n = idx.shape[0]
    if dst is None:
        if scatter:
            raise RuntimeError("move_rows: scatter needs a destination")
        dst = torch.empty((n,) + tuple(src.shape[1:]), device=src.device, dtype=src.dtype)
    d2 = dst if dst.dim() == 2 else dst.reshape(dst.shape[0], -1)
    words = s2.shape[1] * esz // 4
    call("sfx_move_rows", n, words, s2.data_ptr(), s2.stride(0) * esz // 4, ptr(idx, torch.int32), d2.data_ptr(),
         d2.stride(0) * esz // 4, 1 if scatter else 0, stream())
    return dst


def gs_pack(gs: dict, feat_out: Tensor, grid_resolution: float, grid_out: Optional[Tensor],
            grid_max: Optional[Tensor] = None) -> None:
    n = gs["means"].shape[0]

    def rp(t):
        t2 = t if t.dim() == 2 else t.reshape(t.shape[0], -1)
        if t2.stride(-1) != 1:
            t2 = t2.contiguous()
        return t2.data_ptr(), t2.stride(0), t2

    keep = []
    args = []
    for k in ["means", "scales", "opacities", "quats", "features_dc"]:
        p_, l_, t_ = rp(gs[k])
        keep.append(t_)
        args += [p_, l_]
    rest = gs.get("features_rest")
    if rest is not None:
        p_, l_, t_ = rp(rest if rest.is_contiguous() else rest.contiguous())
        keep.append(t_)
        rd = t_.shape[1]
    else:
        p_, l_, rd = None, 0, 0
    pf, ldf = _rows(feat_out)
    call("sfx_gs_pack", n, *args, p_, l_, rd, float(grid_resolution), pf, ldf, ptr(grid_out), ptr(grid_max),
         stream())
```

Before: 684.9 renders/s.

## Group submanifold conv neighbor triples into fused K=3*Cin GEMM tiles

Adds a grouped submanifold-conv path that buckets each point's 27 neighbors into 9 triples, classified into 54 classes by which of the three neighbors exist. A new MODE_PAIRG GEMM kernel gathers up to three input rows per entry and multiplies by a contiguous K=segs*Cin weight slice, writing one partial per (point, triple) instead of one per pair. The aim is fewer partial rows and larger K per tile for the 128/256/512-channel stages, cutting partial-store traffic and per-pair GEMM overhead. In exchange it adds a group-list build pass, an extra host readback of class offsets, and a new reduction layout that the fused LN/QKV path does not accept.

```diff
diff --git a/include/sfx.h b/include/sfx.h
--- a/include/sfx.h
+++ b/include/sfx.h
@@ -234,6 +234,13 @@
                                  const float* weight, const float* bias, const int* pair_in, const int* pair_out,
                                  const int* pair_off_host, float* out, long long ldo, float* partials, long long ldp,
                                  const float* w_split, const float* w_inv, void* stream);
+size_t sfx_subm_group_lists_workspace_bytes(int n);
+int sfx_subm_group_lists(int n, const int* nbr, void* ws, size_t ws_bytes, int* grp_in, int* grp_out, int* grp_off,
+                         int* grp_cpos, void* stream);
+int sfx_gemm_split_mode(int K);
+int sfx_subm_conv_grouped(int n, int cin, int cout, const float* x, long long ldx, const int* grp_in,
+                          const int* grp_off_host, float* partials, long long ldp, const float* w_split,
+                          const float* w_inv, void* stream);
 
 int sfx_gs_pack(int n, const float* means, long long ld_means, const float* scales, long long ld_scales,
                 const float* opacities, long long ld_opacities, const float* quats, long long ld_quats,
diff --git a/splatformer_amd/csrc/gemm.hip b/splatformer_amd/csrc/gemm.hip
--- a/splatformer_amd/csrc/gemm.hip
+++ b/splatformer_amd/csrc/gemm.hip
@@ -637,6 +637,8 @@
 
 int sfx_gemm_last_epilogue(void) { return last_epi; }
 
+int sfx_gemm_split_mode(int K) { return split_mode(K); }
+
 int sfx_weight_split(int rows, int cols, const float* w, long long ld, float* w_split, float* w_inv, void* stream) {
   SFX_REQUIRE(rows >= 0 && cols > 0 && cols % 4 == 0 && ld >= cols && ld % 4 == 0,
               "sfx_weight_split: bad sizes (cols and ld must be multiples of 4)");
@@ -781,6 +783,44 @@
               "sfx_subm_conv_partials_pairs: null partials / pair lists");
   return subm_conv_impl(n, cin, cout, x, ldx, nbr, weight, bias, pair_in, pair_out, pair_off_host, out, ldo, nullptr,
                         0, nullptr, 0, w_split, w_inv, partials, ldp, stream, true);
+}
+
+int sfx_subm_conv_grouped(int n, int cin, int cout, const float* x, long long ldx, const int* grp_in,
+                          const int* grp_off_host, float* partials, long long ldp, const float* w_split,
+                          const float* w_inv, void* stream) {
+  SFX_REQUIRE(n >= 0 && cin > 0 && cout > 0, "sfx_subm_conv_grouped: bad sizes");
+  SFX_REQUIRE(cin % BK == 0, "sfx_subm_conv_grouped: cin must be a multiple of %d", BK);
+  if (n == 0) return SFX_OK;
+  SFX_REQUIRE(x && grp_off_host && w_split && w_inv, "sfx_subm_conv_grouped: null buffer");
+  const long long total = grp_off_host[kMaxSlices];
+  SFX_REQUIRE(grp_off_host[0] == 0 && total >= 0 && total <= 9ll * n, "sfx_subm_conv_grouped: bad class offsets");
+  for (int c = 0; c < kMaxSlices; ++c)
+    SFX_REQUIRE(grp_off_host[c + 1] >= grp_off_host[c], "sfx_subm_conv_grouped: class offsets decrease");
+  if (total == 0) return SFX_OK;
+  SFX_REQUIRE(grp_in && partials, "sfx_subm_conv_grouped: null lists / partials");
+  SFX_REQUIRE(ldx >= cin && ldx % 4 == 0 && ldp >= cout && aligned16(x) && aligned16(w_split),
+              "sfx_subm_conv_grouped: leading dimensions / 16-byte alignment");
+  SFX_REQUIRE(fits(n, ldx) && fits(cout, 27ll * cin) && fits(total, ldp) && fits(total, 3),
+              "sfx_subm_conv_grouped: operand exceeds the 2 GiB buffer-descriptor range");
+  SFX_REQUIRE(split_mode(cin) == 2 && g_prec == 0,
+              "sfx_subm_conv_grouped: fp16x2 operands only (SFX_GEMM_PREC / reference precision select the pair path)");
+  GemmArgs a{};
+  a.M = (int)total; a.N = cout; a.K = 3 * cin; a.A = x; a.lda = ldx; a.S = 3; a.Kseg = cin; a.gstride = 3;
+  a.W = w_split; a.ldw = 27ll * cin; a.Wsp = w_split; a.ldws = 27ll * cin; a.winv = w_inv;
+  a.act = 0; a.act_ncols = cout; a.Y = partials; a.ldy = ldp;
+  a.pair_mode = 1; a.pair_grouped = 1; a.pair_store = 1; a.pair_in = grp_in; a.pair_out = grp_in;
+  a.slice_w_stride = cin; a.num_slices = kMaxSlices; a.split = 2;
+  for (int c = 0; c <= kMaxSlices; ++c) a.slice_pair_off[c] = grp_off_host[c];
+  for (const TunedLaunch& t : kTunedConv)
+    if (t.N == cout && t.K == cin && 5ll * n >= 4ll * t.M && 4ll * n <= 5ll * t.M) {
+      a.tuned = t.cfg + 1;
+      break;
+    }
+  const int cfg = pick_cfg(a, 1, true);
+  a.sk = 0;
+  a.epi = last_epi = EPI_PAIR_STORE;
+  (kCfgs[cfg].nw == 8 ? launch_m4_w8 : launch_m4_w4)(cfg, a, sfx::as_stream(stream));
+  return sfx::check_launch("sfx_subm_conv_grouped");
 }
 
 int sfx_subm_conv_bwd_data(int n, int cin, int cout, const float* dy, long long ldy, const int* nbr,
diff --git a/splatformer_amd/csrc/gemm_common.h b/splatformer_amd/csrc/gemm_common.h
--- a/splatformer_amd/csrc/gemm_common.h
+++ b/splatformer_amd/csrc/gemm_common.h
@@ -29,6 +29,8 @@
 enum Act { ACT_NONE = 0, ACT_GELU = 1, ACT_RELU = 2, ACT_TANH = 3 };
 enum Epi { EPI_GENERAL = 0, EPI_LIN = 1, EPI_LIN_GELU = 2, EPI_PAIR_STORE = 3 };
 
+constexpr int kMaxSlices = 54;
+
 struct GemmArgs {
   int M, N, K;
   const float* A;
@@ -53,9 +55,10 @@
   int pair_mode;
   const int* pair_in;
   const int* pair_out;
-  int slice_tile_off[28];
-  int slice_pair_off[28];
+  int slice_tile_off[kMaxSlices + 1];
+  int slice_pair_off[kMaxSlices + 1];
   int num_slices;
+  int pair_grouped;
   long long slice_w_stride;
   const float* rowscale;
   int pre_before_act;
@@ -144,7 +147,21 @@
 using sfx::split3;
 using sfx::split2h;
 
-enum Mode { MODE_DENSE = 0, MODE_GATHER1 = 1, MODE_GATHERS = 2, MODE_PAIR = 3 };
+enum Mode { MODE_DENSE = 0, MODE_GATHER1 = 1, MODE_GATHERS = 2, MODE_PAIR = 3, MODE_PAIRG = 4 };
+
+__host__ __device__ inline int grp_class_at(int pos) {
+  if (pos < 9) return 6 * pos + 5;
+  if (pos < 27) return 6 * ((pos - 9) >> 1) + 3 + ((pos - 9) & 1);
+  return 6 * ((pos - 27) / 3) + (pos - 27) % 3;
+}
+__host__ __device__ inline int grp_segs(int cls) {
+  const int q = cls % 6;
+  return q < 3 ? 1 : (q < 5 ? 2 : 3);
+}
+__host__ __device__ inline int grp_first(int cls) {
+  const int q = cls % 6;
+  return 3 * (cls / 6) + (q < 3 ? q : (q == 4 ? 1 : 0));
+}
 
 inline int num_cus() {
   static int cus = 0;
@@ -160,8 +177,9 @@
   if (!a.pair_mode) return (int)sfx::ceil_div(a.M, BM);
   int t = 0;
   for (int k = 0; k < a.num_slices; ++k) {
+    const int c = a.pair_grouped ? grp_class_at(k) : k;
     a.slice_tile_off[k] = t;
-    t += (a.slice_pair_off[k + 1] - a.slice_pair_off[k] + BM - 1) / BM;
+    t += (a.slice_pair_off[c + 1] - a.slice_pair_off[c] + BM - 1) / BM;
   }
   a.slice_tile_off[a.num_slices] = t;
   return t;
@@ -174,5 +192,7 @@
 void launch_m2_w4(int cfg, const GemmArgs& a, int groups, bool vec, hipStream_t st);
 void launch_m3_w4(int cfg, const GemmArgs& a, int groups, bool vec, hipStream_t st);
 void launch_m3_w8(int cfg, const GemmArgs& a, int groups, bool vec, hipStream_t st);
+void launch_m4_w4(int cfg, const GemmArgs& a, hipStream_t st);
+void launch_m4_w8(int cfg, const GemmArgs& a, hipStream_t st);
 
 }
diff --git a/splatformer_amd/csrc/gemm_k44.hip b/splatformer_amd/csrc/gemm_k44.hip
--- /dev/null
+++ b/splatformer_amd/csrc/gemm_k44.hip
@@ -0,0 +1,15 @@
+#include "gemm_kernel.h"
+
+namespace sfxg {
+
+void launch_m4_w4(int cfg, const GemmArgs& a, hipStream_t st) {
+  switch (cfg) {
+    case 0: launch_grouped<128, 128, 2, 4>(a, st); break;
+    case 1: launch_grouped<128, 96, 4, 4>(a, st); break;
+    case 2: launch_grouped<128, 64, 2, 4>(a, st); break;
+    case 3: launch_grouped<64, 128, 2, 4>(a, st); break;
+    default: launch_grouped<64, 64, 2, 4>(a, st); break;
+  }
+}
+
+}
diff --git a/splatformer_amd/csrc/gemm_k48.hip b/splatformer_amd/csrc/gemm_k48.hip
--- /dev/null
+++ b/splatformer_amd/csrc/gemm_k48.hip
@@ -0,0 +1,12 @@
+#include "gemm_kernel.h"
+
+namespace sfxg {
+
+void launch_m4_w8(int cfg, const GemmArgs& a, hipStream_t st) {
+  switch (cfg) {
+    case 5: launch_grouped<256, 128, 4, 8>(a, st); break;
+    default: launch_grouped<128, 256, 2, 8>(a, st); break;
+  }
+}
+
+}
diff --git a/splatformer_amd/csrc/gemm_kernel.h b/splatformer_amd/csrc/gemm_kernel.h
--- a/splatformer_amd/csrc/gemm_kernel.h
+++ b/splatformer_amd/csrc/gemm_kernel.h
@@ -18,7 +18,8 @@
   constexpr bool SPLIT = SPL != 0;
   static_assert(EPI == EPI_GENERAL || (SPL == 2 && VEC), "specialised epilogues: fp16x2 operands only");
   static_assert((EPI != EPI_LIN && EPI != EPI_LIN_GELU) || MODE == MODE_DENSE, "EPI_LIN*: dense rows");
-  static_assert(EPI != EPI_PAIR_STORE || MODE == MODE_PAIR, "EPI_PAIR_STORE: pair mode");
+  static_assert(EPI != EPI_PAIR_STORE || MODE == MODE_PAIR || MODE == MODE_PAIRG, "EPI_PAIR_STORE: pair mode");
+  static_assert(MODE != MODE_PAIRG || (EPI == EPI_PAIR_STORE && SPL == 2), "MODE_PAIRG: fp16x2, one row per entry");
   constexpr bool F16 = SPL == 2 || SPL == 1;
   constexpr int NTERM = SPL == 1 ? 1 : (F16 ? 2 : 3);
   static_assert(SPL == 0 || SPL == 1 || SPL == 2 || SPL == 3, "operand precision");
@@ -70,6 +71,7 @@
 
   struct Tile {
     int m0, n0, M;
+    int K;
     const int* gidx;
     int gstride;
     const int* out_rows;
@@ -100,10 +102,38 @@
       ti.W = (F16 ? p.Wsp : p.W) + sl * p.slice_w_stride;
       if (p.winv) ti.winv = p.winv + sl * p.slice_winv_stride;
     }
+    if constexpr (MODE == MODE_PAIRG) {
+      int sl = 0;
+      for (int q = 1; q < p.num_slices; ++q)
+        if (p.slice_tile_off[q] <= tm) sl = q;
+      const int cls = grp_class_at(sl);
+      const int base = p.slice_pair_off[cls];
+      ti.M = p.slice_pair_off[cls + 1] - base;
+      ti.m0 = (tm - p.slice_tile_off[sl]) * BM;
+      ti.gidx = p.pair_in + 3ll * base;
+      ti.gstride = 3;
+      ti.out_rows = p.pair_out + base;
+      ti.W = p.Wsp + grp_first(cls) * p.slice_w_stride;
+      ti.K = grp_segs(cls) * p.Kseg;
+    }
     return ti;
   };
 
   int grow[A_ITERS];
+  int gseg[2][A_ITERS];
+  const int spk = MODE == MODE_PAIRG ? p.Kseg / BK : 1;
+  auto load_segs = [&](const Tile& ti, int (&gs)[2][A_ITERS]) {
+    if constexpr (MODE == MODE_PAIRG) {
+      const __amdgpu_buffer_rsrc_t rG = rsrc(ti.gidx);
+#pragma unroll
+      for (int s = 0; s < 2; ++s)
+#pragma unroll
+        for (int i = 0; i < A_ITERS; ++i) {
+          const int m = ti.m0 + lrow + RPP * i;
+          gs[s][i] = bload1i(rG, m < ti.M ? ((unsigned)m * 3u + (unsigned)(s + 1)) * 4u : OOB);
+        }
+    }
+  };
   auto load_rows = [&](const Tile& ti, int kt, int (&rows)[A_ITERS]) {
     if constexpr (MODE != MODE_DENSE) {
       const __amdgpu_buffer_rsrc_t rG = rsrc(ti.gidx);
@@ -111,8 +141,9 @@
 #pragma unroll
       for (int i = 0; i < A_ITERS; ++i) {
         const int m = ti.m0 + lrow + RPP * i;
-        rows[i] = bload1i(rG, (m < ti.M && seg < p.S) ? ((unsigned)m * (unsigned)ti.gstride + (unsigned)seg) * 4u
-                                                      : OOB);
+        rows[i] = bload1i(rG, (m < ti.M && (MODE == MODE_PAIRG || seg < p.S))
+                                  ? ((unsigned)m * (unsigned)ti.gstride + (unsigned)seg) * 4u
+                                  : OOB);
       }
     }
   };
@@ -121,18 +152,25 @@
   auto load_tiles = [&](const Tile& ti, int kt, bool first) {
     const __amdgpu_buffer_rsrc_t rW = rsrc(ti.W);
     const int k = kt * BK + lcol;
-    const bool kin = k < K && !(p.dbg & 2);
+    const bool kin = k < (MODE == MODE_PAIRG ? ti.K : K) && !(p.dbg & 2);
     int seg = 0, kk = k;
     if constexpr (MODE == MODE_GATHERS) {
       seg = k / p.Kseg;
       kk = k - seg * p.Kseg;
     }
+    if constexpr (MODE == MODE_PAIRG) {
+      seg = kt >= 2 * spk ? 2 : (kt >= spk ? 1 : 0);
+      kk = k - seg * p.Kseg;
+    }
 #pragma unroll
     for (int i = 0; i < A_ITERS; ++i) {
       const int m = ti.m0 + lrow + RPP * i;
       const bool mok = m < ti.M;
       unsigned off;
-      if constexpr (MODE != MODE_DENSE) {
+      if constexpr (MODE == MODE_PAIRG) {
+        const int r = seg == 0 ? grow[i] : (seg == 1 ? gseg[0][i] : gseg[1][i]);
+        off = (mok && r >= 0 && kin) ? ((unsigned)r * lda32 + (unsigned)kk) * 4u : OOB;
+      } else if constexpr (MODE != MODE_DENSE) {
         const int r = grow[i];
         off = (mok && r >= 0 && kin && seg < p.S) ? ((unsigned)r * lda32 + (unsigned)kk) * 4u : OOB;
       } else {
@@ -746,9 +784,11 @@
     t = lid;
     if (t >= total_tiles) return;
   }
-  constexpr bool per_tile_rows = MODE == MODE_GATHER1 || MODE == MODE_PAIR;
+  constexpr bool per_tile_rows = MODE == MODE_GATHER1 || MODE == MODE_PAIR || MODE == MODE_PAIRG;
   Tile ti = tile_info(t);
+  if constexpr (MODE == MODE_PAIRG) ke = (ti.K + BK - 1) / BK;
   load_rows(ti, kb, grow);
+  load_segs(ti, gseg);
   load_tiles(ti, kb, true);
   store_tiles(0, true, sp);
   __syncthreads();
@@ -765,8 +805,11 @@
       has_next = nt < total_tiles;
     }
     const Tile tn = has_next ? tile_info(nt) : ti;
+    if constexpr (MODE == MODE_PAIRG) nke = (tn.K + BK - 1) / BK;
     int grow_next[A_ITERS];
+    int gseg_next[2][A_ITERS];
     if constexpr (per_tile_rows) load_rows(tn, 0, grow_next);
+    load_segs(tn, gseg_next);
     zero_acc();
     for (int kt = kb; kt + 1 < ke; ++kt) {
       if constexpr (MODE == MODE_GATHERS) load_rows(ti, kt + 1, grow);
@@ -784,6 +827,13 @@
       if constexpr (per_tile_rows) {
 #pragma unroll
         for (int i = 0; i < A_ITERS; ++i) grow[i] = grow_next[i];
+        if constexpr (MODE == MODE_PAIRG) {
+#pragma unroll
+          for (int i = 0; i < A_ITERS; ++i) {
+            gseg[0][i] = gseg_next[0][i];
+            gseg[1][i] = gseg_next[1][i];
+          }
+        }
       } else {
         load_rows(tn, 0, grow);
       }
@@ -792,7 +842,7 @@
     __builtin_amdgcn_sched_barrier(0);
     compute(buf);
     __builtin_amdgcn_sched_barrier(0);
-    epilogue(ti, kb != 0 || ke != nk, kb == 0);
+    epilogue(ti, MODE != MODE_PAIRG && (kb != 0 || ke != nk), kb == 0);
     if (!has_next) break;
     if constexpr (NBUF == 1) __syncthreads();
     __builtin_amdgcn_sched_barrier(0);
@@ -830,6 +880,19 @@
     }
   }
   gemm_kernel<BM, BN, WGM, NW, true, MODE, 2><<<grid, T, 0, st>>>(a, tiles_n, total);
+}
+
+template <int BM, int BN, int WGM, int NW>
+void launch_grouped(GemmArgs a, hipStream_t st) {
+  const int tiles_n = (int)sfx::ceil_div(a.N, BN);
+  const int total = tiles_m_of(a, BM) * tiles_n;
+  if (total == 0) return;
+  const int slots = (NW == 4 ? kPerCu4 : kPerCu8) * num_cus();
+  const int per = (total + slots - 1) / slots;
+  int grid_x = (total + per - 1) / per;
+  if (grid_x >= 8) grid_x = (grid_x + 7) / 8 * 8;
+  gemm_kernel<BM, BN, WGM, NW, true, MODE_PAIRG, 2, EPI_PAIR_STORE><<<dim3(grid_x, 1, 1), NW * 64, 0, st>>>(a, tiles_n,
+                                                                                                       total);
 }
 
 template <int BM, int BN, int WGM, int NW, int MODE>
diff --git a/splatformer_amd/csrc/subm.hip b/splatformer_amd/csrc/subm.hip
--- a/splatformer_amd/csrc/subm.hip
+++ b/splatformer_amd/csrc/subm.hip
@@ -144,6 +144,7 @@
                                                               int* __restrict__ pair_off, int* __restrict__ pair_pos,
                                                               int* __restrict__ pair_cpos) {
   __shared__ int wc[27][4];
+  const long long cap = (with_centre ? 27ll : 26ll) * n;
   const int i = blockIdx.x * 256 + threadIdx.x, lane = threadIdx.x & 63, wid = threadIdx.x >> 6;
   const bool in = i < n;
   const int* row = nbr + 27ll * (in ? i : 0);
@@ -164,14 +165,15 @@
                                                      __builtin_amdgcn_mbcnt_lo((unsigned)bal[k], 0u));
     const bool fl = (bal[k] >> lane) & 1ull;
     const int p = base + (int)lrank;
-    if (fl) {
+    const bool wr = fl && p >= 0 && p < cap;
+    if (wr) {
       pair_out[p] = i;
       pair_in[p] = row[k];
     }
-    if (pair_pos && in) pair_pos[27ll * i + k] = fl ? p : -1;
-    pk[k] = fl ? p : -1;
+    if (pair_pos && in) pair_pos[27ll * i + k] = wr ? p : -1;
+    pk[k] = wr ? p : -1;
     rank[k] = cnt;
-    cnt += fl ? 1 : 0;
+    cnt += wr ? 1 : 0;
   }
   if (pair_cpos && in) {
     int c[32];
@@ -183,6 +185,97 @@
       for (int q = 0; q <= k; ++q) c[q] = (pk[k] >= 0 && rank[k] == q) ? pk[k] : c[q];
     c[31] = cnt;
     int4* dst = reinterpret_cast<int4*>(pair_cpos + 32ll * i);
+#pragma unroll
+    for (int q = 0; q < 8; ++q) dst[q] = make_int4(c[4 * q], c[4 * q + 1], c[4 * q + 2], c[4 * q + 3]);
+  }
+}
+
+constexpr int GRP_CLS = 54;
+__device__ __forceinline__ int grp_class_of(int pat) {
+  return pat ? (int)((0x54523100u >> (4 * pat)) & 7u) : -1;
+}
+__device__ __forceinline__ int grp_pattern(const int* row, int j, bool in) {
+  return in ? (row[3 * j] >= 0 ? 1 : 0) | (row[3 * j + 1] >= 0 ? 2 : 0) | (row[3 * j + 2] >= 0 ? 4 : 0) : 0;
+}
+__global__ void __launch_bounds__(256) subm_group_count_kernel(int n, const int* __restrict__ nbr,
+                                                               int* __restrict__ counts, int nb) {
+  __shared__ int wc[GRP_CLS][4];
+  const int i = blockIdx.x * 256 + threadIdx.x, lane = threadIdx.x & 63, wid = threadIdx.x >> 6;
+  const bool in = i < n;
+  const int* row = nbr + 27ll * (in ? i : 0);
+#pragma unroll
+  for (int j = 0; j < 9; ++j) {
+    const int cls = grp_class_of(grp_pattern(row, j, in));
+#pragma unroll
+    for (int q = 0; q < 6; ++q) {
+      const unsigned long long bal = __ballot(cls == q);
+      if (lane == 0) wc[6 * j + q][wid] = __popcll(bal);
+    }
+  }
+  __syncthreads();
+  if (threadIdx.x < GRP_CLS) {
+    const int c = threadIdx.x;
+    counts[(long long)c * nb + blockIdx.x] = wc[c][0] + wc[c][1] + wc[c][2] + wc[c][3];
+  }
+}
+__global__ void __launch_bounds__(256) subm_group_write_kernel(int n, const int* __restrict__ nbr,
+                                                               const int* __restrict__ first, int nb,
+                                                               int* __restrict__ grp_in, int* __restrict__ grp_out,
+                                                               int* __restrict__ grp_off, int* __restrict__ grp_cpos) {
+  __shared__ int wc[GRP_CLS][4];
+  const int i = blockIdx.x * 256 + threadIdx.x, lane = threadIdx.x & 63, wid = threadIdx.x >> 6;
+  const bool in = i < n;
+  const int* row = nbr + 27ll * (in ? i : 0);
+  const long long cap = 9ll * n;
+  int cls[9];
+#pragma unroll
+  for (int j = 0; j < 9; ++j) {
+    cls[j] = grp_class_of(grp_pattern(row, j, in));
+#pragma unroll
+    for (int q = 0; q < 6; ++q) {
+      const unsigned long long bal = __ballot(cls[j] == q);
+      if (lane == 0) wc[6 * j + q][wid] = __popcll(bal);
+    }
+  }
+  __syncthreads();
+  if (blockIdx.x == 0 && threadIdx.x < GRP_CLS) grp_off[threadIdx.x] = first[(long long)threadIdx.x * nb];
+  int ent[9], cnt = 0;
+#pragma unroll
+  for (int j = 0; j < 9; ++j) {
+    int p = -1;
+#pragma unroll
+    for (int q = 0; q < 6; ++q) {
+      const unsigned long long bal = __ballot(cls[j] == q);
+      int base = first[(long long)(6 * j + q) * nb + blockIdx.x];
+      for (int w = 0; w < wid; ++w) base += wc[6 * j + q][w];
+      const unsigned lrank = __builtin_amdgcn_mbcnt_hi((unsigned)(bal >> 32),
+                                                       __builtin_amdgcn_mbcnt_lo((unsigned)bal, 0u));
+      if (cls[j] == q) p = base + (int)lrank;
+    }
+    const bool wr = p >= 0 && p < cap;
+    if (wr) {
+      const int q = cls[j];
+      const int f = q < 3 ? q : (q == 4 ? 1 : 0), ns = q < 3 ? 1 : (q < 5 ? 2 : 3);
+      grp_out[p] = i;
+#pragma unroll
+      for (int s = 0; s < 3; ++s) grp_in[3ll * p + s] = (s < ns) ? row[3 * j + (f + s < 3 ? f + s : 2)] : -1;
+    }
+    ent[j] = wr ? p : -1;
+    cnt += wr ? 1 : 0;
+  }
+  if (grp_cpos && in) {
+    int c[32];
+#pragma unroll
+    for (int q = 0; q < 31; ++q) c[q] = -1;
+    int rank = 0;
+#pragma unroll
+    for (int j = 0; j < 9; ++j) {
+#pragma unroll
+      for (int q = 0; q <= j; ++q) c[q] = (ent[j] >= 0 && rank == q) ? ent[j] : c[q];
+      rank += ent[j] >= 0 ? 1 : 0;
+    }
+    c[31] = cnt;
+    int4* dst = reinterpret_cast<int4*>(grp_cpos + 32ll * i);
 #pragma unroll
     for (int q = 0; q < 8; ++q) dst[q] = make_int4(c[4 * q], c[4 * q + 1], c[4 * q + 2], c[4 * q + 3]);
   }
@@ -250,6 +343,7 @@
   SFX_REQUIRE(n >= 0, "sfx_subm_pair_lists: n < 0");
   SFX_REQUIRE(ws_bytes >= sfx_subm_pair_lists_workspace_bytes(n), "sfx_subm_pair_lists: workspace too small");
   SFX_REQUIRE(pair_off, "sfx_subm_pair_lists: null pair_off");
+  SFX_REQUIRE((reinterpret_cast<uintptr_t>(pair_cpos) & 15) == 0, "sfx_subm_pair_lists: pair_cpos must be 16-byte aligned");
   hipStream_t st = sfx::as_stream(stream);
   if (n == 0) {
     hipMemsetAsync(pair_off, 0, 28 * sizeof(int), st);
@@ -269,6 +363,35 @@
                                              pair_cpos);
   return sfx::check_launch("sfx_subm_pair_lists");
 }
+size_t sfx_subm_group_lists_workspace_bytes(int n) {
+  const long long e = (long long)GRP_CLS * sfx::ceil_div(n > 0 ? n : 1, 256);
+  return (size_t)(2 * e * sizeof(int) + 256) + sfx_scan_workspace_bytes(e);
+}
+int sfx_subm_group_lists(int n, const int* nbr, void* ws, size_t ws_bytes, int* grp_in, int* grp_out, int* grp_off,
+                         int* grp_cpos, void* stream) {
+  SFX_REQUIRE(n >= 0, "sfx_subm_group_lists: n < 0");
+  SFX_REQUIRE(ws_bytes >= sfx_subm_group_lists_workspace_bytes(n), "sfx_subm_group_lists: workspace too small");
+  SFX_REQUIRE(grp_off, "sfx_subm_group_lists: null grp_off");
+  SFX_REQUIRE((reinterpret_cast<uintptr_t>(grp_cpos) & 15) == 0, "sfx_subm_group_lists: grp_cpos must be 16-byte aligned");
+  SFX_REQUIRE(9ll * n * 3 < (long long)INT_MAX, "sfx_subm_group_lists: n too large for 32-bit entry indices");
+  hipStream_t st = sfx::as_stream(stream);
+  if (n == 0) {
+    hipMemsetAsync(grp_off, 0, (GRP_CLS + 1) * sizeof(int), st);
+    return sfx::check_launch("sfx_subm_group_lists");
+  }
+  SFX_REQUIRE(nbr && ws && grp_in && grp_out, "sfx_subm_group_lists: null buffer");
+  const int nb = (int)sfx::ceil_div(n, 256);
+  const long long e = (long long)GRP_CLS * nb;
+  int* counts = reinterpret_cast<int*>(ws);
+  int* first = counts + e;
+  char* scan_ws = reinterpret_cast<char*>(first + e);
+  scan_ws += (256 - (reinterpret_cast<uintptr_t>(scan_ws) & 255)) & 255;
+  subm_group_count_kernel<<<nb, 256, 0, st>>>(n, nbr, counts, nb);
+  const int rc = sfx_scan_i32(e, counts, first, 0, scan_ws, sfx_scan_workspace_bytes(e), grp_off + GRP_CLS, stream);
+  if (rc) return rc;
+  subm_group_write_kernel<<<nb, 256, 0, st>>>(n, nbr, first, nb, grp_in, grp_out, grp_off, grp_cpos);
+  return sfx::check_launch("sfx_subm_group_lists");
+}
 int sfx_subm_pair_pos(int n, long long num_pairs, const int* pair_out, const int* pair_off, int* pair_pos,
                       void* stream) {
   SFX_REQUIRE(n >= 0 && num_pairs >= 0 && num_pairs <= 26ll * n, "sfx_subm_pair_pos: bad sizes");
diff --git a/splatformer_amd/ptv3.py b/splatformer_amd/ptv3.py
--- a/splatformer_amd/ptv3.py
+++ b/splatformer_amd/ptv3.py
@@ -129,7 +129,10 @@
                                     ln1.eps, rowexp=re[1] if re is not None and re[0] is xc else None)
         else:
             wf, bf = self.cpe_fused()
-            t = ops.subm_conv(xc, point.nbr, wf, bf, partials=ops.subm_partials_ok(xc, point.nbr, C))
+            if ops.subm_grouped_ok(C, xc):
+                t = ops.subm_conv(xc, point.nbr, wf, bf, grouped=True)
+            else:
+                t = ops.subm_conv(xc, point.nbr, wf, bf, partials=ops.subm_partials_ok(xc, point.nbr, C))
             if ops.cpe_ln_qkv_ok(t, C, self.attn.qkv.weight):
                 x1, qkv, q_amax = ops.cpe_ln_qkv(t, x, ln_c.weight, ln_c.bias, ln1.weight, ln1.bias, ln1.eps,
                                                  self.attn.qkv)
@@ -203,7 +206,8 @@
         return ops.pool_geometry_begin(point.codes_phys, point.order_phys, self._pd(point))
 
     def geometry_end(self, point: Point, perm: Sequence[int], state, m: Optional[int] = None,
-                     deferred: Optional[list] = None, pairs: bool = True, centre: bool = False):
+                     deferred: Optional[list] = None, pairs: bool = True, centre: bool = False,
+                     groups: bool = False):
         pd = self._pd(point)
         depth = point.serialized_depth - pd
         code_bits = point.code_bits - 3 * pd
@@ -219,17 +223,18 @@
             new.offset = torch.cumsum(torch.bincount(batch.long().cpu(), minlength=len(point.offset)), 0).tolist()
         else:
             new.offset = [m]
-        new.nbr = ops.subm_neighbors(grid, new.get("batch"), with_pairs=pairs, centre=centre)
+        new.nbr = ops.subm_neighbors(grid, new.get("batch"), with_pairs=pairs, centre=centre, groups=groups)
         return new, sidx, idx_ptr, m
 
     def geometry(self, point: Point, perm: Sequence[int]):
         return self.geometry_end(point, perm, self.geometry_begin(point))
 
     def run(self, point: Point, perm: Sequence[int], m: Optional[int] = None, deferred: Optional[list] = None,
-            pairs: bool = True, centre: bool = False) -> Point:
+            pairs: bool = True, centre: bool = False, groups: bool = False) -> Point:
         st = self.geometry_begin(point)
         pf = ops.linear(point.feat, self.proj.weight, self.proj.bias)
-        new, sidx, idx_ptr, m = self.geometry_end(point, perm, st, m, deferred, pairs=pairs, centre=centre)
+        new, sidx, idx_ptr, m = self.geometry_end(point, perm, st, m, deferred, pairs=pairs, centre=centre,
+                                                  groups=groups)
         sc, sh = bn_affine(self.norm[0])
         new.feat = ops.segment_max_affine_act(pf, idx_ptr, sidx, m, sc, sh, ops.ACT_GELU)
         return new
@@ -345,10 +350,14 @@
 
     def stage_needs_pairs(self, s: int, n: Optional[int] = None) -> bool:
         chans = [self.enc_channels[s]] + ([self.dec_channels[s]] if s < len(self.dec_channels) else [])
-        return not all(ops.subm_fused_ok(c, n) for c in chans)
+        return not all(ops.subm_fused_ok(c, n) or ops.subm_grouped_ok(c) for c in chans)
+
+    def stage_needs_groups(self, s: int, n: Optional[int] = None) -> bool:
+        chans = [self.enc_channels[s]] + ([self.dec_channels[s]] if s < len(self.dec_channels) else [])
+        return any(ops.subm_grouped_ok(c) and not ops.subm_fused_ok(c, n) for c in chans)
 
     def prepare(self, data_dict, perms: Optional[List[Sequence[int]]] = None, pairs: bool = True,
-                reorder: bool = False, centre_pairs: bool = False) -> Point:
+                reorder: bool = False, centre_pairs: bool = False, groups: bool = False) -> Point:
         feat = data_dict["feat"]
         _lib.require_gpu(feat)
         dev = feat.device
@@ -365,7 +374,7 @@
             offs = torch.tensor(offset, dtype=torch.int64, device=dev)
             _lib.call("sfx_offsets_to_batch", n, B, offs.data_ptr(), batch.data_ptr(), _lib.stream())
         nbr = None if (reorder or not NBR_EARLY) else ops.subm_neighbors(grid, batch, with_pairs=pairs,
-                                                                          centre=centre_pairs)
+                                                                          centre=centre_pairs, groups=groups)
         d = data_dict.get("serialized_depth")
         if isinstance(d, _lib.HostRead):
             depth = int(d.get()[0]).bit_length()
@@ -388,7 +397,8 @@
             point.perm = perm
         if batch is not None:
             point.batch = batch
-        point.nbr = nbr if nbr is not None else ops.subm_neighbors(grid, batch, with_pairs=pairs, centre=centre_pairs)
+        point.nbr = nbr if nbr is not None else ops.subm_neighbors(grid, batch, with_pairs=pairs, centre=centre_pairs,
+                                                                   groups=groups)
         return point
 
     @torch.no_grad()
@@ -404,7 +414,7 @@
             emb_feat = ops.linear(feat, emb.weight, emb.bias, scale=sc, shift=sh, act=ops.ACT_GELU)
         cp = ops.SUBM_CENTRE_PAIRS
         point = self.prepare(data_dict, perms, pairs=self.stage_needs_pairs(0, feat.shape[0]), reorder=reorder,
-                             centre_pairs=cp)
+                             centre_pairs=cp, groups=self.stage_needs_groups(0, feat.shape[0]))
         perm = point.get("perm")
         point.feat = emb_feat if perm is None else ops.move_rows(emb_feat, perm)
         final_out = out
@@ -427,7 +437,8 @@
                 if name == "down":
                     m = counts_rd.get()[k - 1] if counts_rd is not None else None
                     point = mod.run(point, self._draw_perm(perms, k), m=m, deferred=deferred,
-                                    pairs=self.stage_needs_pairs(s, m), centre=cp)
+                                    pairs=self.stage_needs_pairs(s, m), centre=cp,
+                                    groups=self.stage_needs_groups(s, m))
                     k += 1
                 else:
                     point = mod.run(point)
diff --git a/splatformer_amd/ptv3_ops.py b/splatformer_amd/ptv3_ops.py
--- a/splatformer_amd/ptv3_ops.py
+++ b/splatformer_amd/ptv3_ops.py
@@ -361,7 +361,8 @@
 
 
 def cpe_ln_qkv_ok(t, C: int, qkv_weight: Tensor) -> bool:
-    return (LN_QKV and isinstance(t, SubmPartials) and C in LN_QKV_CHANNELS and get_precision() == "fp32"
+    return (LN_QKV and isinstance(t, SubmPartials) and not isinstance(t, SubmGroupPartials)
+            and C in LN_QKV_CHANNELS and get_precision() == "fp32"
             and weight_split(qkv_weight)[0] is not None)
 
 
@@ -671,6 +672,40 @@
         return self._pos
 
 
+class GroupLists:
+
+    def __init__(self, nbr: Tensor):
+        n = nbr.shape[0]
+        dev = nbr.device
+        cap = max(1, 9 * n)
+        self.grp_in = torch.empty(cap, 3, device=dev, dtype=torch.int32)
+        self.grp_out = torch.empty(cap, device=dev, dtype=torch.int32)
+        self.off_dev = torch.empty(55, device=dev, dtype=torch.int32)
+        self.cpos = torch.empty(max(1, n), 32, device=dev, dtype=torch.int32)
+        ws = _lib.workspace(_lib.fn("sfx_subm_group_lists_workspace_bytes")(n), dev)
+        call("sfx_subm_group_lists", n, ptr(nbr), ptr(ws), ws.numel(), ptr(self.grp_in), ptr(self.grp_out),
+             ptr(self.off_dev), ptr(self.cpos), stream())
+        self._rd = _lib.HostRead(self.off_dev)
+        self._off = None
+        self._off_c = None
+
+    @property
+    def grp_off(self) -> List[int]:
+        if self._off is None:
+            self._off = self._rd.get()
+        return self._off
+
+    @property
+    def off_host(self):
+        if self._off_c is None:
+            self._off_c = (ctypes.c_int * 55)(*self.grp_off)
+        return self._off_c
+
+    @property
+    def num_entries(self) -> int:
+        return self.grp_off[54]
+
+
 class SubmMap:
 
     def __init__(self, nbr: Tensor, mask: Optional[Tensor], centre_pref: bool = False):
@@ -678,6 +713,13 @@
         self.centre_pref = centre_pref
         self._lists = {}
         self._order = None
+        self._groups = None
+        self._npairs = None
+
+    def groups(self) -> GroupLists:
+        if self._groups is None:
+            self._groups = GroupLists(self.nbr)
+        return self._groups
 
     def lists(self, centre: bool = False) -> PairLists:
         pl = self._lists.get(centre)
@@ -727,13 +769,18 @@
 
     @property
     def num_pairs(self) -> int:
+        if False not in self._lists and self._groups is not None:
+            if self._npairs is None:
+                self._npairs = int(((self.nbr >= 0).sum() - (self.nbr[:, 13] >= 0).sum()).item())
+            return self._npairs
         return self.lists(False).num_pairs
 
 
 SUBM_MASK = os.environ.get("SFX_SUBM_MASK", "0") == "1"
 
 
-def subm_neighbors(grid_coord: Tensor, batch: Optional[Tensor], with_pairs: bool = True, centre: bool = False):
+def subm_neighbors(grid_coord: Tensor, batch: Optional[Tensor], with_pairs: bool = True, centre: bool = False,
+                   groups: bool = False):
     n = grid_coord.shape[0]
     dev = grid_coord.device
     l2 = _lib.fn("sfx_subm_table_log2")(n)
@@ -744,6 +791,8 @@
     call("sfx_subm_neighbors", n, ptr(grid_coord, torch.int32), ptr(batch), l2, ptr(tk), ptr(tv), ptr(nbr), ptr(mask),
          None, stream())
     smap = SubmMap(nbr, mask, centre_pref=centre)
+    if groups:
+        smap.groups()
     if with_pairs:
         smap.lists(centre)
     return smap
@@ -836,9 +885,58 @@
         return out
 
 
+class SubmGroupPartials(SubmPartials):
+
+    def __init__(self, bias: Tensor, partials: Tensor, cpos: Tensor, num_entries: int):
+        super().__init__(bias, partials, None, num_entries, ldt=0, cpos=cpos)
+
+    @property
+    def pair_pos(self) -> Tensor:
+        raise RuntimeError("SubmGroupPartials has no [n][27] pair index: its rows are per (point, triple), see cpos")
+
+    def total(self) -> Tensor:
+        n = self.cpos.shape[0]
+        out = self.centre.expand(n, -1).clone()
+        pos = self.cpos.long()
+        for q in range(9):
+            sel = pos[:, q] >= 0
+            if bool(sel.any()):
+                out[sel] += self.partials[pos[sel, q]]
+        return out
+
+
+SUBM_GROUPED = os.environ.get("SFX_SUBM_GROUPED", "1") != "0"
+SUBM_GROUPED_CHANNELS = tuple(int(c) for c in os.environ.get("SFX_SUBM_GROUPED_CHANNELS", "128,256,512").split(",")
+                              if c)
+
+
+def subm_grouped_ok(C: int, x: Optional[Tensor] = None) -> bool:
+    return (SUBM_GROUPED and SUBM_PARTIALS and C in SUBM_GROUPED_CHANNELS and C in PAIRS_LN_CHANNELS and C % 32 == 0
+            and _lib.fn("sfx_gemm_split_mode")(C) == 2 and get_precision() == "fp32"
+            and (x is None or (x.shape[1] == C and x.is_contiguous() and x.data_ptr() % 16 == 0
+                               and 9 * x.shape[0] * C * 4 + 64 < 0x7ffffff0)))
+
+
+def subm_conv_grouped(x: Tensor, smap: "SubmMap", weight: Tensor, bias: Optional[Tensor]) -> SubmGroupPartials:
+    n, cin = x.shape
+    cout = weight.shape[0]
+    wsp = weight_split(weight)
+    if wsp[0] is None:
+        raise RuntimeError("subm_conv_grouped: the weight has no fp16x2 split (27 * Cin < 64 or not a multiple of 4)")
+    gl = smap.groups()
+    ne = gl.num_entries
+    part = torch.empty(max(1, ne), cout, device=x.device, dtype=torch.float32)
+    px, ldx = _rows(x)
+    call("sfx_subm_conv_grouped", n, cin, cout, px, ldx, ptr(gl.grp_in), gl.off_host, ptr(part), cout, *wsp, stream())
+    b = bias if bias is not None else torch.zeros(cout, device=x.device, dtype=torch.float32)
+    return SubmGroupPartials(b.contiguous(), part, gl.cpos, ne)
+
+
 def subm_conv(x: Tensor, smap: "SubmMap", weight: Tensor, bias: Optional[Tensor],
               out: Optional[Tensor] = None, x_amax: Optional[Tuple[int, int]] = None,
-              w_amax: Optional[Tuple[int, int]] = None, partials: bool = False):
+              w_amax: Optional[Tuple[int, int]] = None, partials: bool = False, grouped: bool = False):
+    if grouped:
+        return subm_conv_grouped(x, smap, weight, bias)
     n, cin = x.shape
     cout = weight.shape[0]
     if out is None:
```

Measured after the change: 709.4 renders/s, median of 5. +3.6%, better.
